# tennisonliu/bayesian-neural-network

Measured on AMD Instinct MI355X. Metric: MC-forward-samples/sec + KL-elements/sec, 784-1200-1200-10 BNN, higher is better.
Workload: dtype bf16

## Files before the change

bayesian-neural-network_amd/bnn_hip/_lib.py:

```python
from __future__ import annotations

import ctypes as C
import os

_HERE = os.path.dirname(os.path.abspath(__file__))
LIB_PATH = os.environ.get("BNN_HIP_LIB") or os.path.join(_HERE, "libbnn_hip.so")
ABI_VERSION = 9

F32, BF16 = 0, 1
MATH_F32, MATH_BF16, MATH_BF16X3 = 0, 1, 2
EPS_PHILOX, EPS_MEMORY, EPS_ZERO = 0, 1, 2
PRIOR_GAUSS, PRIOR_MIXTURE = 0, 1
NLL_REGRESSION, NLL_CLASSIFICATION = 0, 1
FORM_AUTO, FORM_TILE, FORM_GEMM, FORM_GEMM_KSLICE, FORM_BLOCK256 = 0, 1, 2, 3, 4

EXPORTS = (
    "bnn_version", "bnn_philox_rounds", "bnn_status_string",
    "bnn_bbb_linear_fwd_workspace_bytes", "bnn_bbb_split_scratch_bytes", "bnn_bbb_split_scratch_zero_bytes", "bnn_bbb_linear_fwd",
    "bnn_bbb_linear_bwd_workspace_bytes",
    "bnn_bbb_linear_bwd", "bnn_lr_linear_bwd_workspace_bytes", "bnn_lr_linear_bwd", "bnn_adam_step", "bnn_nll_bwd", "bnn_mc_softmax_mean", "bnn_elbo_loss",
    "bnn_elbo_loss_nll_bwd", "bnn_stage_inputs", "bnn_stage_inputs_cast", "bnn_bbb_sample_weights", "bnn_bbb_sample_workspace_bytes",
    "bnn_lr_linear_fwd_workspace_bytes", "bnn_lr_split_scratch_bytes", "bnn_lr_split_scratch_zero_bytes", "bnn_lr_linear_fwd", "bnn_lr_final_fwd", "bnn_lr_plan", "bnn_bbb_plan", "bnn_lr_prepare_bytes", "bnn_lr_prepare", "bnn_lr_prepare_x3_bytes", "bnn_lr_prepare_x3", "bnn_lr_prepare_many",
    "bnn_gauss_kl_workspace_bytes", "bnn_gauss_kl",
    "bnn_elbo_finalize", "bnn_bbb_final_fwd", "bnn_bbb_final_scratch_bytes", "bnn_philox_normal", "bnn_cast_bf16", "bnn_softplus", "bnn_eval_prepare",
    "bnn_ece_workspace_bytes", "bnn_ece", "bnn_snr_db", "bnn_snr_prune", "bnn_mc_predictive",
    "bnn_bandit_rows", "bnn_bandit_act", "bnn_bandit_replay",
    "bnn_bandit_rows_group", "bnn_bandit_act_group", "bnn_bandit_replay_group", "bnn_mlp_group_fwd", "bnn_mlp_group_train",
    "bnn_bbb_group_workspace_bytes", "bnn_bbb_group_fwd", "bnn_bbb_group_train",
    "bnn_dense_fwd", "bnn_dense_plan", "bnn_dropout_mask",
    "bnn_dense_loss", "bnn_dense_bwd", "bnn_sgd_step",
    "bnn_epoch_permutation", "bnn_epoch_stage",
    "bnn_snr_select_workspace_bytes", "bnn_snr_select", "bnn_prune_codes", "bnn_pruned_fwd", "bnn_prune_sweep_tail",
    "bnn_acquire_topk_workspace_bytes", "bnn_acquire_topk", "bnn_acquire_compose", "bnn_acquire_random",
    "bnn_param_hist_workspace_bytes", "bnn_param_hist",
    "bnn_mc_score_workspace_bytes", "bnn_mc_score",
    "bnn_sparse_count", "bnn_sparse_fill", "bnn_sparse_fwd",
)


class Prior(C.Structure):
    _fields_ = [("kind", C.c_int32), ("sigma_p", C.c_float), ("pi", C.c_float),
                ("sigma1", C.c_float), ("sigma2", C.c_float)]


class BbbFwdArgs(C.Structure):
    _fields_ = [
        ("struct_bytes", C.c_uint32),
        ("n_samples", C.c_int32), ("batch", C.c_int32), ("in_features", C.c_int32), ("out_features", C.c_int32),
        ("x", C.c_void_p), ("x_dtype", C.c_int32), ("x_per_sample", C.c_int32),
        ("w_mu", C.c_void_p), ("w_rho", C.c_void_p), ("b_mu", C.c_void_p), ("b_rho", C.c_void_p),
        ("eps_mode", C.c_int32), ("math", C.c_int32),
        ("eps_w", C.c_void_p), ("eps_b", C.c_void_p),
        ("seed", C.c_uint64), ("layer_id", C.c_uint32), ("sample_offset", C.c_uint32),
        ("sample_counter", C.c_void_p), ("sample_group", C.c_uint32), ("sample_group_stride", C.c_uint32),
        ("eps_w_dump", C.c_void_p), ("eps_b_dump", C.c_void_p),
        ("prior", Prior),
        ("want_stats", C.c_int32), ("relu", C.c_int32),
        ("workspace", C.c_void_p), ("workspace_bytes", C.c_size_t),
        ("log_prior", C.c_void_p), ("log_q", C.c_void_p),
        ("y", C.c_void_p), ("y_dtype", C.c_int32), ("form", C.c_int32),
        ("split_scratch", C.c_void_p), ("split_scratch_bytes", C.c_size_t), ("w_sigma", C.c_void_p),
        ("w_sampled", C.c_void_p), ("b_sampled", C.c_void_p), ("rider", C.c_void_p), ("y_bf16_copy", C.c_void_p),
        ("w_sampled_t_out", C.c_void_p), ("x_lo", C.c_void_p), ("y_lo", C.c_void_p),
    ]


SAMPLE_MAX_LAYERS = 8


class SampleLayer(C.Structure):
    _fields_ = [
        ("in_features", C.c_int32), ("out_features", C.c_int32), ("layer_id", C.c_uint32), ("reserved", C.c_int32),
        ("w_mu", C.c_void_p), ("w_rho", C.c_void_p), ("b_mu", C.c_void_p), ("b_rho", C.c_void_p),
        ("w_out", C.c_void_p), ("b_out", C.c_void_p), ("workspace", C.c_void_p), ("workspace_bytes", C.c_size_t),
        ("prior", Prior), ("reserved2", C.c_int32),
    ]


class SampleArgs(C.Structure):
    _fields_ = [
        ("struct_bytes", C.c_uint32), ("n_layers", C.c_int32), ("n_samples", C.c_int32), ("sample_offset", C.c_uint32),
        ("seed", C.c_uint64), ("sample_counter", C.c_void_p), ("sample_group", C.c_uint32), ("sample_group_stride", C.c_uint32),
        ("layer", SampleLayer * SAMPLE_MAX_LAYERS),
        ("cast_src", C.c_void_p), ("cast_dst", C.c_void_p), ("cast_n", C.c_int64),
    ]


class LrRider(C.Structure):
    _fields_ = [
        ("struct_bytes", C.c_uint32), ("in_features", C.c_int32), ("out_features", C.c_int32),
        ("w_mu", C.c_void_p), ("w_rho", C.c_void_p), ("b_mu", C.c_void_p), ("b_rho", C.c_void_p),
        ("w_frag", C.c_void_p), ("w_frag_bytes", C.c_size_t), ("kl_workspace", C.c_void_p), ("kl_workspace_bytes", C.c_size_t),
    ]


class LrFwdArgs(C.Structure):
    _fields_ = [
        ("struct_bytes", C.c_uint32),
        ("n_samples", C.c_int32), ("batch", C.c_int32), ("in_features", C.c_int32), ("out_features", C.c_int32),
        ("x", C.c_void_p), ("x_dtype", C.c_int32), ("x_per_sample", C.c_int32),
        ("w_mu", C.c_void_p), ("w_rho", C.c_void_p), ("b_mu", C.c_void_p), ("b_rho", C.c_void_p),
        ("eps_mode", C.c_int32), ("math", C.c_int32),
        ("eps_act", C.c_void_p), ("eps_b", C.c_void_p),
        ("seed", C.c_uint64), ("layer_id", C.c_uint32), ("sample_offset", C.c_uint32),
        ("sample_counter", C.c_void_p), ("sample_group", C.c_uint32), ("sample_group_stride", C.c_uint32),
        ("eps_act_dump", C.c_void_p), ("eps_b_dump", C.c_void_p),
        ("sigma_p", C.c_float), ("want_kl", C.c_int32), ("relu", C.c_int32), ("form", C.c_int32),
        ("workspace", C.c_void_p), ("workspace_bytes", C.c_size_t),
        ("kl_out", C.c_void_p),
        ("y", C.c_void_p), ("y_dtype", C.c_int32), ("reserved2", C.c_int32),
        ("x_sq", C.c_void_p), ("y_sq", C.c_void_p), ("w_frag", C.c_void_p), ("v_out", C.c_void_p),
        ("hfac_out", C.c_void_p), ("y_bf16_copy", C.c_void_p),
        ("rider", C.POINTER(LrRider)), ("split_scratch", C.c_void_p), ("split_scratch_bytes", C.c_size_t),
        ("x_lo", C.c_void_p), ("y_lo", C.c_void_p),
    ]


class BbbBwdArgs(C.Structure):
    _fields_ = [
        ("struct_bytes", C.c_uint32),
        ("n_samples", C.c_int32), ("batch", C.c_int32), ("in_features", C.c_int32), ("out_features", C.c_int32),
        ("x", C.c_void_p), ("x_per_sample", C.c_int32), ("relu", C.c_int32),
        ("gy", C.c_void_p), ("y", C.c_void_p),
        ("w_mu", C.c_void_p), ("w_rho", C.c_void_p), ("b_mu", C.c_void_p), ("b_rho", C.c_void_p),
        ("eps_mode", C.c_int32), ("math", C.c_int32),
        ("eps_w", C.c_void_p), ("eps_b", C.c_void_p),
        ("seed", C.c_uint64), ("layer_id", C.c_uint32), ("sample_offset", C.c_uint32),
        ("prior", Prior), ("gx_relu_mask", C.c_int32),
        ("g_log_prior", C.c_void_p), ("g_log_q", C.c_void_p),
        ("g_w_mu", C.c_void_p), ("g_w_rho", C.c_void_p), ("g_b_mu", C.c_void_p), ("g_b_rho", C.c_void_p),
        ("g_x", C.c_void_p),
        ("workspace", C.c_void_p), ("workspace_bytes", C.c_size_t),
        ("sample_counter", C.c_void_p), ("w_sampled", C.c_void_p),
        ("w_sampled_t", C.c_void_p), ("gy_bf16", C.c_void_p), ("g_x_bf16", C.c_void_p),
    ]


class LrBwdArgs(C.Structure):
    _fields_ = [
        ("struct_bytes", C.c_uint32),
        ("n_samples", C.c_int32), ("batch", C.c_int32), ("in_features", C.c_int32), ("out_features", C.c_int32),
        ("x", C.c_void_p), ("x_per_sample", C.c_int32), ("relu", C.c_int32),
        ("gy", C.c_void_p), ("y", C.c_void_p), ("v", C.c_void_p),
        ("w_mu", C.c_void_p), ("w_rho", C.c_void_p), ("b_mu", C.c_void_p), ("b_rho", C.c_void_p),
        ("eps_mode", C.c_int32), ("math", C.c_int32),
        ("eps_act", C.c_void_p), ("eps_b", C.c_void_p),
        ("seed", C.c_uint64), ("layer_id", C.c_uint32), ("sample_offset", C.c_uint32),
        ("sigma_p", C.c_float), ("gx_relu_mask", C.c_int32),
        ("g_kl", C.c_void_p),
        ("g_w_mu", C.c_void_p), ("g_w_rho", C.c_void_p), ("g_b_mu", C.c_void_p), ("g_b_rho", C.c_void_p),
        ("g_x", C.c_void_p), ("workspace", C.c_void_p), ("workspace_bytes", C.c_size_t),
        ("sample_counter", C.c_void_p), ("hfac", C.c_void_p),
    ]


ADAM_MAX_TENSORS = 16


class AdamArgs(C.Structure):
    _fields_ = [
        ("struct_bytes", C.c_uint32), ("n_tensors", C.c_int32),
        ("param", C.c_void_p * ADAM_MAX_TENSORS), ("grad", C.c_void_p * ADAM_MAX_TENSORS),
        ("exp_avg", C.c_void_p * ADAM_MAX_TENSORS), ("exp_avg_sq", C.c_void_p * ADAM_MAX_TENSORS),
        ("numel", C.c_int64 * ADAM_MAX_TENSORS),
        ("lr", C.c_double), ("beta1", C.c_double), ("beta2", C.c_double), ("eps", C.c_double), ("weight_decay", C.c_double),
        ("step", C.c_uint32), ("bump_by", C.c_uint32),
        ("lr_device", C.c_void_p), ("step_device", C.c_void_p), ("step_advance", C.c_int32), ("grad_dtype", C.c_int32),
        ("ticket", C.c_void_p), ("bump_counter", C.c_void_p),
    ]


class LossArgs(C.Structure):
    _fields_ = [("beta", C.c_void_p), ("total_samples", C.c_float), ("grad_scale", C.c_float), ("out4", C.c_void_p),
                ("g_a", C.c_void_p), ("g_b", C.c_void_p), ("g_kl3", C.c_void_p), ("g_logits", C.c_void_p)]


class FinalizeArgs(C.Structure):
    _fields_ = [
        ("struct_bytes", C.c_uint32),
        ("n_layers", C.c_int32), ("local_reparam", C.c_int32),
        ("n_samples", C.c_int32), ("batch", C.c_int32), ("classes", C.c_int32),
        ("layer_workspace", C.c_void_p * 8), ("layer_in", C.c_int32 * 8), ("layer_out", C.c_int32 * 8),
        ("prior", Prior),
        ("logits", C.c_void_p), ("target", C.c_void_p),
        ("nll_mode", C.c_int32), ("nll_sigma", C.c_float),
        ("log_prior", C.c_void_p), ("log_q", C.c_void_p), ("kl", C.c_void_p), ("nll", C.c_void_p),
        ("sample_counter", C.c_void_p), ("sample_counter_inc", C.c_uint32), ("reserved", C.c_uint32),
        ("sums", C.c_void_p), ("ticket", C.c_void_p), ("scratch", C.c_void_p), ("scratch_bytes", C.c_size_t),
        ("group_samples", C.c_int32), ("target_per_group", C.c_int32),
        ("loss", C.POINTER(LossArgs)),
    ]


class Plan(C.Structure):
    _fields_ = [("form", C.c_int32), ("k_classes", C.c_int32), ("waves", C.c_int32), ("batch_rows", C.c_int32),
                ("k_slices", C.c_int32), ("blocks", C.c_int32), ("lds_bytes", C.c_int32), ("features_per_block", C.c_int32)]


PREPARE_MAX = 8
PREPARE_MANY_MAX = 8


class PrepareArgs(C.Structure):
    _fields_ = [("struct_bytes", C.c_uint32), ("n_softplus", C.c_int32),
                ("rho", C.c_void_p * PREPARE_MAX), ("sigma", C.c_void_p * PREPARE_MAX), ("n", C.c_int64 * PREPARE_MAX),
                ("cast_src", C.c_void_p), ("cast_dst", C.c_void_p), ("cast_dst_sq", C.c_void_p), ("cast_n", C.c_int64),
                ("cast_dst_lo", C.c_void_p)]


PREDICTIVE_MAX_QUANTILES = 8
PREDICTIVE_MAX_QUANTILE_SAMPLES = 1024


class McPredictiveArgs(C.Structure):
    _fields_ = [("struct_bytes", C.c_uint32), ("mode", C.c_int32),
                ("groups", C.c_int32), ("n_samples", C.c_int32), ("batch", C.c_int32), ("classes", C.c_int32),
                ("logits", C.c_void_p), ("scale", C.c_float), ("sigma", C.c_float),
                ("probs", C.c_void_p), ("preds", C.c_void_p), ("predictive_entropy", C.c_void_p),
                ("expected_entropy", C.c_void_p), ("mutual_information", C.c_void_p),
                ("mean", C.c_void_p), ("variance", C.c_void_p), ("predictive_variance", C.c_void_p),
                ("n_quantiles", C.c_int32), ("reserved", C.c_int32),
                ("quantile", C.c_double * PREDICTIVE_MAX_QUANTILES), ("quantiles", C.c_void_p)]


BANDIT_MAX_ACTIONS = 64
BANDIT_MAX_BUFFER = 8192


class BanditActArgs(C.Structure):
    _fields_ = [("struct_bytes", C.c_uint32), ("n_actions", C.c_int32), ("n_labels", C.c_int32), ("n_samples", C.c_int32),
                ("output_sample_stride", C.c_int32), ("context_dim", C.c_int32), ("n_contexts", C.c_int64),
                ("buffer_size", C.c_int32), ("sample_counter_inc", C.c_uint32), ("max_steps", C.c_int64),
                ("n_indices", C.c_int64), ("epsilon", C.c_float), ("reserved", C.c_uint32), ("seed", C.c_uint64),
                ("x", C.c_void_p), ("labels", C.c_void_p), ("rewards", C.c_void_p), ("oracle", C.c_void_p),
                ("indices", C.c_void_p), ("outputs", C.c_void_p), ("step", C.c_void_p), ("cur_index", C.c_void_p),
                ("rows", C.c_void_p), ("actions", C.c_void_p), ("reward_out", C.c_void_p), ("regrets", C.c_void_p),
                ("counts", C.c_void_p), ("ring_index", C.c_void_p), ("ring_action", C.c_void_p), ("ring_reward", C.c_void_p),
                ("sample_counter", C.c_void_p)]


class BanditReplayArgs(C.Structure):
    _fields_ = [("struct_bytes", C.c_uint32), ("batch_size", C.c_int32), ("num_batches", C.c_int32), ("buffer_size", C.c_int32),
                ("context_dim", C.c_int32), ("n_actions", C.c_int32), ("n_contexts", C.c_int64), ("seed", C.c_uint64),
                ("step", C.c_void_p), ("x", C.c_void_p), ("ring_index", C.c_void_p), ("ring_action", C.c_void_p),
                ("ring_reward", C.c_void_p), ("workspace", C.c_void_p), ("slab", C.c_void_p), ("targets", C.c_void_p),
                ("n_batches", C.c_void_p)]


MLP_GROUP_MAX_IN = 128
MLP_GROUP_MAX_HIDDEN = 128
MLP_GROUP_MAX_OUT = 1
MLP_GROUP_MAX_BATCH = 64
MLP_GROUP_MAX_BATCHES = 128
MLP_GROUP_MAX_AGENTS = 4096


class BanditGroupArgs(C.Structure):
    _fields_ = [("struct_bytes", C.c_uint32), ("n_agents", C.c_int32), ("blocks_host", C.c_void_p), ("blocks", C.c_void_p),
                ("blocks_bytes", C.c_int64)]


class MlpGroupAgent(C.Structure):
    _fields_ = [("param", C.c_void_p * 6), ("exp_avg", C.c_void_p * 6), ("exp_avg_sq", C.c_void_p * 6), ("step", C.c_void_p),
                ("lr", C.c_void_p), ("slab", C.c_void_p), ("targets", C.c_void_p), ("n_batches", C.c_void_p), ("loss", C.c_void_p),
                ("rows", C.c_void_p), ("outputs", C.c_void_p)]


class MlpGroupArgs(C.Structure):
    _fields_ = [("struct_bytes", C.c_uint32), ("n_agents", C.c_int32), ("in_features", C.c_int32), ("hidden", C.c_int32),
                ("out_features", C.c_int32), ("batch", C.c_int32), ("max_batches", C.c_int32), ("n_rows", C.c_int32),
                ("beta1", C.c_double), ("beta2", C.c_double), ("eps", C.c_double), ("weight_decay", C.c_double),
                ("agents_host", C.c_void_p), ("agents", C.c_void_p), ("agents_bytes", C.c_int64)]


BBB_GROUP_MAX_SAMPLES = 8


class BbbGroupAgent(C.Structure):
    _fields_ = [("param", C.c_void_p * 12), ("exp_avg", C.c_void_p * 12), ("exp_avg_sq", C.c_void_p * 12), ("step", C.c_void_p),
                ("lr", C.c_void_p), ("slab", C.c_void_p), ("targets", C.c_void_p), ("n_batches", C.c_void_p),
                ("loss_info", C.c_void_p), ("rows", C.c_void_p), ("outputs", C.c_void_p), ("sample_counter", C.c_void_p),
                ("workspace", C.c_void_p), ("eps_seed", C.c_uint64), ("eps_mode", C.c_int32), ("reserved", C.c_int32)]


class BbbGroupArgs(C.Structure):
    _fields_ = [("struct_bytes", C.c_uint32), ("n_agents", C.c_int32), ("in_features", C.c_int32), ("hidden", C.c_int32),
                ("out_features", C.c_int32), ("batch", C.c_int32), ("max_batches", C.c_int32), ("n_rows", C.c_int32),
                ("n_samples", C.c_int32), ("prior", Prior),
                ("beta1", C.c_double), ("beta2", C.c_double), ("eps", C.c_double), ("weight_decay", C.c_double),
                ("beta", C.c_float * MLP_GROUP_MAX_BATCHES), ("workspace_bytes", C.c_int64),
# ... 396 lines not shown
```

bayesian-neural-network_amd/bnn_hip/engine.py:

```python
from __future__ import annotations

import os
from typing import List, Optional, Sequence, Tuple

import torch

from . import _lib as L
from . import ops
from .functional import AllReduceSumFn, BBBLinearFn, ElboFn, LayerCall, LRLinearFn, NetCall, NLLFn
from .ops import Predictive
from .runtime import state, take_samples


CAST_INPUT_MIN_SAMPLES = 4
CAST_INPUT_MIN_SAMPLES_LR = 1
LR_SQUARES_MIN_SAMPLES = 7
SPLIT_MIN_SAMPLES = 4
SPLIT_MIN_WEIGHTS = 250_000
SPLIT_MAX_UNITS = 1024

FUSED_ELBO_NODE = True


FINAL_ROWS_MAX_SAMPLES = 16
# ... 433 lines not shown
        self.counter = torch.tensor([first], dtype=torch.int32, device=dev)
        S = self.n_local
        B = self.x.shape[-2]
        self.lr_x3 = (self.lr and state.math == L.MATH_BF16X3 and self.G > 1 and len(self.specs) >= 2 and S >= LR_SQUARES_MIN_SAMPLES and
                      self.x.dtype == torch.float32 and
                      all(sp.in_out[0] % 8 == 0 and lr_use_prepare(sp.in_out[1], S, B) for sp in self.specs[:-1]))
        math_mode = self.math = L.MATH_BF16X3 if self.lr_x3 else effective_math(self.lr)
        self.x3 = math_mode == L.MATH_BF16X3
        hid = torch.float32 if math_mode == L.MATH_F32 else torch.bfloat16
        self.bufs, self.ws, self.bufs_lo = [], [], []
        nl_ = len(self.specs)
        for i, sp in enumerate(self.specs):
            fin, fout = sp.in_out
            last = i == nl_ - 1
            f32_out = last or (self.lr_x3 and i == nl_ - 2)
            self.bufs.append(torch.empty((S, B, fout), dtype=torch.float32 if f32_out else hid, device=dev))
            self.bufs_lo.append(torch.empty((S, B, fout), dtype=torch.bfloat16, device=dev) if (self.x3 and not f32_out) else None)
            self.ws.append(ops.lr_workspace(fout, dev) if self.lr else ops.bbb_workspace(S, fout, dev))
        keys = ("kl",) if self.lr else ("log_prior", "log_q")
        self.out = {k: torch.zeros(S, dtype=torch.float32, device=dev) for k in keys + ("nll",)}
        self._sums = torch.zeros((self.G, 4), dtype=torch.float32, device=dev)
        self.sums = self._sums if self.G > 1 else self._sums.view(4)
        self.ticket = torch.zeros(1, dtype=torch.int32, device=dev)
        self.scratch = ops.final_scratch(S, dev) if (not self.lr or wide_nll(self.specs, B) or self.specs[-1].in_out[1] <= 16) else None
        self.lib = [use_block_gemm(sp, B, hid) for sp in self.specs]
        self.lib_w = [torch.empty((S, sp.in_out[1], sp.in_out[0]), dtype=torch.bfloat16, device=dev) if lb else None
                      for sp, lb in zip(self.specs, self.lib)]
        self.lib_b = [torch.empty((S, sp.in_out[1]), dtype=torch.float32, device=dev) if lb else None
                      for sp, lb in zip(self.specs, self.lib)]
        for i, (sp, lb) in enumerate(zip(self.specs, self.lib)):
            if lb:
                self.ws[i] = ops.sample_workspace(S, sp.in_out[0], sp.in_out[1], dev)
        shared0 = self.lr and not self.G > 1 and lr_unit_samples(S, True) == 1
        k3s_first = (self.lr and hid == torch.bfloat16 and len(self.specs) > 1 and self.specs[0].in_out[0] % 8 == 0 and
                     lr_use_split(self.specs[0].in_out[1], S, B, shared0) and not self.G > 1)
        shared0 = shared0 and k3s_first
        self.x16 = (torch.empty(self.x.shape, dtype=torch.bfloat16, device=dev)
                    if (hid == torch.bfloat16 and self.x.dtype == torch.float32 and
                        (self.lib[0] or S >= (CAST_INPUT_MIN_SAMPLES_LR if self.lr else CAST_INPUT_MIN_SAMPLES)) and
                        not k3s_first) else None)
        self.x16_lo = torch.empty(self.x.shape, dtype=torch.bfloat16, device=dev) if (self.x3 and self.x16 is not None) else None
        self.lr_sq = self.lr and (self.x16 is not None or (k3s_first and hid == torch.bfloat16)) and S >= LR_SQUARES_MIN_SAMPLES
        self.x16_sq = torch.empty(self.x.shape, dtype=torch.bfloat16, device=dev) if (self.lr_sq and self.x16 is not None) else None
        self.bufs_sq = [torch.empty(b.shape, dtype=torch.bfloat16, device=dev)
                        if (self.lr_sq and i < len(self.bufs) - 1 and b.dtype == torch.bfloat16) else None for i, b in enumerate(self.bufs)]
        self.split = [ops.split_scratch(S, B, sp.in_out[1], dev)
                      if (not self.lr and hid == torch.bfloat16 and not self.lib[i] and
                          use_split(sp.in_out[0], sp.in_out[1], S, B)) else None
                      for i, sp in enumerate(self.specs)]
        self.lr_split = [ops.lr_split_scratch(lr_unit_samples(S, shared0 and i == 0), B, sp.in_out[1], dev)
                         if (self.lr and hid == torch.bfloat16 and i < len(self.specs) - 1 and
                             lr_use_split(sp.in_out[1], S, B, shared0 and i == 0)) else None
                         for i, sp in enumerate(self.specs)]
        self.wsigma = [torch.empty_like(sp.m.weight_rho.detach())
                      if (not self.lr and hid == torch.bfloat16 and not lb and hoist_sigma(*sp.in_out, S, B)) else None
                      for sp, lb in zip(self.specs, self.lib)]
        self.wfrag = [None] * len(self.specs)
        if self.lr_sq:
            frag_bytes = L.load().bnn_lr_prepare_x3_bytes if self.lr_x3 else L.load().bnn_lr_prepare_bytes
            self.wfrag = [torch.empty(frag_bytes(*sp.in_out) // 4, dtype=torch.float32, device=dev)
                          if (lr_use_prepare(sp.in_out[1], S, B) and not (shared0 and i == 0) and not (self.lr_x3 and i == nl_ - 1)) else None
                          for i, sp in enumerate(self.specs)]
        nl = len(self.specs)
        self.lr_rider = None
        if (self.lr_sq and not self.lr_x3 and self.wfrag[nl - 1] is None and any(w is not None for w in self.wfrag) and
                self.scratch is not None and not wide_nll(self.specs, B) and self.specs[-1].in_out[1] <= 16 and S <= LR_FINAL_ROWS_MAX_SAMPLES):
            self.wfrag[nl - 1] = torch.empty(L.load().bnn_lr_prepare_bytes(*self.specs[-1].in_out) // 4, dtype=torch.float32, device=dev)
        if (self.lr and hid == torch.bfloat16 and nl > 1 and self.wfrag[nl - 1] is None and self.scratch is not None and
                not wide_nll(self.specs, B) and self.specs[-1].in_out[1] <= 16 and S <= 16 and self.lr_split[nl - 2] is not None and
                lr_kslice_expected(*self.specs[-2].in_out, S, B)):
            sp = self.specs[-1]
            self.lr_rider = dict(w_mu=sp.m.weight_mu.detach(), w_rho=sp.m.weight_rho.detach(), b_mu=sp.m.bias_mu.detach(),
                                 b_rho=sp.m.bias_rho.detach(), workspace=self.ws[nl - 1],
                                 w_frag=torch.empty(L.load().bnn_lr_prepare_bytes(*sp.in_out) // 4, dtype=torch.float32, device=dev))
        self.pre_from = presample_from(self.specs, S, B, hid)
        self.rows = self.pre_from >= 0
        self.w_pre, self.b_pre = [None] * len(self.specs), [None] * len(self.specs)
        if self.rows:
            for i in range(self.pre_from + 1, len(self.specs)):
                k_i, n_i = self.specs[i].in_out
                self.w_pre[i] = torch.empty((S, n_i, k_i), dtype=torch.bfloat16, device=dev)
                self.b_pre[i] = torch.empty((S, n_i), dtype=torch.float32, device=dev)
                self.ws[i] = ops.sample_workspace(S, k_i, n_i, dev)
        self.graph = None
        self.calls = None
        if capture == "calls":
            rec_stream = self.stream if self.stream is not None else torch.cuda.current_stream()
            with torch.cuda.stream(rec_stream):
                self._enqueue()
            take_samples(self.total_samples)
            torch.cuda.synchronize()
            before = torch.cuda.memory_stats(dev).get("allocation.all.allocated", 0)
            with L.recording() as calls, torch.cuda.stream(rec_stream):
                self._eager()
            take_samples(self.total_samples * self.per_replay)
            torch.cuda.synchronize()
            if torch.cuda.memory_stats(dev).get("allocation.all.allocated", 0) != before:
                raise ops.BnnHipError("GraphedElbo(capture='calls'): the evaluation allocated device memory while it was recorded -- "
                                      "a replay would launch on freed buffers; use capture=True (hipGraph) for this configuration")
            self.calls = list(calls)
        elif capture:
            self._enqueue()
            take_samples(self.total_samples)
            torch.cuda.synchronize()
            side = self.stream if self.stream is not None else torch.cuda.Stream()
            side.wait_stream(torch.cuda.current_stream())
            with torch.cuda.stream(side):
                g = torch.cuda.CUDAGraph()
                with torch.cuda.graph(g, stream=side):
                    self._eager()
            torch.cuda.current_stream().wait_stream(side)
            self.graph = g

    def _enqueue(self):
        math_mode = self.math
        h_sq, h_lo = None, None
        hoist = [i for i, w in enumerate(self.wsigma) if w is not None]
        h = self.x
        if self.x16 is not None or hoist:
            ops.eval_prepare([self.specs[i].m.weight_rho.detach() for i in hoist], [self.wsigma[i] for i in hoist],
                             cast=self.x if self.x16 is not None else None, cast_out=self.x16,
                             cast_out_sq=self.x16_sq, cast_out_lo=self.x16_lo)
            if self.x16 is not None:
                h, h_sq, h_lo = self.x16, self.x16_sq, self.x16_lo
        last = len(self.specs) - 1
        if self.lr and any(w is not None for w in self.wfrag):
            jobs = [dict(w_mu=sp.m.weight_mu.detach(), w_rho=sp.m.weight_rho.detach(), b_mu=sp.m.bias_mu.detach(),
                         b_rho=sp.m.bias_rho.detach(), workspace=self.ws[i], out=self.wfrag[i])
                    for i, sp in enumerate(self.specs) if self.wfrag[i] is not None]
            ops.lr_prepare_many(jobs, x3=self.lr_x3)
        grp = dict(sample_group=self.group, sample_group_stride=self.samples) if self.G > 1 else {}
        fin_kw = dict(layer_in=[sp.in_out[0] for sp in self.specs], layer_out=[sp.in_out[1] for sp in self.specs],
                      local_reparam=self.lr, prior=self.specs[0].m._prior_spec, n_samples=self.n_local,
                      target=self.target, mode=self.net.mode, nll_sigma=self.sigma, sample_counter=self.counter,
                      sample_counter_inc=self.total_samples, out=self.out, sums=self._sums,
                      ticket=self.ticket, scratch=self.scratch, group_samples=self.group)
        for i, sp in enumerate(self.specs):
            p = tuple(t.detach() for t in (sp.m.weight_mu, sp.m.weight_rho, sp.m.bias_mu, sp.m.bias_rho))
            common = dict(n_samples=self.n_local, math_mode=math_mode, relu=sp.relu, y_dtype=self.bufs[i].dtype,
                          eps_mode=L.EPS_PHILOX, seed=state.seed, layer_id=sp.layer_id, sample_offset=self.lo,
                          sample_counter=self.counter, workspace=self.ws[i], out=self.bufs[i], form=state.form, **grp)
            if self.lr:
                if self.lr_x3 and i == last:
                    common["math_mode"] = L.MATH_F32
                if i == last and self.scratch is not None and not wide_nll(self.specs, self.x.shape[-2]):
                    ops.lr_final_fwd((h,) + p, dict(sigma_p=sp.m._prior_spec.sigma_p, want_kl=True, x_sq=h_sq,
                                                    w_frag=self.lr_rider["w_frag"] if self.lr_rider is not None else self.wfrag[i],
                                                    **common), dict(workspaces=self.ws, **fin_kw))
                    return
                ops.lr_linear_fwd(h, *p, sigma_p=sp.m._prior_spec.sigma_p, want_kl=True, x_sq=h_sq,
                                  out_sq=self.bufs_sq[i], w_frag=self.wfrag[i], split_scratch=self.lr_split[i],
                                  rider=self.lr_rider if i == last - 1 else None,
                                  x_lo=h_lo if self.lr_x3 else None, out_lo=self.bufs_lo[i] if self.lr_x3 else None, **common)
                h_sq = self.bufs_sq[i]
            elif self.lib[i]:
                self._sample_layer(i, grp)
                ops.bbb_sampled_matmul(h, self.lib_w[i], self.lib_b[i], n_samples=self.n_local, relu=sp.relu,
                                       y_dtype=self.bufs[i].dtype, out=self.bufs[i])
                if i == last:
                    ops.elbo_finalize(workspaces=self.ws, logits=self.bufs[i], **fin_kw)
            else:
                kw = dict(prior=sp.m._prior_spec, want_stats=True, split_scratch=self.split[i], w_sigma=self.wsigma[i], **common)
                if self.x3:
                    kw.update(x_lo=h_lo if h.dtype == torch.bfloat16 else None, out_lo=self.bufs_lo[i])
                if i == last and self.rows:
                    ops.bbb_final_fwd((h, None, None, None, None),
                                      dict(n_samples=self.n_local, prior=sp.m._prior_spec, math_mode=math_mode, relu=sp.relu,
                                           y_dtype=self.bufs[i].dtype, eps_mode=L.EPS_ZERO, want_stats=False, out=self.bufs[i],
                                           w_sampled=self.w_pre[i], b_sampled=self.b_pre[i]),
                                      dict(workspaces=self.ws, **fin_kw))
                elif i == last:
                    ops.bbb_final_fwd((h,) + p, kw, dict(workspaces=self.ws[:last], **fin_kw))
                else:
                    if i == self.pre_from:
                        kw["rider"] = ops.build_sample_job(
                            [dict(w_mu=q.m.weight_mu.detach(), w_rho=q.m.weight_rho.detach(), b_mu=q.m.bias_mu.detach(),
                                  b_rho=q.m.bias_rho.detach(), prior=q.m._prior_spec, layer_id=q.layer_id,
                                  workspace=self.ws[j], w_out=self.w_pre[j], b_out=self.b_pre[j])
                             for j, q in enumerate(self.specs) if j > i],
                            n_samples=self.n_local, seed=state.seed, sample_offset=self.lo, sample_counter=self.counter, **grp)
                    ops.bbb_linear_fwd(h, *p, **kw)
            h, h_lo = self.bufs[i], self.bufs_lo[i]
        if self.lr:
            ops.elbo_finalize(workspaces=self.ws, logits=h, **fin_kw)

    def _sample_layer(self, i, grp):
        sp = self.specs[i]
        p = tuple(t.detach() for t in (sp.m.weight_mu, sp.m.weight_rho, sp.m.bias_mu, sp.m.bias_rho))
        ops.bbb_sample_weights([dict(w_mu=p[0], w_rho=p[1], b_mu=p[2], b_rho=p[3], prior=sp.m._prior_spec, layer_id=sp.layer_id,
                                     workspace=self.ws[i], w_out=self.lib_w[i], b_out=self.lib_b[i])],
                               n_samples=self.n_local, seed=state.seed, sample_offset=self.lo, sample_counter=self.counter, **grp)

    def _eager(self):
        for _ in range(self.per_replay):
            self._enqueue()

    def replay(self) -> torch.Tensor:
        if self.calls is not None:
            for fn, args, name in self.calls:
                rc = fn(*args)
                if rc:
                    L.check(rc, name)
            take_samples(self.total_samples * self.per_replay)
            return self.sums
        if self.stream is not None:
            with torch.cuda.stream(self.stream):
                self.graph.replay() if self.graph is not None else self._eager()
        elif self.graph is not None:
            self.graph.replay()
        else:
            self._eager()
        take_samples(self.total_samples * self.per_replay)
        return self.sums

    @property
    def logits(self) -> torch.Tensor:
        return self.bufs[-1]


class GraphedPredict(GraphedElbo):

    def __init__(self, net, x: torch.Tensor, samples: int, capture: bool = True, stream: Optional[torch.cuda.Stream] = None):
        if net.mode != "classification":
            raise ops.BnnHipError("GraphedPredict: the MC-averaged class prediction exists for classification networks")
        xf = net._flat(x)
        self.probs = torch.empty((xf.shape[0], net._specs()[-1].in_out[1]), dtype=torch.float32, device=x.device)
        self.preds = torch.empty(xf.shape[0], dtype=torch.int64, device=x.device)
        super().__init__(net, x, torch.zeros(xf.shape[0], dtype=torch.int64, device=x.device), samples, capture=capture, stream=stream)

    def _enqueue(self):
        super()._enqueue()
        ops.mc_softmax_mean(self.logits, 1.0 / self.samples, out_probs=self.probs, out_preds=self.preds if self.world == 1 else None,
                            want_preds=self.world == 1)

    def replay(self):
        super().replay()
        if self.world > 1:
            import torch.distributed as dist
            dist.all_reduce(self.probs, op=dist.ReduceOp.SUM)
            self.preds.copy_(torch.argmax(self.probs, dim=1))
        return self.preds, self.probs


class GraphedPredictive(GraphedElbo):

    def __init__(self, net, x: torch.Tensor, samples: int, quantiles=None, sigma: float = 1.0, capture=True,
                 stream: Optional[torch.cuda.Stream] = None, stacked: bool = False):
        mode = net.mode
        if mode not in ("classification", "regression"):
            raise Exception("Training mode must be either 'regression' or 'classification'")
        if mode == "classification" and quantiles:
            raise ops.BnnHipError("GraphedPredictive: quantiles are a regression summary")
        self.mode, self.quantile_levels, self.pred_sigma = mode, ops.quantile_levels(quantiles), float(sigma)
        if self.quantile_levels and dist_info()[1] > 1:
            raise ops.BnnHipError("GraphedPredictive: quantiles need every MC sample on one rank (sample sharding is on)")
        G = int(x.shape[0]) if stacked else 1
        B = net._flat(x[0] if stacked else x).shape[0]
        Cc = net._specs()[-1].in_out[1]
        lead = (G, B) if stacked else (B,)
        target = (torch.zeros(lead, dtype=torch.int64, device=x.device) if mode == "classification"
                  else torch.zeros(lead + (Cc,), dtype=torch.float32, device=x.device))
        self._pred = ops.predictive_buffers(mode, G, B, Cc, x.device, self.quantile_levels)
        self.result = self._pred if stacked else _first_minibatch(self._pred)
        super().__init__(net, x, target, samples, sigma=sigma, capture=capture, stream=stream, stacked=stacked)

    def _enqueue(self):
        super()._enqueue()
# ... 63 lines not shown
```

bayesian-neural-network_amd/bnn_hip/ops.py:

```python
from __future__ import annotations

import ctypes as C
import math
from dataclasses import dataclass
from typing import NamedTuple, Optional, Sequence

import torch

from . import _lib as L
from ._lib import BnnHipError


@dataclass(frozen=True)
class PriorSpec:
    mixture: bool = False
    sigma_p: float = 1.0
    pi: float = 0.5
    sigma1: float = 1.0
    sigma2: float = 1.0

    @staticmethod
    def from_init(prior_init: Sequence[float], mixture: bool) -> "PriorSpec":
        if mixture:
            assert len(prior_init) == 3, "Scale Mixture Prior requires three values in prior initialisation"
            return PriorSpec(True, 1.0, float(prior_init[0]), math.exp(prior_init[1]), math.exp(prior_init[2]))
        assert len(prior_init) == 1, "Gaussian Prior requires one value in prior initialisation"
        return PriorSpec(False, float(prior_init[0]))

    def c(self) -> L.Prior:
        return L.Prior(L.PRIOR_MIXTURE if self.mixture else L.PRIOR_GAUSS, self.sigma_p, self.pi,
                       self.sigma1, self.sigma2)


def _stream() -> int:
    return torch._C._cuda_getCurrentRawStream(torch._C._cuda_getDevice())


def require_device(*tensors: torch.Tensor):
    for t in tensors:
        if t is not None and not t.is_cuda:
            raise BnnHipError(
                "bnn_hip: the Bayes-by-backprop hot path runs on a ROCm device only (tensor is on "
                f"{t.device}); there is no CPU fallback.  Move the module and its inputs to DEVICE.")


def _f32c(t: torch.Tensor, name: str) -> torch.Tensor:
    if t.dtype != torch.float32:
        raise BnnHipError(f"{name} must be float32, got {t.dtype}")
    return t if t.is_contiguous() else t.contiguous()


def _ptr(t: Optional[torch.Tensor]) -> Optional[int]:
    return None if t is None else t.data_ptr()


def _dt(t: torch.Tensor) -> int:
    if t.dtype == torch.float32:
        return L.F32
    if t.dtype == torch.bfloat16:
        return L.BF16
    raise BnnHipError(f"activations must be float32 or bfloat16, got {t.dtype}")


def _exact_unless_bf16(math_mode: int) -> int:
    return L.MATH_F32 if math_mode == L.MATH_BF16X3 else math_mode


def _x3(x: torch.Tensor, n_samples: int):
    if x.dim() == 2:
        xs = x if x.is_contiguous() else x.contiguous()
        return xs, x.shape[0], x.shape[1], 0
    if x.dim() == 3:
        if x.shape[0] < 1 or n_samples % x.shape[0]:
            raise BnnHipError(f"x has {x.shape[0]} row blocks, which does not divide {n_samples} samples")
        xs = x if x.is_contiguous() else x.contiguous()
        return xs, x.shape[1], x.shape[2], n_samples // x.shape[0]
    raise BnnHipError(f"x must be [batch,in] or [rows,batch,in], got {tuple(x.shape)}")


def bbb_workspace(n_samples: int, out_features: int, device) -> torch.Tensor:
    nbytes = L.load().bnn_bbb_linear_fwd_workspace_bytes(n_samples, out_features)
    return torch.empty(nbytes // 4, dtype=torch.float32, device=device)


def split_scratch(n_samples: int, batch: int, out_features: int, device) -> torch.Tensor:
    lib = L.load()
    nbytes = lib.bnn_bbb_split_scratch_bytes(n_samples, batch, out_features)
    t = torch.empty((nbytes + 3) // 4, dtype=torch.int32, device=device)
    t[:lib.bnn_bbb_split_scratch_zero_bytes(n_samples, batch, out_features) // 4].zero_()
    return t


_split_cache = {}


def split_scratch_cached(n_samples: int, batch: int, out_features: int, device) -> torch.Tensor:
    if torch.cuda.is_current_stream_capturing():
        return split_scratch(n_samples, batch, out_features, device)
    key = (str(device), torch.cuda.current_stream(device).cuda_stream, n_samples, batch, out_features)
    t = _split_cache.get(key)
    if t is None:
        if len(_split_cache) >= 16:
            _split_cache.clear()
        t = _split_cache[key] = split_scratch(n_samples, batch, out_features, device)
    return t


def final_scratch(n_samples: int, device) -> torch.Tensor:
    nbytes = L.load().bnn_bbb_final_scratch_bytes(n_samples)
    return torch.zeros((nbytes + 3) // 4, dtype=torch.int32, device=device)


def lr_split_scratch(n_samples: int, batch: int, out_features: int, device) -> torch.Tensor:
    lib = L.load()
    nbytes = lib.bnn_lr_split_scratch_bytes(n_samples, batch, out_features)
    t = torch.empty((nbytes + 3) // 4, dtype=torch.int32, device=device)
    t[:lib.bnn_lr_split_scratch_zero_bytes(n_samples, batch, out_features) // 4].zero_()
    return t


_lr_split_cache = {}


def lr_split_scratch_cached(n_samples: int, batch: int, out_features: int, device) -> torch.Tensor:
    if torch.cuda.is_current_stream_capturing():
        return lr_split_scratch(n_samples, batch, out_features, device)
    key = (str(device), torch.cuda.current_stream(device).cuda_stream, n_samples, batch, out_features)
    t = _lr_split_cache.get(key)
    if t is None:
        if len(_lr_split_cache) >= 16:
            _lr_split_cache.clear()
        t = _lr_split_cache[key] = lr_split_scratch(n_samples, batch, out_features, device)
    return t


def lr_workspace(out_features: int, device) -> torch.Tensor:
    nbytes = L.load().bnn_lr_linear_fwd_workspace_bytes(out_features)
    return torch.empty(nbytes // 4, dtype=torch.float32, device=device)


def _y16(a, y: torch.Tensor) -> torch.Tensor:
    if y.dtype != torch.float32:
        raise BnnHipError("want_y16 goes with fp32 y")
    y16 = torch.empty(tuple(y.shape), dtype=torch.bfloat16, device=y.device)
    a.y_bf16_copy = y16.data_ptr()
    return y16


def _bbb_build(x, w_mu, w_rho, b_mu, b_rho, *, n_samples: int, prior: PriorSpec, math_mode: int,
               relu: bool, y_dtype: torch.dtype, eps_mode: int, eps_w=None, eps_b=None, seed: int = 0,
               layer_id: int = 0, sample_offset: int = 0, want_stats: bool = True,
               want_scalars: bool = False, dump_eps: bool = False, workspace=None, sample_counter=None,
               out=None, split_scratch=None, w_sigma=None, form: int = 0, sample_group: int = 0,
               sample_group_stride: int = 0, w_sampled=None, b_sampled=None, rider=None, want_y16: bool = False, wt_out=None,
               x_lo=None, out_lo=None):
    require_device(x, w_mu, w_rho, b_mu, b_rho, eps_w, eps_b, w_sampled, b_sampled)
    if w_sampled is not None:
        if w_sampled.dtype != torch.bfloat16 or b_sampled is None or b_sampled.dtype != torch.float32 or \
                not w_sampled.is_contiguous() or not b_sampled.is_contiguous() or w_sampled.dim() != 3:
            raise BnnHipError("w_sampled must be contiguous bf16 [S,out,in], b_sampled contiguous fp32 [S,out]")
        if w_sampled.shape[0] != n_samples or b_sampled.numel() != n_samples * w_sampled.shape[1]:
            raise BnnHipError("w_sampled / b_sampled do not match n_samples")
        N, K = w_sampled.shape[1], w_sampled.shape[2]
        xs, B, Kx, per_sample = _x3(x, n_samples)
        if Kx != K:
            raise BnnHipError(f"shape mismatch: x[...,{Kx}] sampled weight {tuple(w_sampled.shape)}")
        y = out if out is not None else torch.empty((n_samples, B, N), dtype=y_dtype, device=xs.device)
        a = L.BbbFwdArgs()
        a.struct_bytes = C.sizeof(L.BbbFwdArgs)
        a.n_samples, a.batch, a.in_features, a.out_features = n_samples, B, K, N
        a.x, a.x_dtype, a.x_per_sample = xs.data_ptr(), _dt(xs), per_sample
        a.eps_mode, a.math = L.EPS_ZERO, L.MATH_BF16
        a.want_stats, a.relu = 0, int(relu)
        a.y, a.y_dtype = y.data_ptr(), _dt(y)
        a.w_sampled, a.b_sampled = w_sampled.data_ptr(), b_sampled.data_ptr()
        if wt_out is not None:
            require_device(wt_out)
            if wt_out.dtype != torch.bfloat16 or not wt_out.is_contiguous() or tuple(wt_out.shape) != (n_samples, K, N):
                raise BnnHipError("wt_out must be a contiguous bf16 [samples,in,out] tensor")
            a.w_sampled_t_out = wt_out.data_ptr()
        a.form = int(form)
        y16 = _y16(a, y) if want_y16 else None
        return a, dict(y=y, y16=y16, workspace=None, log_prior=None, log_q=None, eps_w=None, eps_b=None), (xs, w_sampled, b_sampled, y)
    w_mu, w_rho = _f32c(w_mu, "weight_mu"), _f32c(w_rho, "weight_rho")
    b_mu, b_rho = _f32c(b_mu, "bias_mu"), _f32c(b_rho, "bias_rho")
    N, K = w_mu.shape
    xs, B, Kx, per_sample = _x3(x, n_samples)
    if Kx != K or tuple(w_rho.shape) != (N, K) or tuple(b_mu.shape) != (N,) or tuple(b_rho.shape) != (N,):
        raise BnnHipError(f"shape mismatch: x[...,{Kx}] weight {tuple(w_mu.shape)} bias {tuple(b_mu.shape)}")
    dev = xs.device
    y = out if out is not None else torch.empty((n_samples, B, N), dtype=y_dtype, device=dev)
    if want_stats and workspace is None:
        workspace = bbb_workspace(n_samples, N, dev)
    lp = torch.empty(n_samples, dtype=torch.float32, device=dev) if want_scalars else None
    lq = torch.empty(n_samples, dtype=torch.float32, device=dev) if want_scalars else None
    if eps_mode == L.EPS_MEMORY:
        eps_w, eps_b = _f32c(eps_w, "eps_w"), _f32c(eps_b, "eps_b")
        if eps_w.numel() != n_samples * N * K or eps_b.numel() != n_samples * N:
            raise BnnHipError("eps_w/eps_b must be [samples,out,in] / [samples,out]")
    dw = torch.empty((n_samples, N, K), dtype=torch.float32, device=dev) if dump_eps else None
    db = torch.empty((n_samples, N), dtype=torch.float32, device=dev) if dump_eps else None
    a = L.BbbFwdArgs()
    a.struct_bytes = C.sizeof(L.BbbFwdArgs)
    a.n_samples, a.batch, a.in_features, a.out_features = n_samples, B, K, N
    a.x, a.x_dtype, a.x_per_sample = xs.data_ptr(), _dt(xs), per_sample
    a.w_mu, a.w_rho, a.b_mu, a.b_rho = w_mu.data_ptr(), w_rho.data_ptr(), b_mu.data_ptr(), b_rho.data_ptr()
    a.eps_mode, a.math = eps_mode, math_mode
    a.eps_w, a.eps_b = _ptr(eps_w) if eps_mode == L.EPS_MEMORY else None, _ptr(eps_b) if eps_mode == L.EPS_MEMORY else None
    a.seed, a.layer_id, a.sample_offset = seed & 0xFFFFFFFFFFFFFFFF, layer_id, sample_offset & 0xFFFFFFFF
    a.sample_counter = _ptr(sample_counter)
    a.sample_group, a.sample_group_stride = int(sample_group), int(sample_group_stride)
    a.form = int(form)
    a.eps_w_dump, a.eps_b_dump = _ptr(dw), _ptr(db)
    a.prior = prior.c()
    a.want_stats, a.relu = int(want_stats), int(relu)
    a.workspace = _ptr(workspace) if want_stats else None
    a.workspace_bytes = workspace.numel() * 4 if (want_stats and workspace is not None) else 0
    a.log_prior, a.log_q = _ptr(lp), _ptr(lq)
    a.y, a.y_dtype = y.data_ptr(), _dt(y)
    y_lo = None
    if math_mode == L.MATH_BF16X3:
        if xs.dtype == torch.bfloat16:
            if x_lo is None or x_lo.dtype != torch.bfloat16 or tuple(x_lo.shape) != tuple(x.shape) or not x_lo.is_contiguous():
                raise BnnHipError("bf16x3 math on bf16 x needs x_lo: the contiguous bf16 low plane, shaped like x")
            require_device(x_lo)
            a.x_lo = x_lo.data_ptr()
        if y.dtype == torch.bfloat16:
            y_lo = out_lo if out_lo is not None else torch.empty(tuple(y.shape), dtype=torch.bfloat16, device=dev)
            if y_lo.dtype != torch.bfloat16 or y_lo.numel() != y.numel() or not y_lo.is_contiguous():
                raise BnnHipError("out_lo must be a contiguous bf16 tensor shaped like y")
            a.y_lo = y_lo.data_ptr()
    if w_sigma is not None:
        a.w_sigma = w_sigma.data_ptr()
    if split_scratch is not None:
        a.split_scratch = split_scratch.data_ptr()
        a.split_scratch_bytes = split_scratch.numel() * split_scratch.element_size()
    if rider is not None:
        a.rider = C.addressof(rider[0])
    res = dict(y=y, y16=_y16(a, y) if want_y16 else None, workspace=workspace, log_prior=lp, log_q=lq, eps_w=dw, eps_b=db, y_lo=y_lo)
    keep = (xs, w_mu, w_rho, b_mu, b_rho, eps_w, eps_b, sample_counter, split_scratch, w_sigma, rider, x_lo, y_lo)
    a._keep = keep
    return a, res, keep


def bbb_linear_fwd(x, w_mu, w_rho, b_mu, b_rho, **kw):
    lib = L.load()
    a, res, keep = _bbb_build(x, w_mu, w_rho, b_mu, b_rho, **kw)
    L.check(lib.bnn_bbb_linear_fwd(C.byref(a), _stream()), "bnn_bbb_linear_fwd")
    return res


def _plan_dict(pl: L.Plan) -> dict:
    return {k: getattr(pl, k) for k, _ in L.Plan._fields_}


def bbb_plan(x, w_mu, w_rho, b_mu, b_rho, **kw) -> dict:
    a, res, keep = _bbb_build(x, w_mu, w_rho, b_mu, b_rho, **kw)
    pl = L.Plan()
    L.check(L.load().bnn_bbb_plan(C.byref(a), C.byref(pl)), "bnn_bbb_plan")
    return _plan_dict(pl)


def sample_workspace(n_samples: int, fin: int, fout: int, device) -> torch.Tensor:
    nbytes = L.load().bnn_bbb_sample_workspace_bytes(n_samples, fin, fout) or \
        L.load().bnn_bbb_linear_fwd_workspace_bytes(n_samples, fout)
    return torch.empty(nbytes // 4, dtype=torch.float32, device=device)


def build_sample_job(layers, *, n_samples: int, seed: int = 0, sample_offset: int = 0, sample_counter=None, cast=None,
                     sample_group: int = 0, sample_group_stride: int = 0):
    if not 1 <= len(layers) <= L.SAMPLE_MAX_LAYERS:
        raise BnnHipError(f"bbb_sample_weights: 1..{L.SAMPLE_MAX_LAYERS} layers per launch")
    a = L.SampleArgs()
    a.struct_bytes = C.sizeof(L.SampleArgs)
    a.n_layers, a.n_samples = len(layers), int(n_samples)
    a.seed, a.sample_offset = seed & 0xFFFFFFFFFFFFFFFF, sample_offset & 0xFFFFFFFF
    a.sample_counter = _ptr(sample_counter)
    a.sample_group, a.sample_group_stride = int(sample_group), int(sample_group_stride)
    res, keep = [], [sample_counter]
    for i, ly in enumerate(layers):
        w_mu, w_rho = _f32c(ly["w_mu"], "weight_mu"), _f32c(ly["w_rho"], "weight_rho")
        b_mu, b_rho = _f32c(ly["b_mu"], "bias_mu"), _f32c(ly["b_rho"], "bias_rho")
        require_device(w_mu, w_rho, b_mu, b_rho)
        N, K = w_mu.shape
        if K % 8:
            raise BnnHipError("bbb_sample_weights: in_features must be a multiple of 8")
        if tuple(w_rho.shape) != (N, K) or tuple(b_mu.shape) != (N,) or tuple(b_rho.shape) != (N,):
            raise BnnHipError("bbb_sample_weights: parameter shapes disagree")
        dev = w_mu.device
        ws = ly.get("workspace")
        if ws is None:
            ws = sample_workspace(n_samples, K, N, dev)
        w = ly.get("w_out")
        if w is None:
            w = torch.empty((n_samples, N, K), dtype=torch.bfloat16, device=dev)
        b = ly.get("b_out")
        if b is None:
            b = torch.empty((n_samples, N), dtype=torch.float32, device=dev)
        if w.dtype != torch.bfloat16 or w.numel() != n_samples * N * K or b.dtype != torch.float32 or b.numel() != n_samples * N:
            raise BnnHipError("bbb_sample_weights: w_out must be bf16 [S,out,in], b_out fp32 [S,out]")
        e = a.layer[i]
        e.in_features, e.out_features, e.layer_id = K, N, int(ly.get("layer_id", i))
        e.w_mu, e.w_rho, e.b_mu, e.b_rho = w_mu.data_ptr(), w_rho.data_ptr(), b_mu.data_ptr(), b_rho.data_ptr()
        e.w_out, e.b_out = w.data_ptr(), b.data_ptr()
        e.workspace, e.workspace_bytes = ws.data_ptr(), ws.numel() * 4
        e.prior = ly["prior"].c()
        res.append(dict(w=w, b=b, workspace=ws))
        keep.append((w_mu, w_rho, b_mu, b_rho, w, b, ws))
    if cast is not None:
        src, dst = cast
        require_device(src, dst)
        if src.dtype != torch.float32 or dst.dtype != torch.bfloat16 or src.numel() != dst.numel() or \
                not src.is_contiguous() or not dst.is_contiguous():
            raise BnnHipError("bbb_sample_weights: cast = (contiguous fp32 source, contiguous bf16 destination) of one size")
        a.cast_src, a.cast_dst, a.cast_n = src.data_ptr(), dst.data_ptr(), src.numel()
        keep.append((src, dst))
    a._keep = keep
    return a, res, keep


def bbb_sample_weights(layers, **kw):
    a, res, keep = build_sample_job(layers, **kw)
    L.check(L.load().bnn_bbb_sample_weights(C.byref(a), _stream()), "bnn_bbb_sample_weights")
# ... 598 lines not shown
    require_device(src0, dst0, src1, dst1, word)
    for s_, d_ in ((src0, dst0), (src1, dst1)):
        if s_ is None:
            continue
        if s_.dtype != d_.dtype or s_.numel() != d_.numel() or not s_.is_contiguous() or not d_.is_contiguous():
            raise BnnHipError("stage_inputs: source and destination must be contiguous, same dtype and size")
    nb = lambda t: 0 if t is None else t.numel() * t.element_size()
    if cast0 is not None:
        require_device(cast0)
        if src0.dtype != torch.float32 or cast0.dtype != torch.bfloat16 or cast0.numel() != src0.numel() or not cast0.is_contiguous():
            raise BnnHipError("stage_inputs: cast0 must be a contiguous bf16 tensor of the fp32 src0's size")
        L.check(lib.bnn_stage_inputs_cast(_ptr(src0), _ptr(dst0), nb(src0), _ptr(src1), _ptr(dst1), nb(src1), _ptr(word),
                                          float(value), cast0.data_ptr(), _stream()), "bnn_stage_inputs_cast")
        return
    L.check(lib.bnn_stage_inputs(_ptr(src0), _ptr(dst0), nb(src0), _ptr(src1), _ptr(dst1), nb(src1), _ptr(word), float(value),
                                 _stream()), "bnn_stage_inputs")


def nll_bwd(logits, target, g_nll, mode: str, sigma: float = 1.0):
    lib = L.load()
    require_device(logits, target, g_nll)
    lg = _f32c(logits, "logits")
    S, B, Cc = lg.shape
    gn = _f32c(g_nll.reshape(-1), "g_nll")
    if gn.numel() != S:
        raise BnnHipError("g_nll must have one element per MC sample")
    tg, m = _nll_target(target, mode, B, Cc)
    out = torch.empty_like(lg)
    L.check(lib.bnn_nll_bwd(lg.data_ptr(), tg.data_ptr(), gn.data_ptr(), out.data_ptr(), S, B, Cc, m, float(sigma), _stream()),
            "bnn_nll_bwd")
    return out


def adam_step(params, grads, exp_avgs, exp_avg_sqs, *, lr: float, betas, eps: float, weight_decay: float, step: int = 0,
              lr_device=None, step_device=None, ticket=None, bump_counter=None, bump_by: int = 0):
    lib = L.load()
    n = len(params)
    for lo in range(0, n, L.ADAM_MAX_TENSORS):
        hi = min(n, lo + L.ADAM_MAX_TENSORS)
        a = L.AdamArgs()
        a.struct_bytes = C.sizeof(L.AdamArgs)
        a.n_tensors = hi - lo
        for j in range(lo, hi):
            p, g, m, v = params[j], grads[j], exp_avgs[j], exp_avg_sqs[j]
            require_device(p, g, m, v)
            for t_ in (p, m, v):
                if t_.dtype != torch.float32 or not t_.is_contiguous() or t_.numel() != p.numel():
                    raise BnnHipError("adam_step: tensors must be contiguous float32 of the parameter's size")
            if g.dtype not in (torch.float32, torch.bfloat16) or g.dtype != grads[lo].dtype or not g.is_contiguous() or \
                    g.numel() != p.numel():
                raise BnnHipError("adam_step: gradients must be contiguous float32 or bfloat16 (one dtype per launch) of the "
                                  "parameter's size")
            a.param[j - lo], a.grad[j - lo] = p.data_ptr(), g.data_ptr()
            a.exp_avg[j - lo], a.exp_avg_sq[j - lo] = m.data_ptr(), v.data_ptr()
            a.numel[j - lo] = p.numel()
        a.lr, a.beta1, a.beta2, a.eps, a.weight_decay = float(lr), float(betas[0]), float(betas[1]), float(eps), float(weight_decay)
        a.step = int(step)
        a.grad_dtype = _dt(grads[lo])
        a.lr_device = _ptr(lr_device)
        a.step_device = _ptr(step_device)
        a.step_advance = int(lo == 0)
        if lo == 0 and ticket is not None and step_device is not None:
            if ticket.numel() < 16 or ticket.element_size() != 4:
                raise BnnHipError("adam_step: ticket must be a zeroed array of 16 32-bit words")
            a.ticket = ticket.data_ptr()
            if bump_counter is not None:
                a.bump_counter, a.bump_by = bump_counter.data_ptr(), int(bump_by)
        elif bump_counter is not None and lo == 0:
            raise BnnHipError("adam_step: bump_counter needs a device step and a ticket word")
        L.check(lib.bnn_adam_step(C.byref(a), _stream()), "bnn_adam_step")


def softplus(rho: torch.Tensor, out: Optional[torch.Tensor] = None) -> torch.Tensor:
    lib = L.load()
    require_device(rho)
    rho = _f32c(rho, "rho")
    if out is None:
        out = torch.empty_like(rho)
    L.check(lib.bnn_softplus(rho.data_ptr(), out.data_ptr(), rho.numel(), _stream()), "bnn_softplus")
    return out


def eval_prepare(rhos=(), sigmas=None, cast: Optional[torch.Tensor] = None, cast_out: Optional[torch.Tensor] = None,
                 cast_out_sq: Optional[torch.Tensor] = None, want_sq: bool = False, cast_out_lo: Optional[torch.Tensor] = None):
    lib = L.load()
    rhos = [_f32c(r, "rho") for r in rhos]
    require_device(*rhos, cast)
    if len(rhos) > L.PREPARE_MAX:
        raise BnnHipError(f"eval_prepare: at most {L.PREPARE_MAX} tensors per launch")
    if sigmas is None:
        sigmas = [torch.empty_like(r) for r in rhos]
    a = L.PrepareArgs()
    a.struct_bytes = C.sizeof(L.PrepareArgs)
    a.n_softplus = len(rhos)
    for i, (r, sg) in enumerate(zip(rhos, sigmas)):
        if sg.shape != r.shape or sg.dtype != torch.float32 or not sg.is_contiguous():
            raise BnnHipError("eval_prepare: sigma must be a contiguous fp32 tensor of rho's shape")
        a.rho[i], a.sigma[i], a.n[i] = r.data_ptr(), sg.data_ptr(), r.numel()
    if cast is not None:
        cast = _f32c(cast, "x")
        if cast_out is None:
            cast_out = torch.empty(cast.shape, dtype=torch.bfloat16, device=cast.device)
        if want_sq and cast_out_sq is None:
            cast_out_sq = torch.empty(cast.shape, dtype=torch.bfloat16, device=cast.device)
        a.cast_src, a.cast_dst, a.cast_dst_sq, a.cast_n = cast.data_ptr(), cast_out.data_ptr(), _ptr(cast_out_sq), cast.numel()
        if cast_out_lo is not None:
            if cast_out_lo.dtype != torch.bfloat16 or cast_out_lo.numel() != cast.numel() or not cast_out_lo.is_contiguous():
                raise BnnHipError("eval_prepare: cast_out_lo must be a contiguous bf16 tensor of the input's size")
            require_device(cast_out_lo)
            a.cast_dst_lo = cast_out_lo.data_ptr()
    if not rhos and cast is None:
        return [], None, None
    L.check(lib.bnn_eval_prepare(C.byref(a), _stream()), "bnn_eval_prepare")
    return list(sigmas), cast_out, cast_out_sq


def ece_bins(probs: torch.Tensor, labels: torch.Tensor, bin_edges) -> torch.Tensor:
    lib = L.load()
    require_device(probs, labels)
    pr = _f32c(probs, "probs")
    if pr.dim() != 2 or labels.numel() != pr.shape[0]:
        raise BnnHipError("ece: probs must be [n, classes] and labels [n]")
    lb = labels.to(torch.int64).contiguous()
    edges = (C.c_double * len(bin_edges))(*[float(e) for e in bin_edges])
    ws = torch.empty(lib.bnn_ece_workspace_bytes() // 8, dtype=torch.float64, device=pr.device)
    out = torch.empty(1 + 3 * (len(bin_edges) - 1), dtype=torch.float32, device=pr.device)
    L.check(lib.bnn_ece(pr.data_ptr(), lb.data_ptr(), pr.shape[0], pr.shape[1], edges, len(bin_edges), ws.data_ptr(),
                        ws.numel() * 8, out.data_ptr(), _stream()), "bnn_ece")
    return out


def snr_db(mu: torch.Tensor, rho: torch.Tensor, out: Optional[torch.Tensor] = None) -> torch.Tensor:
    lib = L.load()
    require_device(mu, rho)
    mu, rho = _f32c(mu, "mu"), _f32c(rho, "rho")
    if mu.numel() != rho.numel():
        raise BnnHipError("snr_db: mu and rho must have the same number of elements")
    if out is None:
        out = torch.empty_like(mu)
    L.check(lib.bnn_snr_db(mu.data_ptr(), rho.data_ptr(), mu.numel(), out.data_ptr(), _stream()), "bnn_snr_db")
    return out


def snr_prune_(mu: torch.Tensor, rho: torch.Tensor, threshold: float, kept: Optional[torch.Tensor] = None):
    lib = L.load()
    require_device(mu, rho)
    if mu.dtype != torch.float32 or rho.dtype != torch.float32 or not mu.is_contiguous() or not rho.is_contiguous() or \
            mu.numel() != rho.numel():
        raise BnnHipError("snr_prune_: contiguous float32 mu and rho of one size")
    L.check(lib.bnn_snr_prune(mu.data_ptr(), rho.data_ptr(), mu.numel(), float(threshold), _ptr(kept), _stream()),
            "bnn_snr_prune")


def _typed(t: torch.Tensor, dtype: torch.dtype, name: str, numel: Optional[int] = None) -> torch.Tensor:
    require_device(t)
    if t.dtype != dtype or not t.is_contiguous():
        raise BnnHipError(f"{name} must be a contiguous {dtype} tensor")
    if numel is not None and t.numel() != numel:
        raise BnnHipError(f"{name} must have {numel} elements, got {t.numel()}")
    return t


def bandit_act_args(*, x, labels, rewards, oracle, outputs, n_samples: int, output_sample_stride: int, step, cur_index, rows,
                    actions, reward_out, regrets, counts, ring_index, ring_action, ring_reward, epsilon: float, seed: int,
                    indices=None, sample_counter=None, sample_counter_inc: int = 0) -> L.BanditActArgs:
    N, d = x.shape
    K, A = rewards.shape[0], rewards.shape[1]
    T = actions.numel()
    a = L.BanditActArgs()
    a.struct_bytes = C.sizeof(L.BanditActArgs)
    a.n_actions, a.n_labels, a.n_samples, a.output_sample_stride = A, K, int(n_samples), int(output_sample_stride)
    a.context_dim, a.n_contexts, a.buffer_size = d, N, ring_index.numel()
    a.max_steps, a.epsilon, a.seed = T, float(epsilon), int(seed) & 0xFFFFFFFFFFFFFFFF
    keep = [_typed(x, torch.float32, "x"), _typed(labels, torch.int64, "labels", N), _typed(rewards, torch.float32, "rewards", K * A * 3),
            _typed(oracle, torch.float32, "oracle", K), _typed(outputs, torch.float32, "outputs"),
            _typed(step, torch.int32, "step", 1), _typed(cur_index, torch.int32, "cur_index", 1),
            _typed(rows, torch.float32, "rows", A * (d + A)), _typed(actions, torch.int64, "actions"),
            _typed(reward_out, torch.float32, "reward_out", T), _typed(regrets, torch.float64, "regrets", T + 1),
            _typed(counts, torch.int64, "counts", K * A), _typed(ring_index, torch.int32, "ring_index"),
            _typed(ring_action, torch.int32, "ring_action", ring_index.numel()),
            _typed(ring_reward, torch.float32, "ring_reward", ring_index.numel())]
    (a.x, a.labels, a.rewards, a.oracle, a.outputs, a.step, a.cur_index, a.rows, a.actions, a.reward_out, a.regrets, a.counts,
     a.ring_index, a.ring_action, a.ring_reward) = (t.data_ptr() for t in keep)
    if outputs.numel() < (n_samples - 1) * output_sample_stride + A:
        raise BnnHipError("outputs is smaller than its samples and stride say")
    if indices is not None:
        keep.append(_typed(indices, torch.int64, "indices"))
        a.indices, a.n_indices = indices.data_ptr(), indices.numel()
# ... 860 lines not shown
```

bayesian-neural-network_amd/bnn_hip/runtime.py:

```python
from __future__ import annotations

import os
import threading

from . import _lib as L

_lock = threading.Lock()


class _State:
    def __init__(self):
        m = os.environ.get("BNN_HIP_MATH", "bf16").lower()
        self.math = L.MATH_F32 if m in ("f32", "fp32", "float32") else L.MATH_BF16X3 if m in ("bf16x3", "x3") else L.MATH_BF16
        self.seed = int(os.environ.get("BNN_HIP_SEED", "2026"))
        self.host_eps = os.environ.get("BNN_HIP_EPS", "device").lower() == "host"
        self.counter = 0
        self.shard_samples = False
        self.form = L.FORM_AUTO
        self.device_counter = None


state = _State()


def set_math(mode: str):
    m = mode.lower()
    if m in ("bf16", "bfloat16"):
        state.math = L.MATH_BF16
    elif m in ("f32", "fp32", "float32"):
        state.math = L.MATH_F32
    elif m in ("bf16x3", "x3"):
        state.math = L.MATH_BF16X3
    else:
        raise ValueError(f"unknown math mode {mode!r}")


def get_math() -> str:
    return {L.MATH_BF16: "bf16", L.MATH_F32: "f32", L.MATH_BF16X3: "bf16x3"}[state.math]


def manual_seed(seed: int, counter: int = 0):
    with _lock:
        state.seed = int(seed) & 0xFFFFFFFFFFFFFFFF
        state.counter = int(counter)


def take_samples(n: int) -> int:
    with _lock:
        first = state.counter
        state.counter = (state.counter + int(n)) & 0xFFFFFFFF
        return first


def set_host_eps(flag: bool):
    state.host_eps = bool(flag)


def shard_samples(flag: bool = True):
    state.shard_samples = bool(flag)
```

bayesian-neural-network_amd/csrc/bbb_linear.hip:

```cpp
#include "bnn_device.h"
#include "bnn_fin.h"
#include "bbb_sample_body.h"
#include "bbb_block_gemm.h"
#include "../../include/bnn_hip.h"
#include <string.h>

namespace bnn {

struct BbbK {
  const void* x;
  long x_sstride;
  const float* w_mu;
  const float* w_rho;
  const float* w_sigma;
  const float* b_mu;
  const float* b_rho;
  const float* eps_w;
  const float* eps_b;
  float* eps_w_dump;
  float* eps_b_dump;
  void* y;
  float4* ws;
  int S, B, K, N;
  __bf16* y16;
  int eps_mode, prior_kind, want_stats, relu, y_bf16, spb;
  int ksl;
  float4* ks_part;
  uint32_t* ks_ticket;
#ifdef BNN_TUNE
  int tune;
#endif
  Xcd2D xc;
  int ldw;
  const __bf16* w_pre;
  const float* b_pre;
  __bf16* wt_out;
  const float* mask;
  long mask_sstride;
  uint32_t k0, k1, layer_id, sample_offset;
  const uint32_t* sample_counter;
  int xg;
  uint32_t sgrp, sgrp_stride;
  float inv2var1, c1, inv2var2, c2, pi;
  const void* x_lo;
  void* y_lo;
#ifdef BNN_STAMPS
  unsigned long long* dbg;
#endif
};

#ifdef BNN_STAMPS
#define BNN_STAMP(i)                                                                              \
  do {                                                                                            \
    if (p.dbg && threadIdx.x == 0)                                                                \
      p.dbg[((size_t)blockIdx.x) * 16 + (i)] = __builtin_amdgcn_s_memtime(); \
  } while (0)
#define BNN_STAMP_RT(i)                                                                           \
  do {                                                                                            \
    if (p.dbg && threadIdx.x == 0)                                                                \
      p.dbg[((size_t)blockIdx.x) * 16 + (i)] = __builtin_amdgcn_s_memrealtime(); \
  } while (0)
#else
#define BNN_STAMP(i)
#define BNN_STAMP_RT(i)
#endif

template <bool ALIGNED>
__device__ __forceinline__ void load8(const float* __restrict__ p, int valid, float v[8]) {
  if (ALIGNED) {
    if (valid > 0) {
      const float4 a = *reinterpret_cast<const float4*>(p);
      const float4 b = *reinterpret_cast<const float4*>(p + 4);
      v[0] = a.x; v[1] = a.y; v[2] = a.z; v[3] = a.w;
      v[4] = b.x; v[5] = b.y; v[6] = b.z; v[7] = b.w;
    } else {
#pragma unroll
      for (int j = 0; j < 8; ++j) v[j] = 0.0f;
    }
  } else {
#pragma unroll
    for (int j = 0; j < 8; ++j) v[j] = (j < valid) ? p[j] : 0.0f;
  }
}

template <bool ALIGNED>
__device__ __forceinline__ void store8(float* __restrict__ p, int valid, const float v[8]) {
  if (ALIGNED) {
    if (valid > 0) {
      *reinterpret_cast<float4*>(p) = make_float4(v[0], v[1], v[2], v[3]);
      *reinterpret_cast<float4*>(p + 4) = make_float4(v[4], v[5], v[6], v[7]);
    }
  } else {
#pragma unroll
    for (int j = 0; j < 8; ++j)
      if (j < valid) p[j] = v[j];
  }
}

template <int MATH, int XDT, bool ALIGNED>
__device__ __forceinline__ void load_xfrag(const char* __restrict__ xs, long off, int valid, float xv[8], bf16x8& xb) {
  if (XDT == BNN_F32) {
    load8<ALIGNED>(reinterpret_cast<const float*>(xs) + off, valid, xv);
    if (MATH == BNN_MATH_BF16) {
#pragma unroll
      for (int j = 0; j < 8; ++j) xb[j] = (__bf16)xv[j];
    }
  } else {
    const __bf16* p = reinterpret_cast<const __bf16*>(xs) + off;
    if (ALIGNED) {
      if (valid > 0) {
        xb = *reinterpret_cast<const bf16x8*>(p);
      } else {
#pragma unroll
        for (int j = 0; j < 8; ++j) xb[j] = (__bf16)0.0f;
      }
    } else {
#pragma unroll
      for (int j = 0; j < 8; ++j) xb[j] = (j < valid) ? p[j] : (__bf16)0.0f;
    }
    if (MATH == BNN_MATH_F32) {
#pragma unroll
      for (int j = 0; j < 8; ++j) xv[j] = (float)xb[j];
    }
  }
}

__device__ __forceinline__ uint32_t global_sample(const BbbK& p, int s) {
  const uint32_t base = p.sample_offset + (p.sample_counter ? *p.sample_counter : 0u);
// ... 973 lines not shown
      acc[m] = v;
      asm volatile("global_store_dwordx4 %0, %1, off sc1" ::"v"(mine + m * 64), "v"(v) : "memory");
    }
    asm volatile("s_waitcnt vmcnt(0)" ::: "memory");
    __syncthreads();
    if (threadIdx.x == 0) {
      const uint32_t tk = __hip_atomic_fetch_add(p.ks_ticket + item, 1u, __ATOMIC_RELAXED, __HIP_MEMORY_SCOPE_AGENT);
      last_s = (tk == (uint32_t)KS - 1u) ? 1u : 0u;
    }
    __syncthreads();
    if (last_s == 0u) return;
    if (threadIdx.x == 0) __hip_atomic_store(p.ks_ticket + item, 0u, __ATOMIC_RELAXED, __HIP_MEMORY_SCOPE_AGENT);
    f32x4 sum[8];
#pragma unroll
    for (int m = 0; m < 8; ++m) sum[m] = f32x4{0.f, 0.f, 0.f, 0.f};
#pragma nounroll
    for (int j = 0; j < KS; ++j) {
      f32x4 part[8];
      if (j != ks) {
        const float4* src = unit_part + ((size_t)j * NW + wave) * (8 * 64) + lane;
#pragma unroll
        for (int m = 0; m < 8; ++m)
          asm volatile("global_load_dwordx4 %0, %1, off sc1" : "=v"(part[m]) : "v"(src + m * 64) : "memory");
        asm volatile("s_waitcnt vmcnt(0)" ::: "memory");
      } else {
#pragma unroll
        for (int m = 0; m < 8; ++m) part[m] = acc[m];
      }
#pragma unroll
      for (int m = 0; m < 8; ++m) sum[m] += part[m];
    }
#pragma unroll
    for (int m = 0; m < 8; ++m) acc[m] = sum[m];
#pragma unroll
    for (int i = 0; i < 4; ++i) bq[i] = 0.f;
  }
  if (nb < N) {
#pragma unroll
    for (int m = 0; m < 8; ++m) {
      const int brow = m0 + m * 16 + r;
      if (brow < B) {
        f32x4 v = acc[m];
#pragma unroll
        for (int i = 0; i < 4; ++i) {
          float o = v[i] + bq[i];
          if (p.relu) o = fmaxf(o, 0.f);
          v[i] = o;
        }
        const size_t yoff = ((size_t)s * B + brow) * N + nb;
        if (p.y_bf16) {
          __bf16* yp = reinterpret_cast<__bf16*>(p.y) + yoff;
          if (vec_ok) {
            bf16x4 o;
#pragma unroll
            for (int i = 0; i < 4; ++i) o[i] = (__bf16)v[i];
            *reinterpret_cast<bf16x4*>(yp) = o;
          } else {
#pragma unroll
            for (int i = 0; i < 4; ++i)
              if (nb + i < N) yp[i] = (__bf16)v[i];
          }
        } else {
          float* yp = reinterpret_cast<float*>(p.y) + yoff;
          if (vec_ok) {
            *reinterpret_cast<float4*>(yp) = make_float4(v[0], v[1], v[2], v[3]);
          } else {
#pragma unroll
            for (int i = 0; i < 4; ++i)
              if (nb + i < N) yp[i] = v[i];
          }
        }
      }
    }
  }
}

template <int NW, bool SIG, int EPS>
__global__ __launch_bounds__(NW * 64, 4) void bbb_fwd_gemm_kernel(const BbbK p) {
  __shared__ __attribute__((aligned(16))) float4 xt[2][8 * 64];
  __shared__ float bias_s[NW][16];
  bbb_gemm_body<NW, SIG, EPS>(p, xt, bias_s);
}

template <int NF, int SB, int EPS, int NB = 2, bool X3 = false>
__global__ __launch_bounds__(NF * SB * 64, 4) void bbb_fwd_gemm2_kernel(const BbbK p) {
  constexpr int NW = NF * SB;
  static_assert(NB == 2, "two staging buffers");
  constexpr int WPW = 4 / SB;
  constexpr int XPW = 8 / NF;
  constexpr int XT = X3 ? 1024 : 512;
  static_assert(SB == 1 || SB == 2 || SB == 4, "pairs per block");
  static_assert(NF == 2 || NF == 4 || NF == 8, "feature waves per block");
  constexpr int BUF = NF * 256 + SB * XT;
  auto p_idx = [](int buf) { return X3 ? 0 : buf * BUF; };
  auto x_idx = [](int buf) { return X3 ? NF * 256 + buf * (SB * XT) : buf * BUF + NF * 256; };
  __shared__ __attribute__((aligned(16))) float4 sm_all[X3 ? NF * 256 + 2 * SB * XT : NB * BUF + NW * 4];
  float (*bias_s)[16] = reinterpret_cast<float (*)[16]>(sm_all + (X3 ? 0 : NB * BUF));
  const int lane = threadIdx.x & 63, wave = __builtin_amdgcn_readfirstlane(threadIdx.x >> 6);
  const int fw = wave % NF, sb = wave / NF;
  const int r = lane & 15, q = lane >> 4;
  const int K = p.K, N = p.N, B = p.B;
  const int mbs = (B + 127) >> 7;
  const int U = p.S * mbs;
  int tb, ub, in_;
  if (!xcd2d_work_item(p.xc, tb, ub, in_)) return;
  const int unit_raw = ub * SB + sb;
  const bool active = unit_raw < U;
  const int unit = active ? unit_raw : U - 1;
  const int s = unit / mbs, mb = unit - s * mbs;
  const int tile = tb * NF + fw;
  const int n = tile * 16 + r;
  const bool n_ok = n < N;
  const int nc = min(n, N - 1);
  const int m0 = mb * 128;
  const int ksteps = (K + 31) >> 5;
  const uint32_t gs = global_sample(p, s);
  const bool do_stats = p.want_stats && mb == 0 && active;
  const bool do_ls = do_stats && s == 0;
  const bool do_dump = mb == 0 && active;
  const int gpr = (K + 3) >> 2;
  const uint32_t wid = p.layer_id * 4u;
  const __bf16* xs = reinterpret_cast<const __bf16*>(p.x) + (size_t)(s / p.xg) * (size_t)p.x_sstride;
  const __bf16* xs_lo = X3 ? reinterpret_cast<const __bf16*>(p.x_lo) + (size_t)(s / p.xg) * (size_t)p.x_sstride : nullptr;
  const int T = (N + 15) >> 4;

  if (do_stats && tb == 0 && unit == 0 && fw == 0 && lane == 0) p.ws[0] = make_float4(__int_as_float(T), 0.f, 0.f, 0.f);

  const size_t wrow = (size_t)nc * K;
  size_t xrow[XPW];
#pragma unroll
  for (int i = 0; i < XPW; ++i) xrow[i] = (size_t)min(m0 + (fw + i * NF) * 16 + r, B - 1) * K;
  const uint32_t voff_w = ((uint32_t)nc * (uint32_t)K + (uint32_t)(q * 8)) * 4u;
  uint32_t voff_x[XPW];
#pragma unroll
  for (int i = 0; i < XPW; ++i) voff_x[i] = ((uint32_t)xrow[i] + (uint32_t)(q * 8)) * 2u;
  const uint32_t lds0 = (uint32_t)(size_t)(__attribute__((address_space(3))) void*)&sm_all[0];
  auto x_slot = [&](int slot) { return x_idx(slot) + sb * XT; };
  auto stage_fast = [&](int t, int pbuf, int xbuf, auto wp_, auto wx_) __attribute__((always_inline)) {
    if (decltype(wp_)::value) {
#pragma unroll
      for (int i = 0; i < WPW; ++i) {
        const int j = sb * WPW + i;
        const char* base = reinterpret_cast<const char*>((j & 2) ? p.w_sigma : p.w_mu) + (size_t)t * 128 + (j & 1) * 16;
        const uint32_t m0v = lds0 + (uint32_t)((p_idx(pbuf) + (fw * 4 + j) * 64) * 16);
        asm volatile("s_mov_b32 m0, %2\n\ts_nop 0\n\tglobal_load_lds_dwordx4 %0, %1" ::"v"(voff_w), "s"(base), "s"(m0v) : "memory", "m0");
      }
    }
    if (decltype(wx_)::value) {
#pragma unroll
      for (int i = 0; i < XPW; ++i) {
        const char* base = reinterpret_cast<const char*>(xs) + (size_t)t * 64;
        const uint32_t m0v = lds0 + (uint32_t)((x_slot(xbuf) + (fw + i * NF) * 64) * 16);
        asm volatile("s_mov_b32 m0, %2\n\ts_nop 0\n\tglobal_load_lds_dwordx4 %0, %1" ::"v"(voff_x[i]), "s"(base), "s"(m0v) : "memory", "m0");
      }
      if (X3) {
#pragma unroll
        for (int i = 0; i < XPW; ++i) {
          const char* base = reinterpret_cast<const char*>(xs_lo) + (size_t)t * 64;
          const uint32_t m0v = lds0 + (uint32_t)((x_idx(xbuf) + sb * XT + 512 + (fw + i * NF) * 64) * 16);
          asm volatile("s_mov_b32 m0, %2\n\ts_nop 0\n\tglobal_load_lds_dwordx4 %0, %1" ::"v"(voff_x[i]), "s"(base), "s"(m0v) : "memory", "m0");
        }
      }
    }
  };
  auto stage_slow = [&](int t, int pbuf, int xbuf, auto wp_, auto wx_) __attribute__((always_inline)) {
    const int kk = min(t * 32 + q * 8, K - 8);
    if (decltype(wp_)::value) {
#pragma unroll
      for (int i = 0; i < WPW; ++i) {
#ifdef BNN_TUNE
        const int j = ((p.tune & 64) ? (SB - 1 - sb) : sb) * WPW + i;
#else
        const int j = sb * WPW + i;
#endif
        const float* src = ((j & 2) ? p.w_sigma : p.w_mu) + wrow + kk + (j & 1) * 4;
        __builtin_amdgcn_global_load_lds((const __attribute__((address_space(1))) void*)src,
                                         (__attribute__((address_space(3))) void*)&sm_all[p_idx(pbuf) + (fw * 4 + j) * 64], 16, 0, 0);
      }
    }
    if (decltype(wx_)::value) {
#pragma unroll
      for (int i = 0; i < XPW; ++i) {
        __builtin_amdgcn_global_load_lds((const __attribute__((address_space(1))) void*)(xs + xrow[i] + kk),
                                         (__attribute__((address_space(3))) void*)&sm_all[x_slot(xbuf) + (fw + i * NF) * 64], 16, 0, 0);
      }
      if (X3) {
#pragma unroll
        for (int i = 0; i < XPW; ++i) {
          __builtin_amdgcn_global_load_lds((const __attribute__((address_space(1))) void*)(xs_lo + xrow[i] + kk),
                                           (__attribute__((address_space(3))) void*)&sm_all[x_idx(xbuf) + sb * XT + 512 + (fw + i * NF) * 64], 16, 0, 0);
        }
      }
    }
  };
  auto stage_sel = [&](int t, int pbuf, int xbuf, auto wp_, auto wx_) __attribute__((always_inline)) {
    if ((t + 1) * 32 <= K) stage_fast(t, pbuf, xbuf, wp_, wx_);
    else stage_slow(t, pbuf, xbuf, wp_, wx_);
  };
  auto stage = [&](int t, int buf) __attribute__((always_inline)) { stage_sel(t, buf, buf, std::true_type{}, std::true_type{}); };
  const bool phantom = tile >= T;

  if (phantom) stage_sel(0, 0, 0, std::false_type{}, std::true_type{});
  else stage(0, 0);
  float bmu_pre = 0.f, brho_pre = 0.f, beps_pre = 0.f;
  if (q == 0 && n_ok) {
    bmu_pre = p.b_mu[n];
    brho_pre = p.b_rho[n];
    beps_pre = bias_eps(p, n, s, gs, do_dump);
  }
  asm volatile("s_waitcnt vmcnt(0)" ::: "memory");
  __syncthreads();

  f32x4 acc[8];
#pragma unroll
  for (int m = 0; m < 8; ++m) acc[m] = f32x4{0.f, 0.f, 0.f, 0.f};
  float s_e2 = 0.f, s_a = 0.f, s_ls = 0.f;

  typedef __attribute__((ext_vector_type(2))) float f32x2;
#ifdef BNN_STAMPS
  unsigned long long ph[5] = {0, 0, 0, 0, 0};
#define K2_T(v) const unsigned long long v = __builtin_amdgcn_s_memtime()
#else
#define K2_T(v)
#endif
  auto mfma_phase = [&](const bf16x8& wa, const bf16x8& wl, int xi, const f32x4& m_lo) __attribute__((always_inline)) {
    const uint32_t xa = lds0 + (uint32_t)((xi + q * 16 + r) * 16);
#ifdef BNN_TUNE
    const bool tune_nolds = (p.tune & 16) != 0, tune_nomfma = (p.tune & 32) != 0;
#else
    constexpr bool tune_nolds = false, tune_nomfma = false;
#endif
#pragma unroll
    for (int h = 0; h < 2; ++h) {
      f32x4 x0, x1, x2, x3;
      if (tune_nolds) {
        x0 = x1 = x2 = x3 = m_lo;
      } else if (h == 0)
        asm volatile("ds_read_b128 %0, %4\n\tds_read_b128 %1, %4 offset:1024\n\tds_read_b128 %2, %4 offset:2048\n\tds_read_b128 %3, %4 offset:3072"
                     : "=&v"(x0), "=&v"(x1), "=&v"(x2), "=&v"(x3) : "v"(xa));
      else
        asm volatile("ds_read_b128 %0, %4 offset:4096\n\tds_read_b128 %1, %4 offset:5120\n\tds_read_b128 %2, %4 offset:6144\n\tds_read_b128 %3, %4 offset:7168"
                     : "=&v"(x0), "=&v"(x1), "=&v"(x2), "=&v"(x3) : "v"(xa));
      if (X3) {
        f32x4 l0, l1, l2, l3;
        if (h == 0)
          asm volatile("ds_read_b128 %0, %4 offset:8192\n\tds_read_b128 %1, %4 offset:9216\n\tds_read_b128 %2, %4 offset:10240\n\tds_read_b128 %3, %4 offset:11264"
                       : "=&v"(l0), "=&v"(l1), "=&v"(l2), "=&v"(l3) : "v"(xa));
        else
          asm volatile("ds_read_b128 %0, %4 offset:12288\n\tds_read_b128 %1, %4 offset:13312\n\tds_read_b128 %2, %4 offset:14336\n\tds_read_b128 %3, %4 offset:15360"
                       : "=&v"(l0), "=&v"(l1), "=&v"(l2), "=&v"(l3) : "v"(xa));
        asm volatile("s_waitcnt lgkmcnt(4)" : "+v"(x0), "+v"(x1), "+v"(x2), "+v"(x3));
        acc[h * 4 + 0] = __builtin_amdgcn_mfma_f32_16x16x32_bf16(wa, __builtin_bit_cast(bf16x8, x0), acc[h * 4 + 0], 0, 0, 0);
        acc[h * 4 + 1] = __builtin_amdgcn_mfma_f32_16x16x32_bf16(wa, __builtin_bit_cast(bf16x8, x1), acc[h * 4 + 1], 0, 0, 0);
        acc[h * 4 + 2] = __builtin_amdgcn_mfma_f32_16x16x32_bf16(wa, __builtin_bit_cast(bf16x8, x2), acc[h * 4 + 2], 0, 0, 0);
        acc[h * 4 + 3] = __builtin_amdgcn_mfma_f32_16x16x32_bf16(wa, __builtin_bit_cast(bf16x8, x3), acc[h * 4 + 3], 0, 0, 0);
        acc[h * 4 + 0] = __builtin_amdgcn_mfma_f32_16x16x32_bf16(wl, __builtin_bit_cast(bf16x8, x0), acc[h * 4 + 0], 0, 0, 0);
        acc[h * 4 + 1] = __builtin_amdgcn_mfma_f32_16x16x32_bf16(wl, __builtin_bit_cast(bf16x8, x1), acc[h * 4 + 1], 0, 0, 0);
        acc[h * 4 + 2] = __builtin_amdgcn_mfma_f32_16x16x32_bf16(wl, __builtin_bit_cast(bf16x8, x2), acc[h * 4 + 2], 0, 0, 0);
        acc[h * 4 + 3] = __builtin_amdgcn_mfma_f32_16x16x32_bf16(wl, __builtin_bit_cast(bf16x8, x3), acc[h * 4 + 3], 0, 0, 0);
        asm volatile("s_waitcnt lgkmcnt(0)" : "+v"(l0), "+v"(l1), "+v"(l2), "+v"(l3));
        acc[h * 4 + 0] = __builtin_amdgcn_mfma_f32_16x16x32_bf16(wa, __builtin_bit_cast(bf16x8, l0), acc[h * 4 + 0], 0, 0, 0);
        acc[h * 4 + 1] = __builtin_amdgcn_mfma_f32_16x16x32_bf16(wa, __builtin_bit_cast(bf16x8, l1), acc[h * 4 + 1], 0, 0, 0);
        acc[h * 4 + 2] = __builtin_amdgcn_mfma_f32_16x16x32_bf16(wa, __builtin_bit_cast(bf16x8, l2), acc[h * 4 + 2], 0, 0, 0);
// ... 108 lines not shown
          lw[j] = __builtin_bit_cast(uint32_t, __builtin_convertvector(wv - hf, bf16x2));
        }
        wa = __builtin_bit_cast(bf16x8, make_uint4(hw[0], hw[1], hw[2], hw[3]));
        wl = __builtin_bit_cast(bf16x8, make_uint4(lw[0], lw[1], lw[2], lw[3]));
      } else {
#pragma unroll
        for (int j = 0; j < 4; ++j) {
          wa[2 * j] = lane_ok ? (__bf16)w2[j][0] : (__bf16)0.f;
          wa[2 * j + 1] = lane_ok ? (__bf16)w2[j][1] : (__bf16)0.f;
        }
      }
#ifdef BNN_STAMPS
      asm volatile("" :: "v"(wa));
#endif
      K2_T(st2);
      mfma_phase(wa, wl, x_idx(cur) + sb * XT, m_lo);
#ifdef BNN_STAMPS
      asm volatile("" :: "v"(acc[0]), "v"(acc[7]));
      K2_T(st3);
      ph[0] += st1 - st0; ph[1] += st2 - st1; ph[2] += st3 - st2;
#endif
    }
#ifdef BNN_TUNE
    if (!(p.tune & 2)) asm volatile("s_waitcnt vmcnt(0) lgkmcnt(0)" ::: "memory");
    if (!(p.tune & 1)) __builtin_amdgcn_s_barrier();
#else
    K2_T(st3w);
    asm volatile("s_waitcnt vmcnt(0) lgkmcnt(0)" ::: "memory");
    K2_T(st4);
    __builtin_amdgcn_s_barrier();
#endif
    asm volatile("" ::: "memory");
#ifdef BNN_STAMPS
    K2_T(st5);
    ph[3] += st4 - st3w; ph[4] += st5 - st4;
#endif
  };
  {
    const bool tile_full = (tile + 1) * 16 <= N;
    const int full_steps = tile_full ? (K >> 5) : 0;
    int t = 0, cur = 0;
#pragma nounroll
    for (; t < full_steps; ++t, cur = (cur + 1 == NB ? 0 : cur + 1)) step(t, cur, std::true_type{});
#pragma nounroll
    for (; t < ksteps; ++t, cur = (cur + 1 == NB ? 0 : cur + 1)) step(t, cur, std::false_type{});
  }

#ifdef BNN_STAMPS
  if (p.dbg && lane == 0 && blockIdx.x < 1024) {
    unsigned long long* d = p.dbg + ((size_t)blockIdx.x * NW + wave) * 8;
    d[0] = ph[0]; d[1] = ph[1]; d[2] = ph[2]; d[3] = ph[3]; d[4] = ph[4]; d[5] = (unsigned long long)ksteps;
  }
#endif
#undef K2_T
  float b_own = 0.f;
  if (q == 0) {
    if (n_ok) b_own = sample_bias(p, bmu_pre, brho_pre, beps_pre, do_stats, do_ls, s_e2, s_a, s_ls);
    if (!X3) bias_s[wave][r] = b_own;
  }
  if (do_stats) {
    const float a = wave_sum(s_e2), b = wave_sum(s_a), cc = wave_sum(s_ls);
    if (lane == 0 && tile < T) p.ws[1 + (size_t)s * T + tile] = make_float4(a, b, cc, 0.f);
  }
  float bq[4];
  if (X3) {
#pragma unroll
    for (int i = 0; i < 4; ++i) bq[i] = __shfl(b_own, q * 4 + i, 64);
  } else {
    __syncthreads();
  }
  if (!active) return;
  const int nb = tile * 16 + q * 4;
  const bool vec_ok = (N & 3) == 0;
  if (!X3) {
#pragma unroll
    for (int i = 0; i < 4; ++i) bq[i] = bias_s[wave][q * 4 + i];
  }
  if (nb >= N) return;
  auto store_tiles = [&](auto fast_, auto ybf_, auto relu_) __attribute__((always_inline)) {
    constexpr bool FAST = decltype(fast_)::value;
    const bool ybf = FAST ? decltype(ybf_)::value : p.y_bf16 != 0;
    const bool relu = FAST ? decltype(relu_)::value : p.relu != 0;
    const size_t esz = ybf ? 2 : 4;
    const size_t y0 = (((size_t)s * B + m0 + r) * N + nb) * esz, ystep = (size_t)16 * N * esz;
    char* yrow = reinterpret_cast<char*>(p.y) + y0;
    char* lrow = X3 ? reinterpret_cast<char*>(p.y_lo) + y0 : nullptr;
#pragma unroll
    for (int m = 0; m < 8; ++m, yrow += ystep, lrow += X3 ? ystep : 0) {
      if (!FAST && m0 + m * 16 + r >= B) continue;
      f32x4 v = acc[m];
#pragma unroll
      for (int i = 0; i < 4; ++i) {
        float o = v[i] + bq[i];
        if (relu) o = fmaxf(o, 0.f);
        v[i] = o;
      }
      if (ybf) {
        __bf16* yp = reinterpret_cast<__bf16*>(yrow);
        bf16x4 o;
#pragma unroll
        for (int i = 0; i < 4; ++i) o[i] = (__bf16)v[i];
        if (FAST || vec_ok) {
          *reinterpret_cast<bf16x4*>(yp) = o;
        } else {
#pragma unroll
          for (int i = 0; i < 4; ++i)
            if (nb + i < N) yp[i] = o[i];
        }
        if (X3) {
          __bf16* lp = reinterpret_cast<__bf16*>(lrow);
          bf16x4 l;
#pragma unroll
          for (int i = 0; i < 4; ++i) l[i] = (__bf16)(v[i] - (float)o[i]);
          if (FAST || vec_ok) {
            *reinterpret_cast<bf16x4*>(lp) = l;
          } else {
#pragma unroll
            for (int i = 0; i < 4; ++i)
              if (nb + i < N) lp[i] = l[i];
          }
        }
      } else {
        float* yp = reinterpret_cast<float*>(yrow);
        if (FAST || vec_ok) {
          *reinterpret_cast<float4*>(yp) = make_float4(v[0], v[1], v[2], v[3]);
        } else {
#pragma unroll
          for (int i = 0; i < 4; ++i)
            if (nb + i < N) yp[i] = v[i];
        }
      }
    }
  };
  constexpr std::true_type yes{};
  constexpr std::false_type no{};
  if (vec_ok && m0 + 128 <= B) {
    if (p.y_bf16) {
      if (p.relu) store_tiles(yes, yes, yes);
      else store_tiles(yes, yes, no);
    } else {
      if (p.relu) store_tiles(yes, no, yes);
      else store_tiles(yes, no, no);
    }
  } else {
    store_tiles(no, no, no);
  }
}

template <bool SIG, int EPS>
__global__ __launch_bounds__(256, 4) void bbb_fwd_gemm_rider_kernel(const BbbK p, const SampleK sk, int n_main) {
  __shared__ __attribute__((aligned(16))) float4 xt[2][8 * 64];
  __shared__ float bias_s[4][16];
  if ((int)blockIdx.x >= n_main) {
    sample_block(sk, (int)blockIdx.x - n_main, &bias_s[0][0]);
    return;
  }
  bbb_gemm_body<4, SIG, EPS>(p, xt, bias_s);
}

__global__ void bbb_layer_scalars_kernel(const float4* __restrict__ ws, int K, int N, bnn_prior prior,
                                         float* __restrict__ log_prior, float* __restrict__ log_q) {
  __shared__ double scratch[16];
  const int s = blockIdx.x;
  const int T = __float_as_int(ws[0].x);
  double e2 = 0, a = 0, ls = 0;
  for (int t = threadIdx.x; t < T; t += blockDim.x) {
    const float4 v = ws[1 + (size_t)s * T + t];
// ... 136 lines not shown
    pl.lds = kBgLds;
    return BNN_OK;
  }
  if (a->w_sampled) {
    tile_plan(S, B, K, N, true, 8, pl);
    pl.R = 1;
    pl.mt = 2;
    pl.tiles = (N + 15) / 16;
    pl.blocks = (long)pl.tiles * S * ((B + 31) / 32);
    pl.lds = ((size_t)pl.nw * 2 * 64 * 4 + 16 + 3 * pl.nw) * sizeof(float);
    return BNN_OK;
  }
  const long gemm_blocks = (long)((N + 63) / 64) * S * mbs;
  const bool x3 = a->math == BNN_MATH_BF16X3;
  const bool gemm_ok = al && (a->math == BNN_MATH_BF16 || x3) && a->x_dtype == BNN_BF16 && K >= 8 &&
                       (double)N * K * 4.0 < 4294967295.0 && (double)B * K * 2.0 < 4294967295.0 &&
                       (!x3 || (a->w_sigma && !a->rider && (long)S * mbs >= 2 * kGemmPairsX3 && !(reinterpret_cast<uintptr_t>(a->x_lo) & 15) &&
                                (a->y_dtype != BNN_BF16 || !(reinterpret_cast<uintptr_t>(a->y_lo) & 7))));
  const bool slice_ok = gemm_ok && !x3 && a->split_scratch && !(reinterpret_cast<uintptr_t>(a->split_scratch) & 15) &&
                        a->split_scratch_bytes >= bnn_bbb_split_scratch_bytes(S, B, N);
  int forced = 0;
#ifdef BNN_TUNE
  if (const char* v = getenv("BNN_TUNE_KSL")) forced = atoi(v);
#endif
  const int ksl = slice_ok ? kslices(gemm_blocks, K, a->form == BNN_FORM_GEMM_KSLICE ? 2 : 1, forced) : 1;
  int form = a->form;
  if ((form == BNN_FORM_GEMM && !gemm_ok) || (form == BNN_FORM_GEMM_KSLICE && ksl <= 1)) form = BNN_FORM_AUTO;
  if (a->y_bf16_copy) form = BNN_FORM_TILE;
  if (form == BNN_FORM_AUTO) {
    if (ksl > 1 && (long)K * N >= kSliceMinWeights && S >= kSliceMinSamples) form = BNN_FORM_GEMM_KSLICE;
    else if (gemm_ok && gemm_blocks >= kGemmMinBlocks) form = BNN_FORM_GEMM;
    else form = BNN_FORM_TILE;
  }
  if (form == BNN_FORM_TILE) {
    tile_plan(S, B, K, N, al, 8, pl);
    return BNN_OK;
  }
  pl.form = form;
  pl.R = 1; pl.nw = 4; pl.mt = 8; pl.tiles = (N + 15) / 16;
  pl.ksl = form == BNN_FORM_GEMM_KSLICE ? ksl : 1;
  pl.blocks = gemm_blocks * pl.ksl;
  pl.lds = 2 * 8 * 64 * 16 + 4 * 16 * sizeof(float);
  pl.pairs = 1;
  bool pairs_on = true;
#ifdef BNN_TUNE
  if (const char* v = getenv("BNN_TUNE_PAIRS")) pairs_on = atoi(v) != 0;
#endif
  const int pairs = x3 ? kGemmPairsX3 : kGemmPairs;
  if (pairs_on && form == BNN_FORM_GEMM && a->w_sigma && !a->rider && (long)S * mbs >= 2 * pairs) {
    pl.pairs = pairs;
    pl.nw = 4 * pairs;
    pl.blocks = (long)((N + 63) / 64) * (((long)S * mbs + pairs - 1) / pairs);
    pl.lds = x3 ? (4 * 256 + 2 * pairs * 1024) * 16 : kGemmRing * (4 * 256 + pairs * 512) * 16 + pl.nw * 16 * sizeof(float);
  }
  if (x3 && pl.pairs == 1) {
    tile_plan(S, B, K, N, al, 8, pl);
    return BNN_OK;
  }
  return BNN_OK;
}

static int prepare(const bnn_bbb_fwd_args* a, BbbK& k, bool& al) {
  k.mask = nullptr; k.mask_sstride = 0;
  k.w_pre = nullptr; k.b_pre = nullptr; k.wt_out = nullptr;
  if (a && a->w_sampled_t_out && !a->w_sampled) return BNN_ERR_NULL;
  if (!a) return BNN_ERR_NULL;
  if (a->struct_bytes != sizeof(bnn_bbb_fwd_args)) return BNN_ERR_ABI;
  if (a->n_samples <= 0 || a->batch <= 0 || a->in_features <= 0 || a->out_features <= 0) return BNN_ERR_SHAPE;
  if ((double)a->n_samples * ((a->batch + 127) / 128) * ((a->out_features + 3) / 4) > 2.0e9) return BNN_ERR_SHAPE;
  if (a->x_per_sample < 0) return BNN_ERR_SHAPE;
  const bool pre = a->w_sampled != nullptr;
  if (!a->x || !a->y) return BNN_ERR_NULL;
  if (!pre && (!a->w_mu || !a->w_rho || !a->b_mu || !a->b_rho)) return BNN_ERR_NULL;
  if (pre) {
    if (!a->b_sampled) return BNN_ERR_NULL;
    if (a->math != BNN_MATH_BF16 || a->want_stats || a->log_prior || a->log_q || a->eps_w_dump || a->eps_b_dump ||
        (a->in_features & 7))
      return BNN_ERR_SHAPE;
    if (!aligned16(a->x) || !aligned16(a->w_sampled)) return BNN_ERR_ALIGN;
  }
  if ((unsigned)a->x_dtype > 1u || (unsigned)a->y_dtype > 1u || (unsigned)a->math > 2u || (unsigned)a->eps_mode > 2u ||
      (unsigned)a->prior.kind > 1u || (unsigned)a->form > 4u)
    return BNN_ERR_ENUM;
  if (!pre && a->eps_mode == BNN_EPS_MEMORY && (!a->eps_w || !a->eps_b)) return BNN_ERR_NULL;
  if (a->want_stats) {
    if (!a->workspace || a->workspace_bytes < bnn_bbb_linear_fwd_workspace_bytes(a->n_samples, a->out_features))
      return BNN_ERR_WORKSPACE;
    if (!aligned16(a->workspace)) return BNN_ERR_ALIGN;
  }
  if ((a->log_prior || a->log_q) && !a->want_stats) return BNN_ERR_WORKSPACE;
  k.x_lo = nullptr; k.y_lo = nullptr;
  if (a->math == BNN_MATH_BF16X3) {
    if (pre || a->y_bf16_copy || a->rider) return BNN_ERR_ENUM;
    if (a->x_dtype == BNN_BF16) {
      if (!a->x_lo) return BNN_ERR_NULL;
      if (reinterpret_cast<uintptr_t>(a->x_lo) & 1) return BNN_ERR_ALIGN;
      k.x_lo = a->x_lo;
    }
    if (a->y_dtype == BNN_BF16) {
      if (!a->y_lo) return BNN_ERR_NULL;
      if ((a->out_features % 4 == 0) && (reinterpret_cast<uintptr_t>(a->y_lo) & 7)) return BNN_ERR_ALIGN;
      k.y_lo = a->y_lo;
    }
  }
  k.x = a->x;
  k.x_sstride = a->x_per_sample ? (long)a->batch * a->in_features : 0;
  k.xg = a->x_per_sample > 0 ? a->x_per_sample : 1;
  k.sgrp = a->sample_group; k.sgrp_stride = a->sample_group_stride;
  k.w_mu = a->w_mu; k.w_rho = a->w_rho; k.b_mu = a->b_mu; k.b_rho = a->b_rho;
  k.w_sigma = a->w_sigma;
  if (a->w_sigma && (reinterpret_cast<uintptr_t>(a->w_sigma) & 15)) return BNN_ERR_ALIGN;
  k.eps_w = a->eps_w; k.eps_b = a->eps_b; k.eps_w_dump = a->eps_w_dump; k.eps_b_dump = a->eps_b_dump;
  k.y = a->y;
  k.ws = a->want_stats ? reinterpret_cast<float4*>(a->workspace) : nullptr;
  k.S = a->n_samples; k.B = a->batch; k.K = a->in_features; k.N = a->out_features;
  k.eps_mode = a->eps_mode; k.prior_kind = a->prior.kind; k.want_stats = a->want_stats ? 1 : 0;
  k.y16 = reinterpret_cast<__bf16*>(a->y_bf16_copy);
  if (a->y_bf16_copy && a->y_dtype != BNN_F32) return BNN_ERR_ENUM;
  k.relu = a->relu ? 1 : 0; k.y_bf16 = a->y_dtype == BNN_BF16; k.spb = 1; k.ksl = 1; k.ks_part = nullptr; k.ks_ticket = nullptr; k.ldw = 0;
  k.k0 = (uint32_t)a->seed; k.k1 = (uint32_t)(a->seed >> 32);
  k.layer_id = a->layer_id; k.sample_offset = a->sample_offset; k.sample_counter = a->sample_counter;
#ifdef BNN_STAMPS
  {
    const char* v = getenv("BNN_HIP_DBG_PTR");
    k.dbg = v ? reinterpret_cast<unsigned long long*>(strtoull(v, nullptr, 0)) : nullptr;
  }
#endif
  const double c0 = -0.91893853320467274178;
  k.pi = a->prior.pi;
  if (a->prior.kind == BNN_PRIOR_MIXTURE) {
    if (!(a->prior.sigma1 > 0.f) || !(a->prior.sigma2 > 0.f)) return BNN_ERR_SHAPE;
    k.inv2var1 = (float)(1.0 / (2.0 * (double)a->prior.sigma1 * a->prior.sigma1));
    k.inv2var2 = (float)(1.0 / (2.0 * (double)a->prior.sigma2 * a->prior.sigma2));
    k.c1 = (float)(c0 - log((double)a->prior.sigma1));
    k.c2 = (float)(c0 - log((double)a->prior.sigma2));
  } else {
    if (a->want_stats && !(a->prior.sigma_p > 0.f)) return BNN_ERR_SHAPE;
    k.inv2var1 = k.inv2var2 = k.c1 = k.c2 = 0.f;
  }
  const int K = a->in_features;
  al = (K % 8 == 0) && aligned16(a->x) && aligned16(a->w_mu) && aligned16(a->w_rho) && (!k.x_lo || aligned16(k.x_lo));
  if (pre) {
    k.w_pre = reinterpret_cast<const __bf16*>(a->w_sampled);
    k.b_pre = a->b_sampled;
    k.wt_out = reinterpret_cast<__bf16*>(a->w_sampled_t_out);
    k.eps_mode = BNN_EPS_ZERO;
    al = true;
  } else if (a->eps_mode == BNN_EPS_MEMORY) al = al && aligned16(a->eps_w);
  if (a->eps_w_dump) al = al && aligned16(a->eps_w_dump);
  const bool ybf = a->y_dtype == BNN_BF16;
  if ((a->out_features % 4 == 0) && (reinterpret_cast<uintptr_t>(a->y) & (ybf ? 7 : 15))) return BNN_ERR_ALIGN;
  return BNN_OK;
}

extern "C" int bnn_bbb_plan(const bnn_bbb_fwd_args* a, bnn_plan* out) {
  if (!out) return BNN_ERR_NULL;
  BbbK k;
  bool al = false;
  int rc = prepare(a, k, al);
  if (rc != BNN_OK) return rc;
  BbbPlan pl{};
  rc = bbb_plan(a, al, pl);
  if (rc != BNN_OK) return rc;
  out->form = pl.form;
  out->k_classes = pl.R;
  out->waves = pl.nw;
  out->batch_rows = 16 * pl.mt;
  out->k_slices = pl.ksl;
  out->blocks = (int32_t)pl.blocks;
  out->lds_bytes = (int32_t)pl.lds;
  out->features_per_block = pl.form == BNN_FORM_TILE ? 16 / pl.R : pl.form == BNN_FORM_BLOCK256 ? 256 : 64;
  return BNN_OK;
}

static int bbb_linear_fwd_impl(const bnn_bbb_fwd_args* a, void* stream_, bool no_bias, const float* grad_mask, long mask_sstride) {
  BbbK k;
  bool al = false;
  int rc = prepare(a, k, al);
  if (rc != BNN_OK) return rc;
  if (no_bias) k.b_pre = nullptr;
  if (grad_mask) {
    k.mask = grad_mask;
    k.mask_sstride = mask_sstride;
  }
  BbbPlan pl{};
  rc = bbb_plan(a, al, pl, grad_mask == nullptr);
  if (rc != BNN_OK) return rc;
  hipStream_t stream = reinterpret_cast<hipStream_t>(stream_);
  const int K = a->in_features;
  const int xdt = a->x_dtype, math = a->math;
  hipError_t err = hipSuccess;
  const dim3 grid((unsigned)(((pl.blocks + 7) / 8) * 8)), block(pl.nw * 64);
  SampleK sk;
  long rider_blocks = 0;
  bool ride = false;
  if (a->rider) {
    rc = fill_sample(a->rider, sk, rider_blocks);
    if (rc != BNN_OK) return rc;
    ride = !a->w_sampled && al && math == BNN_MATH_BF16 && pl.nw * 64 >= kSampleThreads;
    if (!ride) {
      rc = bnn_bbb_sample_weights(a->rider, stream_);
      if (rc != BNN_OK) return rc;
    }
  }
  if (pl.form == BNN_FORM_BLOCK256) {
    if (a->rider && ride) return BNN_ERR_SHAPE;
    BlockGemmK g{};
    g.x = reinterpret_cast<const __bf16*>(a->x);
    g.x_sstride = k.x_sstride; g.xg = k.xg;
    g.w = k.w_pre; g.bias = k.b_pre; g.y = a->y;
    g.y_bf16 = k.y_bf16; g.relu = k.relu;
    g.S = a->n_samples; g.M = a->batch; g.N = a->out_features; g.K = K;
    err = launch_block_gemm(g, stream);
    return err == hipSuccess ? BNN_OK : (int)err;
  }
  if (a->w_sampled) {
#define BNN_PRE(XDT)                                                                              \
  do {                                                                                            \
    err = allow_big_lds(bbb_fwd_pre_kernel<XDT, 1, 2>, pl.lds);                                   \
    if (err == hipSuccess)                                                                        \
      hipLaunchKernelGGL((bbb_fwd_pre_kernel<XDT, 1, 2>), grid, block, pl.lds, stream, k);        \
  } while (0)
    if (k.wt_out) {
      err = allow_big_lds(bbb_fwd_pre_kernel<BNN_BF16, 1, 2, true>, pl.lds);
      if (xdt != BNN_BF16) return BNN_ERR_ENUM;
      if (err == hipSuccess) hipLaunchKernelGGL((bbb_fwd_pre_kernel<BNN_BF16, 1, 2, true>), grid, block, pl.lds, stream, k);
    } else if (xdt == BNN_F32) BNN_PRE(BNN_F32); else BNN_PRE(BNN_BF16);
#undef BNN_PRE
    if (err != hipSuccess) return (int)err;
    err = hipGetLastError();
    return err == hipSuccess ? BNN_OK : (int)err;
  }
  if (pl.form != BNN_FORM_TILE) {
    k.ksl = pl.ksl;
#ifdef BNN_TUNE
    k.tune = getenv("BNN_TUNE_K1B") ? atoi(getenv("BNN_TUNE_K1B")) : 0;
#endif
    {
      size_t l2_budget = kL2WeightBudget;
#ifdef BNN_TUNE
      if (const char* v = getenv("BNN_TUNE_L2KB")) l2_budget = (size_t)atol(v) * 1024;
#endif
      const int mbs_ = (a->batch + 127) / 128;
      k.xc = xcd2d_make((a->out_features + 63) / 64, a->n_samples * mbs_, pl.ksl, (size_t)64 * K * 8, l2_budget);
    }
    if (pl.ksl > 1) {
      char* base = reinterpret_cast<char*>(a->split_scratch);
      k.ks_ticket = reinterpret_cast<uint32_t*>(base);
      k.ks_part = reinterpret_cast<float4*>(base + split_ticket_bytes(pl.blocks / pl.ksl));
    }
    if (pl.pairs > 1) {
      const int ub = (int)(((long)a->n_samples * ((a->batch + 127) / 128) + pl.pairs - 1) / pl.pairs);
      k.xc = xcd2d_make((a->out_features + 63) / 64, ub, 1, (size_t)64 * K * 8, kL2WeightBudget);
      const dim3 grid2((unsigned)(((pl.blocks + 7) / 8) * 8)), block2(pl.nw * 64);
      if (math == BNN_MATH_BF16X3) {
        if (k.eps_mode == BNN_EPS_PHILOX) hipLaunchKernelGGL((bbb_fwd_gemm2_kernel<4, kGemmPairsX3, BNN_EPS_PHILOX, 2, true>), grid2, block2, 0, stream, k);
        else if (k.eps_mode == BNN_EPS_MEMORY) hipLaunchKernelGGL((bbb_fwd_gemm2_kernel<4, kGemmPairsX3, BNN_EPS_MEMORY, 2, true>), grid2, block2, 0, stream, k);
        else hipLaunchKernelGGL((bbb_fwd_gemm2_kernel<4, kGemmPairsX3, BNN_EPS_ZERO, 2, true>), grid2, block2, 0, stream, k);
      } else if (k.eps_mode == BNN_EPS_PHILOX) hipLaunchKernelGGL((bbb_fwd_gemm2_kernel<4, kGemmPairs, BNN_EPS_PHILOX, kGemmRing>), grid2, block2, 0, stream, k);
      else if (k.eps_mode == BNN_EPS_MEMORY) hipLaunchKernelGGL((bbb_fwd_gemm2_kernel<4, kGemmPairs, BNN_EPS_MEMORY, kGemmRing>), grid2, block2, 0, stream, k);
      else hipLaunchKernelGGL((bbb_fwd_gemm2_kernel<4, kGemmPairs, BNN_EPS_ZERO, kGemmRing>), grid2, block2, 0, stream, k);
    } else if (ride) {
      const unsigned n_main = grid.x;
      const dim3 grid_r(n_main + (unsigned)rider_blocks);
#define BNN_GEMM_EPS(KERNEL, SIGV, ...)                                                                        \
  do {                                                                                                         \
    if (k.eps_mode == BNN_EPS_PHILOX) hipLaunchKernelGGL((KERNEL<SIGV, BNN_EPS_PHILOX>), __VA_ARGS__);          \
    else if (k.eps_mode == BNN_EPS_MEMORY) hipLaunchKernelGGL((KERNEL<SIGV, BNN_EPS_MEMORY>), __VA_ARGS__);     \
    else hipLaunchKernelGGL((KERNEL<SIGV, BNN_EPS_ZERO>), __VA_ARGS__);                                         \
  } while (0)
      if (a->w_sigma) BNN_GEMM_EPS(bbb_fwd_gemm_rider_kernel, true, grid_r, block, 0, stream, k, sk, (int)n_main);
      else BNN_GEMM_EPS(bbb_fwd_gemm_rider_kernel, false, grid_r, block, 0, stream, k, sk, (int)n_main);
    } else if (a->w_sigma) {
      if (k.eps_mode == BNN_EPS_PHILOX) hipLaunchKernelGGL((bbb_fwd_gemm_kernel<4, true, BNN_EPS_PHILOX>), grid, block, 0, stream, k);
      else if (k.eps_mode == BNN_EPS_MEMORY) hipLaunchKernelGGL((bbb_fwd_gemm_kernel<4, true, BNN_EPS_MEMORY>), grid, block, 0, stream, k);
      else hipLaunchKernelGGL((bbb_fwd_gemm_kernel<4, true, BNN_EPS_ZERO>), grid, block, 0, stream, k);
    } else {
      if (k.eps_mode == BNN_EPS_PHILOX) hipLaunchKernelGGL((bbb_fwd_gemm_kernel<4, false, BNN_EPS_PHILOX>), grid, block, 0, stream, k);
      else if (k.eps_mode == BNN_EPS_MEMORY) hipLaunchKernelGGL((bbb_fwd_gemm_kernel<4, false, BNN_EPS_MEMORY>), grid, block, 0, stream, k);
      else hipLaunchKernelGGL((bbb_fwd_gemm_kernel<4, false, BNN_EPS_ZERO>), grid, block, 0, stream, k);
    }
#undef BNN_GEMM_EPS
  } else if (ride) {
    const unsigned n_main = (unsigned)(((pl.blocks + 7) / 8) * 8);
    const dim3 grid_r(n_main + (unsigned)rider_blocks);
    const size_t lds_r = pl.lds > kSampleRedFloats * sizeof(float) ? pl.lds : kSampleRedFloats * sizeof(float);
#define BNN_RIDE(XDT, RR)                                                                                    \
  do {                                                                                                       \
    err = allow_big_lds(bbb_fwd_rider_kernel<XDT, RR>, lds_r);                                               \
    if (err == hipSuccess)                                                                                   \
      hipLaunchKernelGGL((bbb_fwd_rider_kernel<XDT, RR>), grid_r, block, lds_r, stream, k, sk, (int)n_main); \
  } while (0)
#define BNN_RIDE_R(XDT)                          \
  do {                                           \
    if (pl.R == 1) BNN_RIDE(XDT, 1);             \
    else if (pl.R == 2) BNN_RIDE(XDT, 2);        \
    else BNN_RIDE(XDT, 4);                       \
  } while (0)
    if (xdt == BNN_F32) BNN_RIDE_R(BNN_F32); else BNN_RIDE_R(BNN_BF16);
#undef BNN_RIDE
#undef BNN_RIDE_R
    if (err != hipSuccess) return (int)err;
  } else {
#define BNN_GO(MATH, XDT, RR, AL)                                                              \
  do {                                                                                         \
    err = allow_big_lds(bbb_fwd_kernel<MATH, XDT, RR, AL>, pl.lds);                            \
    if (err == hipSuccess)                                                                     \
      hipLaunchKernelGGL((bbb_fwd_kernel<MATH, XDT, RR, AL>), grid, block, pl.lds, stream, k); \
  } while (0)
#define BNN_GO_R(MATH, XDT)                                   \
  do {                                                        \
    if (!al) BNN_GO(MATH, XDT, 1, false);                     \
    else if (pl.R == 1) BNN_GO(MATH, XDT, 1, true);           \
    else if (pl.R == 2) BNN_GO(MATH, XDT, 2, true);           \
    else BNN_GO(MATH, XDT, 4, true);                          \
  } while (0)
    if (math == BNN_MATH_BF16) {
      if (xdt == BNN_F32) BNN_GO_R(BNN_MATH_BF16, BNN_F32); else BNN_GO_R(BNN_MATH_BF16, BNN_BF16);
    } else if (math == BNN_MATH_BF16X3) {
      if (xdt == BNN_F32) BNN_GO_R(BNN_MATH_BF16X3, BNN_F32); else BNN_GO_R(BNN_MATH_BF16X3, BNN_BF16);
    } else {
      if (xdt == BNN_F32) BNN_GO_R(BNN_MATH_F32, BNN_F32); else BNN_GO_R(BNN_MATH_F32, BNN_BF16);
    }
#undef BNN_GO
#undef BNN_GO_R
    if (err != hipSuccess) return (int)err;
  }
  err = hipGetLastError();
  if (err != hipSuccess) return (int)err;
  if (a->log_prior || a->log_q) {
    hipLaunchKernelGGL(bbb_layer_scalars_kernel, dim3(a->n_samples), dim3(256), 0, stream, k.ws, K, a->out_features,
                       a->prior, a->log_prior, a->log_q);
    err = hipGetLastError();
    if (err != hipSuccess) return (int)err;
  }
  return BNN_OK;
}

extern "C" int bnn_bbb_linear_fwd(const bnn_bbb_fwd_args* a, void* stream_) {
  return bbb_linear_fwd_impl(a, stream_, false, nullptr, 0);
}

static constexpr int kFinalMaxSlices = 8;
static constexpr int kFinalTicketMaxSamples = 16;
static constexpr int kRowsTicketMaxSamples = 64;

extern "C" int bnn_elbo_sums_(const bnn_finalize_args* f, void* stream);

extern "C" size_t bnn_bbb_final_scratch_bytes(int32_t n_samples) {
  if (n_samples <= 0) return 0;
  const size_t S = (size_t)n_samples;
  return ((S * 4 + 255) / 256) * 256 + S * kFinalMaxSlices * 16 + S * kFinalMaxSlices * (128 * 16 * 4);
}

extern "C" int bnn_loss_tail_(const bnn_finalize_args* f, void* stream_);
static int loss_tail(const bnn_finalize_args* f, void* stream_) { return bnn_loss_tail_(f, stream_); }

extern "C" int bnn_bbb_final_fwd(const bnn_bbb_fwd_args* a, const bnn_finalize_args* f, void* stream_) {
  BbbK k;
  bool al = false;
  int rc = prepare(a, k, al);
  if (rc != BNN_OK) return rc;
  FinPack fp;
  rc = make_fin(f, fp.k, fp.c);
  if (rc != BNN_OK) return rc;
  const int nl = f->n_layers;
  rc = check_fin_loss(f);
  if (rc != BNN_OK) return rc;
  if (a->w_sampled) {
    const int S = a->n_samples, B = a->batch, N = a->out_features, K = a->in_features;
    const bool rows = a->y_dtype == BNN_F32 && N <= 16 && B <= 128 && S <= 4096 && !f->local_reparam &&
                      nl >= 1 && f->n_samples == S && f->classes == N && f->batch == B && f->logits == a->y && f->nll &&
                      f->scratch && f->scratch_bytes >= bnn_bbb_final_scratch_bytes(S) &&
                      !(reinterpret_cast<uintptr_t>(f->scratch) & 15) &&
                      (S == 1 || f->ticket || (S > kRowsTicketMaxSamples && !f->loss)) && !a->rider &&
                      (N % 4 != 0 || !(reinterpret_cast<uintptr_t>(a->y) & 15));
    if (!rows) {
      rc = bnn_bbb_linear_fwd(a, stream_);
      if (rc == BNN_OK) rc = bnn_elbo_finalize(f, stream_);
      return rc != BNN_OK ? rc : loss_tail(f, stream_);
    }
    const FinLoss tr = make_fin_loss(f);
    FinRows fr;
    fr.x = a->x;
    fr.x_sstride = k.x_sstride; fr.xg = k.xg;
    fr.w = k.w_pre; fr.b = k.b_pre;
    fr.y = reinterpret_cast<float*>(a->y);
    fr.S = S; fr.B = B; fr.K = K; fr.N = N; fr.relu = a->relu ? 1 : 0;
    char* base = reinterpret_cast<char*>(f->scratch);
    fr.tickets = reinterpret_cast<uint32_t*>(base);
    fr.parts = reinterpret_cast<float*>(base + (((size_t)S * 4 + 255) / 256) * 256);
    const bool rows_tail = S > kRowsTicketMaxSamples && !tr.out4;
    fp.sums = f->sums;
    fp.ticket = rows_tail ? nullptr : f->ticket;
    fp.ks = 1; fp.ks_ticket = nullptr; fp.ks_stats = nullptr; fp.ks_tiles = nullptr;
    const int RB = (B + 15) / 16;
    if (a->x_dtype == BNN_BF16)
      hipLaunchKernelGGL(bbb_final_rows_kernel<false>, dim3((unsigned)(S * (RB + 1))), dim3(256), 0, reinterpret_cast<hipStream_t>(stream_),
                         fr, fp, tr);
    else
      hipLaunchKernelGGL(bbb_final_rows_kernel<true>, dim3((unsigned)(S * (RB + 1))), dim3(256), 0, reinterpret_cast<hipStream_t>(stream_),
                         fr, fp, tr);
    const hipError_t e2 = hipGetLastError();
    if (e2 != hipSuccess) return (int)e2;
    return rows_tail ? bnn_elbo_sums_(f, stream_) : (int)BNN_OK;
  }
  const bool fuse = al && a->out_features <= 16 && a->batch <= 128 && a->want_stats && !f->local_reparam && nl >= 1 &&
                    f->layer_workspace[nl - 1] == a->workspace && f->n_samples == a->n_samples &&
                    f->classes == a->out_features && f->batch == a->batch && a->y_dtype == BNN_F32 &&
                    (a->n_samples == 1 || a->n_samples > kFinalTicketMaxSamples || f->ticket != nullptr) && !(a->log_prior || a->log_q) &&
                    a->form == BNN_FORM_AUTO;
  if (!fuse) {
    rc = bnn_bbb_linear_fwd(a, stream_);
    if (rc != BNN_OK) return rc;
    rc = bnn_elbo_finalize(f, stream_);
    return rc != BNN_OK ? rc : loss_tail(f, stream_);
  }
  hipStream_t stream = reinterpret_cast<hipStream_t>(stream_);
  fp.sums = f->sums;
  const bool tail_kernel = a->n_samples > kFinalTicketMaxSamples;
  fp.ticket = tail_kernel ? nullptr : f->ticket;
  const int K = a->in_features;
  const int ssteps = (K + 31) / 32;
  int KS = (ssteps + 11) / 12;
  KS = KS > kFinalMaxSlices ? kFinalMaxSlices : KS;
  for (int ks = KS; ks <= kFinalMaxSlices; ++ks) {
    const int per = (ssteps + ks - 1) / ks;
    if (per <= 12 && ((per & 3) == 0 || per < 4)) {
      KS = ks;
      break;
    }
  }
  if ((long)a->n_samples * KS > 128) KS = 1;
  if (KS > 1 && (!f->scratch || f->scratch_bytes < bnn_bbb_final_scratch_bytes(a->n_samples) ||
                 (reinterpret_cast<uintptr_t>(f->scratch) & 15)))
    KS = 1;
  const int spb = (ssteps + KS - 1) / KS;
  int spw = 1;
  while ((spb + spw - 1) / spw > 12) ++spw;
  int nw = (spb + spw - 1) / spw;
  nw = nw < 1 ? 1 : nw;
  fp.ks = KS;
  {
    char* base = reinterpret_cast<char*>(f->scratch);
    const size_t S = (size_t)a->n_samples;
// ... 117 lines not shown
```

bayesian-neural-network_amd/csrc/bnn_device.h:

```cpp
#pragma once
#include <hip/hip_runtime.h>
#include <stdint.h>
#include "../../include/bnn_hip.h"

namespace bnn {

typedef __attribute__((ext_vector_type(4))) float f32x4;
typedef __attribute__((ext_vector_type(8))) __bf16 bf16x8;
typedef __attribute__((ext_vector_type(4))) __bf16 bf16x4;

constexpr int kWave = 64;
constexpr float kC0 = -0.918938533204672742f;
constexpr float kLn2 = 0.693147180559945309f;
constexpr float kLog2e = 1.442695040888963407f;

__device__ __forceinline__ uint32_t xor3(uint32_t a, uint32_t b, uint32_t c) {
#if __has_builtin(__builtin_amdgcn_bitop3_b32)
  return __builtin_amdgcn_bitop3_b32(a, b, c, 0x96);
#else
  return a ^ b ^ c;
#endif
}
template <int ROUNDS = BNN_PHILOX_ROUNDS>
__device__ __forceinline__ uint4 philox4x32(uint4 c, uint32_t k0, uint32_t k1) {
// ... 130 lines not shown
  const int chunk = (total + 7) >> 3;
  item = (b & 7) * chunk + (b >> 3);
  return (b >> 3) < chunk && item < total;
}

struct Xcd2D {
  int G, U, classes, inner;
};
__device__ __forceinline__ bool xcd2d_work_item(const Xcd2D& m, int& g, int& u, int& in) {
  const long total = (long)m.G * m.U * m.inner;
  const long chunk = (total + 7) >> 3;
  const int b = blockIdx.x;
  long f = (long)(b & 7) * chunk + (b >> 3);
  if ((b >> 3) >= chunk || f >= total) return false;
  const int base = m.G / m.classes, extra = m.G % m.classes;
  const long per_group = (long)m.U * m.inner;
  int h = 0, start = 0, size = base + (extra > 0 ? 1 : 0);
#pragma unroll 1
  while (f >= (long)size * per_group) {
    f -= (long)size * per_group;
    start += size;
    ++h;
    size = base + (h < extra ? 1 : 0);
  }
  const int row = size * m.inner;
  u = (int)(f / row);
  const int rem = (int)(f - (long)u * row);
  g = start + rem / m.inner;
  in = rem % m.inner;
  return true;
}
inline Xcd2D xcd2d_make(int G, int U, int inner, size_t group_bytes, size_t l2_budget) {
  Xcd2D m;
  m.G = G; m.U = U; m.inner = inner < 1 ? 1 : inner;
  size_t per = group_bytes ? l2_budget / group_bytes : (size_t)G;
  if (per < 1) per = 1;
  int c = (int)((G + per - 1) / per);
  m.classes = c < 1 ? 1 : (c > G ? G : c);
  return m;
}

__device__ __forceinline__ __bf16 split_lo(float v, __bf16 hi) { return (__bf16)(v - (float)hi); }

__device__ __forceinline__ __bf16 sq_bf16(float v) {
  const float r = (float)(__bf16)v;
  return (__bf16)(r * r);
}

__device__ __forceinline__ void cast_bf16_span(const float* __restrict__ src, __bf16* __restrict__ dst,
                                               __bf16* __restrict__ dsq, long n, int vec_ok, long tid, long nt,
                                               __bf16* __restrict__ dlo = nullptr) {
  if (vec_ok) {
    const long n8 = n >> 3;
    for (long i = tid; i < n8; i += nt) {
      const float4 a = reinterpret_cast<const float4*>(src)[2 * i], b = reinterpret_cast<const float4*>(src)[2 * i + 1];
      const float f[8] = {a.x, a.y, a.z, a.w, b.x, b.y, b.z, b.w};
      bf16x8 v, q, l;
#pragma unroll
      for (int j = 0; j < 8; ++j) {
        v[j] = (__bf16)f[j];
        l[j] = split_lo(f[j], v[j]);
        q[j] = dlo ? (__bf16)(f[j] * f[j]) : sq_bf16(f[j]);
      }
      reinterpret_cast<bf16x8*>(dst)[i] = v;
      if (dsq) reinterpret_cast<bf16x8*>(dsq)[i] = q;
      if (dlo) reinterpret_cast<bf16x8*>(dlo)[i] = l;
    }
    for (long i = (n8 << 3) + tid; i < n; i += nt) {
      const __bf16 h = (__bf16)src[i], l = split_lo(src[i], h);
      dst[i] = h;
      if (dsq) dsq[i] = dlo ? (__bf16)(src[i] * src[i]) : sq_bf16(src[i]);
      if (dlo) dlo[i] = l;
    }
  } else {
    for (long i = tid; i < n; i += nt) {
      const __bf16 h = (__bf16)src[i], l = split_lo(src[i], h);
      dst[i] = h;
      if (dsq) dsq[i] = dlo ? (__bf16)(src[i] * src[i]) : sq_bf16(src[i]);
      if (dlo) dlo[i] = l;
    }
  }
}

}
```

bayesian-neural-network_amd/csrc/reduce.hip:

```cpp
#include "bnn_device.h"
#include "bnn_fin.h"
#include "../../include/bnn_hip.h"

namespace bnn {

constexpr int kKlBlock = 256;
constexpr int kKlMaxBlocks = 2048;

__global__ __launch_bounds__(kKlBlock) void gauss_kl_partial_kernel(const float* __restrict__ mu,
                                                                  const float* __restrict__ rho, long n,
                                                                  int vec_ok, float4* __restrict__ partial) {
  __shared__ float scratch[3 * (kKlBlock / 64)];
  float ls = 0.f, s2 = 0.f, m2 = 0.f;
  const long tid = (long)blockIdx.x * blockDim.x + threadIdx.x;
  const long nthreads = (long)gridDim.x * blockDim.x;
  if (vec_ok) {
    const long n4 = n >> 2;
    const float4* mu4 = reinterpret_cast<const float4*>(mu);
    const float4* rho4 = reinterpret_cast<const float4*>(rho);
    for (long i = tid; i < n4; i += nthreads) {
      const float4 m = mu4[i], r = rho4[i];
      const float a = softplus(r.x), b = softplus(r.y), c = softplus(r.z), d = softplus(r.w);
      ls += (fast_log(a) + fast_log(b)) + (fast_log(c) + fast_log(d));
      s2 += (a * a + b * b) + (c * c + d * d);
// ... 118 lines not shown
    }
  }
}

__global__ __launch_bounds__(256) void nll_rows_kernel(const FinK p, const FinC cst, int rows_per_block, float* __restrict__ partial) {
  __shared__ float red[4];
  const int rb = blockIdx.x, s = blockIdx.y, nrb = gridDim.x;
  const int row0 = rb * rows_per_block, row1 = min(p.B, row0 + rows_per_block);
  const float acc = fin_nll(p, cst, s, p.logits + (size_t)s * p.B * p.C, p.C, row0, row1);
  const float w = wave_sum(acc);
  if ((threadIdx.x & 63) == 0) red[threadIdx.x >> 6] = w;
  __syncthreads();
  if (threadIdx.x == 0) partial[(size_t)s * nrb + rb] = ((red[0] + red[1]) + red[2]) + red[3];
}

__global__ void sample_sums_kernel(const float* __restrict__ a, const float* __restrict__ b,
                                   const float* __restrict__ c, int S, int g, float* sums, uint32_t* counter,
                                   uint32_t counter_inc) {
  __shared__ double scratch[16];
  if (g > 0 && g < S) {
    const int G = S / g;
    for (int m = blockIdx.x * blockDim.x + threadIdx.x; m < G; m += gridDim.x * blockDim.x) {
      double x = 0, y = 0, z = 0;
      for (int i = m * g; i < (m + 1) * g; ++i) {
        if (a) x += a[i];
        if (b) y += b[i];
        if (c) z += c[i];
      }
      if (sums) {
        sums[4 * m + 0] = (float)x;
        sums[4 * m + 1] = (float)y;
        sums[4 * m + 2] = (float)z;
        sums[4 * m + 3] = (float)g;
      }
    }
    if (counter && blockIdx.x == 0 && threadIdx.x == 0) *counter += counter_inc;
    return;
  }
  double x = 0, y = 0, z = 0;
  for (int i = threadIdx.x; i < S; i += blockDim.x) {
    if (a) x += a[i];
    if (b) y += b[i];
    if (c) z += c[i];
  }
  x = block_sum(x, scratch);
  y = block_sum(y, scratch);
  z = block_sum(z, scratch);
  if (threadIdx.x == 0) {
    if (sums) {
      sums[0] = (float)x;
      sums[1] = (float)y;
      sums[2] = (float)z;
      sums[3] = (float)S;
    }
    if (counter) *counter += counter_inc;
  }
}

__global__ void softplus_kernel(const float* __restrict__ rho, float* __restrict__ sigma, long n, int vec_ok) {
  const long tid = (long)blockIdx.x * blockDim.x + threadIdx.x, nt = (long)gridDim.x * blockDim.x;
  if (vec_ok) {
    for (long i = tid; i < (n >> 2); i += nt) {
      const float4 r = reinterpret_cast<const float4*>(rho)[i];
      reinterpret_cast<float4*>(sigma)[i] = make_float4(softplus(r.x), softplus(r.y), softplus(r.z), softplus(r.w));
    }
    for (long i = ((n >> 2) << 2) + tid; i < n; i += nt) sigma[i] = softplus(rho[i]);
  } else {
    for (long i = tid; i < n; i += nt) sigma[i] = softplus(rho[i]);
  }
}

struct PrepK {
  const float* rho[BNN_PREPARE_MAX];
  float* sigma[BNN_PREPARE_MAX];
  long n[BNN_PREPARE_MAX];
  int first_block[BNN_PREPARE_MAX + 1];
  int n_softplus;
  const float* cast_src;
  __bf16* cast_dst;
  __bf16* cast_dsq;
  __bf16* cast_dlo;
  long cast_n;
  int cast_vec;
};
constexpr int kPrepPerBlock = 4096;

__global__ __launch_bounds__(256) void eval_prepare_kernel(const PrepK p) {
  const int b = blockIdx.x;
  if (b >= p.first_block[p.n_softplus]) {
    const long lo = (long)(b - p.first_block[p.n_softplus]) * kPrepPerBlock;
    const long cnt = min((long)kPrepPerBlock, p.cast_n - lo);
    cast_bf16_span(p.cast_src + lo, p.cast_dst + lo, p.cast_dsq ? p.cast_dsq + lo : nullptr, cnt, p.cast_vec, threadIdx.x, 256,
                   p.cast_dlo ? p.cast_dlo + lo : nullptr);
    return;
  }
  int j = 0;
#pragma unroll 1
  while (j + 1 < p.n_softplus && b >= p.first_block[j + 1]) ++j;
  const long lo = (long)(b - p.first_block[j]) * kPrepPerBlock;
  const long cnt = min((long)kPrepPerBlock, p.n[j] - lo);
  const float* rho = p.rho[j] + lo;
  float* sg = p.sigma[j] + lo;
  const bool vec = !((reinterpret_cast<uintptr_t>(rho) | reinterpret_cast<uintptr_t>(sg)) & 15);
  if (vec) {
    for (long i = threadIdx.x; i < (cnt >> 2); i += 256) {
      const float4 r = reinterpret_cast<const float4*>(rho)[i];
      reinterpret_cast<float4*>(sg)[i] = make_float4(softplus(r.x), softplus(r.y), softplus(r.z), softplus(r.w));
    }
    for (long i = ((cnt >> 2) << 2) + threadIdx.x; i < cnt; i += 256) sg[i] = softplus(rho[i]);
  } else {
    for (long i = threadIdx.x; i < cnt; i += 256) sg[i] = softplus(rho[i]);
  }
}


__global__ void philox_normal_kernel(float* __restrict__ eps, uint32_t k0, uint32_t k1, uint32_t tensor_id,
                                     uint32_t sample_offset, int S, int rows, int cols) {
  const int gpr = (cols + 3) >> 2;
  const long groups = (long)rows * gpr;
  const long total = groups * S;
  for (long i = (long)blockIdx.x * blockDim.x + threadIdx.x; i < total; i += (long)gridDim.x * blockDim.x) {
    const int s = (int)(i / groups);
    const long g = i - (long)s * groups;
    const int row = (int)(g / gpr), c0 = (int)(g - (long)row * gpr) * 4;
    float e[4];
    philox_normal4((uint32_t)g, sample_offset + (uint32_t)s, tensor_id, k0, k1, e);
    float* out = eps + ((size_t)s * rows + row) * cols + c0;
#pragma unroll
    for (int j = 0; j < 4; ++j)
      if (c0 + j < cols) out[j] = e[j];
  }
}

__device__ __forceinline__ void elbo_loss_block(const float* __restrict__ a, const float* __restrict__ b,
                                                const float* __restrict__ nll, const float* __restrict__ beta_p, int S,
                                                float total, float grad_scale, int local_reparam, float* __restrict__ out4,
                                                float* __restrict__ g_a, float* __restrict__ g_b, float* __restrict__ g_nll,
                                                float* __restrict__ g_kl3) {
  __shared__ double scratch[16];
  double x = 0, y = 0, z = 0;
  for (int i = threadIdx.x; i < S; i += blockDim.x) {
    x += a[i];
    if (b) y += b[i];
    z += nll[i];
  }
  x = block_sum(x, scratch);
  y = block_sum(y, scratch);
  z = block_sum(z, scratch);
  const float beta = *beta_p;
  const float inv = grad_scale / total;
  for (int i = threadIdx.x; i < S; i += blockDim.x) {
    if (g_a) g_a[i] = local_reparam ? 0.f : -beta * inv;
    if (g_b) g_b[i] = beta * inv;
    if (g_nll) g_nll[i] = inv;
  }
  if (threadIdx.x == 0) {
    const float am = (float)x / total, bm = (float)y / total, nm = (float)z / total;
    out4[0] = local_reparam ? beta * am + nm : beta * bm - beta * am + nm;
    out4[1] = am;
    out4[2] = bm;
    out4[3] = nm;
    if (g_kl3) { g_kl3[0] = beta * grad_scale; g_kl3[1] = 0.f; g_kl3[2] = 0.f; }
  }
}

__global__ void elbo_loss_kernel(const float* __restrict__ a, const float* __restrict__ b, const float* __restrict__ nll,
                                 const float* __restrict__ beta_p, int S, float total, float grad_scale, int local_reparam,
                                 float* __restrict__ out4, float* __restrict__ g_a, float* __restrict__ g_b,
                                 float* __restrict__ g_nll, float* __restrict__ g_kl3) {
  elbo_loss_block(a, b, nll, beta_p, S, total, grad_scale, local_reparam, out4, g_a, g_b, g_nll, g_kl3);
}
// ... 255 lines not shown
    hipLaunchKernelGGL(sample_sums_kernel, dim3(1), dim3(256), 0, stream, first, second, a->nll, a->n_samples,
                       a->group_samples, a->sums, (uint32_t*)nullptr, 0u);
    err = hipGetLastError();
  }
  return err == hipSuccess ? BNN_OK : (int)err;
}

extern "C" int bnn_philox_normal(float* eps, uint64_t seed, uint32_t tensor_id, uint32_t sample_offset,
                                 int32_t n_samples, int32_t rows, int32_t cols, void* stream_) {
  if (!eps) return BNN_ERR_NULL;
  if (n_samples <= 0 || rows <= 0 || cols <= 0) return BNN_ERR_SHAPE;
  const long total = (long)n_samples * rows * ((cols + 3) / 4);
  long nb = (total + 255) / 256;
  if (nb > 4096) nb = 4096;
  hipLaunchKernelGGL(philox_normal_kernel, dim3((unsigned)nb), dim3(256), 0, reinterpret_cast<hipStream_t>(stream_), eps,
                     (uint32_t)seed, (uint32_t)(seed >> 32), tensor_id, sample_offset, n_samples, rows, cols);
  hipError_t err = hipGetLastError();
  return err == hipSuccess ? BNN_OK : (int)err;
}

extern "C" int bnn_elbo_sums_(const bnn_finalize_args* f, void* stream_) {
  const float* first = f->local_reparam ? f->kl : f->log_prior;
  const float* second = f->local_reparam ? nullptr : f->log_q;
  hipLaunchKernelGGL(sample_sums_kernel, dim3(1), dim3(256), 0, reinterpret_cast<hipStream_t>(stream_), first, second,
                     f->nll, f->n_samples, f->group_samples, f->sums, f->sample_counter, f->sample_counter_inc);
  hipError_t err = hipGetLastError();
  return err == hipSuccess ? BNN_OK : (int)err;
}

extern "C" int bnn_softplus(const float* rho, float* sigma, int64_t n, void* stream_) {
  if (!rho || !sigma) return BNN_ERR_NULL;
  if (n <= 0) return BNN_ERR_SHAPE;
  if ((reinterpret_cast<uintptr_t>(rho) | reinterpret_cast<uintptr_t>(sigma)) & 3) return BNN_ERR_ALIGN;
  const int vec_ok = !((reinterpret_cast<uintptr_t>(rho) | reinterpret_cast<uintptr_t>(sigma)) & 15);
  long nb = (n / 4 + 255) / 256;
  nb = nb < 1 ? 1 : (nb > 2048 ? 2048 : nb);
  hipLaunchKernelGGL(softplus_kernel, dim3((unsigned)nb), dim3(256), 0, reinterpret_cast<hipStream_t>(stream_), rho, sigma,
                     (long)n, vec_ok);
  hipError_t err = hipGetLastError();
  return err == hipSuccess ? BNN_OK : (int)err;
}

extern "C" int bnn_cast_bf16(const float* src, void* dst, void* dst_sq, int64_t n, void* stream_) {
  if (!src || !dst) return BNN_ERR_NULL;
  if (n <= 0) return BNN_ERR_SHAPE;
  if ((reinterpret_cast<uintptr_t>(src) & 3) || (reinterpret_cast<uintptr_t>(dst) & 1)) return BNN_ERR_ALIGN;
  const int vec_ok = !((reinterpret_cast<uintptr_t>(src) | reinterpret_cast<uintptr_t>(dst) |
                        reinterpret_cast<uintptr_t>(dst_sq)) & 15);
  long nb = (n / 8 + 255) / 256;
  nb = nb < 1 ? 1 : (nb > 2048 ? 2048 : nb);
  hipLaunchKernelGGL(cast_bf16_kernel, dim3((unsigned)nb), dim3(256), 0, reinterpret_cast<hipStream_t>(stream_), src,
                     reinterpret_cast<__bf16*>(dst), reinterpret_cast<__bf16*>(dst_sq), (long)n, vec_ok);
  hipError_t err = hipGetLastError();
  return err == hipSuccess ? BNN_OK : (int)err;
}

extern "C" int bnn_eval_prepare(const bnn_prepare_args* a, void* stream_) {
  if (!a) return BNN_ERR_NULL;
  if (a->struct_bytes != sizeof(bnn_prepare_args)) return BNN_ERR_ABI;
  if (a->n_softplus < 0 || a->n_softplus > BNN_PREPARE_MAX || a->cast_n < 0) return BNN_ERR_SHAPE;
  PrepK k{};
  long blocks = 0;
  for (int i = 0; i < a->n_softplus; ++i) {
    if (!a->rho[i] || !a->sigma[i]) return BNN_ERR_NULL;
    if (a->n[i] <= 0) return BNN_ERR_SHAPE;
    if ((reinterpret_cast<uintptr_t>(a->rho[i]) | reinterpret_cast<uintptr_t>(a->sigma[i])) & 3) return BNN_ERR_ALIGN;
    k.rho[i] = a->rho[i]; k.sigma[i] = a->sigma[i]; k.n[i] = (long)a->n[i];
    k.first_block[i] = (int)blocks;
    blocks += (a->n[i] + kPrepPerBlock - 1) / kPrepPerBlock;
    if (blocks > 0x3fffffff) return BNN_ERR_SHAPE;
  }
  k.n_softplus = a->n_softplus;
  for (int i = a->n_softplus; i <= BNN_PREPARE_MAX; ++i) k.first_block[i] = (int)blocks;
  if (a->cast_n > 0) {
    if (!a->cast_src || !a->cast_dst) return BNN_ERR_NULL;
    if ((reinterpret_cast<uintptr_t>(a->cast_src) & 3) || (reinterpret_cast<uintptr_t>(a->cast_dst) & 1) ||
        (reinterpret_cast<uintptr_t>(a->cast_dst_sq) & 1) || (reinterpret_cast<uintptr_t>(a->cast_dst_lo) & 1))
      return BNN_ERR_ALIGN;
    k.cast_src = a->cast_src; k.cast_dst = reinterpret_cast<__bf16*>(a->cast_dst);
    k.cast_dsq = reinterpret_cast<__bf16*>(a->cast_dst_sq); k.cast_n = (long)a->cast_n;
    k.cast_dlo = reinterpret_cast<__bf16*>(a->cast_dst_lo);
    k.cast_vec = !((reinterpret_cast<uintptr_t>(a->cast_src) | reinterpret_cast<uintptr_t>(a->cast_dst) |
                    reinterpret_cast<uintptr_t>(a->cast_dst_sq) | reinterpret_cast<uintptr_t>(a->cast_dst_lo)) & 15);
    blocks += (a->cast_n + kPrepPerBlock - 1) / kPrepPerBlock;
    if (blocks > 0x3fffffff) return BNN_ERR_SHAPE;
  }
  if (blocks == 0) return BNN_ERR_SHAPE;
  hipLaunchKernelGGL(eval_prepare_kernel, dim3((unsigned)blocks), dim3(256), 0, reinterpret_cast<hipStream_t>(stream_), k);
  hipError_t err = hipGetLastError();
  return err == hipSuccess ? BNN_OK : (int)err;
}

extern "C" int bnn_version(void) { return BNN_HIP_ABI_VERSION; }
extern "C" int bnn_philox_rounds(void) { return BNN_PHILOX_ROUNDS; }

extern "C" const char* bnn_status_string(int status) {
  switch (status) {
    case BNN_OK: return "ok";
    case BNN_ERR_NULL: return "required pointer is NULL";
    case BNN_ERR_SHAPE: return "non-positive or unsupported dimension";
    case BNN_ERR_ENUM: return "unknown dtype / mode / prior kind";
    case BNN_ERR_WORKSPACE: return "workspace missing or too small";
    case BNN_ERR_ABI: return "struct_bytes mismatch (header/library version skew)";
    case BNN_ERR_ALIGN: return "pointer not aligned";
    default: return status > 0 ? "hip runtime error (status is a hipError_t)" : "unknown status";
  }
}
```

include/bnn_hip.h:

```cpp
#ifndef BNN_HIP_H_
#define BNN_HIP_H_

#include <stddef.h>
#include <stdint.h>

#ifdef __cplusplus
extern "C" {
#endif

#define BNN_HIP_ABI_VERSION 9
#define BNN_EPS_MAP_VERSION 2
#ifndef BNN_PHILOX_ROUNDS
#define BNN_PHILOX_ROUNDS 7
#endif

enum bnn_status {
  BNN_OK = 0,
  BNN_ERR_NULL = -1,
  BNN_ERR_SHAPE = -2,
  BNN_ERR_ENUM = -3,
  BNN_ERR_WORKSPACE = -4,
  BNN_ERR_ABI = -5,
  BNN_ERR_ALIGN = -6
};

enum bnn_dtype { BNN_F32 = 0, BNN_BF16 = 1 };

enum bnn_math { BNN_MATH_F32 = 0, BNN_MATH_BF16 = 1, BNN_MATH_BF16X3 = 2 };

enum bnn_eps_mode {
  BNN_EPS_PHILOX = 0,
  BNN_EPS_MEMORY = 1,
  BNN_EPS_ZERO = 2
};

enum bnn_prior_kind {
  BNN_PRIOR_GAUSS = 0,
  BNN_PRIOR_MIXTURE = 1
};

enum bnn_nll_mode { BNN_NLL_REGRESSION = 0, BNN_NLL_CLASSIFICATION = 1 };

enum bnn_form { BNN_FORM_AUTO = 0, BNN_FORM_TILE = 1, BNN_FORM_GEMM = 2, BNN_FORM_GEMM_KSLICE = 3, BNN_FORM_BLOCK256 = 4 };

typedef struct bnn_prior {
  int32_t kind;
  float sigma_p;
  float pi;
  float sigma1;
  float sigma2;
} bnn_prior;

typedef struct bnn_plan {
  int32_t form;
  int32_t k_classes;
  int32_t waves;
  int32_t batch_rows;
  int32_t k_slices;
  int32_t blocks;
  int32_t lds_bytes;
  int32_t features_per_block;
} bnn_plan;

struct bnn_bbb_sample_args;

typedef struct bnn_bbb_fwd_args {
  uint32_t struct_bytes;
  int32_t n_samples, batch, in_features, out_features;
  const void* x;
  int32_t x_dtype;
  int32_t x_per_sample;
  const float* w_mu;
  const float* w_rho;
  const float* b_mu;
  const float* b_rho;
  int32_t eps_mode;
  int32_t math;
  const float* eps_w;
  const float* eps_b;
  uint64_t seed;
  uint32_t layer_id;
  uint32_t sample_offset;
  const uint32_t* sample_counter;
  uint32_t sample_group;
  uint32_t sample_group_stride;
  float* eps_w_dump;
  float* eps_b_dump;
  bnn_prior prior;
  int32_t want_stats;
  int32_t relu;
  void* workspace;
  size_t workspace_bytes;
  float* log_prior;
  float* log_q;
  void* y;
  int32_t y_dtype;
  int32_t form;
  void* split_scratch;
  size_t split_scratch_bytes;
  const float* w_sigma;
  const void* w_sampled;
  const float* b_sampled;
  const struct bnn_bbb_sample_args* rider;
  void* y_bf16_copy;
  void* w_sampled_t_out;
  const void* x_lo;
  void* y_lo;
} bnn_bbb_fwd_args;

size_t bnn_bbb_linear_fwd_workspace_bytes(int32_t n_samples, int32_t out_features);
size_t bnn_bbb_split_scratch_bytes(int32_t n_samples, int32_t batch, int32_t out_features);
size_t bnn_bbb_split_scratch_zero_bytes(int32_t n_samples, int32_t batch, int32_t out_features);
int bnn_bbb_linear_fwd(const bnn_bbb_fwd_args* args, void* stream);
int bnn_bbb_plan(const bnn_bbb_fwd_args* args, bnn_plan* plan);

#define BNN_SAMPLE_MAX_LAYERS 8
typedef struct bnn_bbb_sample_layer {
  int32_t in_features, out_features;
  uint32_t layer_id;
  int32_t reserved;
  const float* w_mu;
  const float* w_rho;
  const float* b_mu;
  const float* b_rho;
  void* w_out;
  float* b_out;
  void* workspace;
  size_t workspace_bytes;
  bnn_prior prior;
  int32_t reserved2;
} bnn_bbb_sample_layer;

typedef struct bnn_bbb_sample_args {
  uint32_t struct_bytes;
  int32_t n_layers;
  int32_t n_samples;
  uint32_t sample_offset;
  uint64_t seed;
  const uint32_t* sample_counter;
  uint32_t sample_group;
  uint32_t sample_group_stride;
  bnn_bbb_sample_layer layer[BNN_SAMPLE_MAX_LAYERS];
  const float* cast_src;
  void* cast_dst;
  int64_t cast_n;
} bnn_bbb_sample_args;

size_t bnn_bbb_sample_workspace_bytes(int32_t n_samples, int32_t in_features, int32_t out_features);
int bnn_bbb_sample_weights(const bnn_bbb_sample_args* args, void* stream);

typedef struct bnn_lr_rider {
  uint32_t struct_bytes;
  int32_t in_features, out_features;
  const float* w_mu;
  const float* w_rho;
  const float* b_mu;
  const float* b_rho;
  void* w_frag;
  size_t w_frag_bytes;
  void* kl_workspace;
  size_t kl_workspace_bytes;
} bnn_lr_rider;

typedef struct bnn_lr_fwd_args {
  uint32_t struct_bytes;
  int32_t n_samples, batch, in_features, out_features;
  const void* x;
  int32_t x_dtype;
  int32_t x_per_sample;
  const float* w_mu;
  const float* w_rho;
  const float* b_mu;
  const float* b_rho;
  int32_t eps_mode;
  int32_t math;
  const float* eps_act;
  const float* eps_b;
  uint64_t seed;
  uint32_t layer_id;
  uint32_t sample_offset;
  const uint32_t* sample_counter;
  uint32_t sample_group;
  uint32_t sample_group_stride;
  float* eps_act_dump;
  float* eps_b_dump;
  float sigma_p;
  int32_t want_kl;
  int32_t relu;
  int32_t form;
  void* workspace;
// ... 651 lines not shown
} bnn_mc_score_args;
size_t bnn_mc_score_workspace_bytes(int32_t groups, int32_t batch, int32_t classes);
int bnn_mc_score(const bnn_mc_score_args* args, void* stream);

typedef struct bnn_sparse_count_args {
  uint32_t struct_bytes;
  int32_t out_features;
  int32_t in_features;
  int32_t ld;
  int32_t level;
  int32_t reserved;
  const uint8_t* code;
  int32_t* row_ptr;
} bnn_sparse_count_args;
int bnn_sparse_count(const bnn_sparse_count_args* args, void* stream);

typedef struct bnn_sparse_fill_args {
  uint32_t struct_bytes;
  int32_t out_features;
  int32_t in_features;
  int32_t ld;
  int32_t level;
  int32_t transposed;
  const uint8_t* code;
  const int32_t* row_ptr;
  const float* mu;
  const float* rho;
  uint16_t* col;
  float* mu_val;
  float* rho_val;
} bnn_sparse_fill_args;
int bnn_sparse_fill(const bnn_sparse_fill_args* args, void* stream);

typedef struct bnn_sparse_fwd_args {
  uint32_t struct_bytes;
  int32_t n_samples;
  int32_t rows;
  int32_t in_features;
  int32_t out_features;
  int32_t eps_mode;
  int32_t relu;
  int32_t x_per_sample;
  int32_t x_feature_major;
  int32_t y_feature_major;
  uint32_t layer_id;
  uint32_t sample_offset;
  uint64_t seed;
  uint32_t sample_group;
  uint32_t sample_group_stride;
  int32_t reserved0, reserved1;
  const uint32_t* sample_counter;
  const int32_t* row_ptr;
  const uint16_t* col;
  const float* mu_val;
  const float* sigma_val;
  const float* b_mu;
  const float* b_sigma;
  const float* x;
  float* y;
  const float* eps;
  const float* eps_b;
  float* eps_dump;
  float* eps_b_dump;
  float* x_scratch;
} bnn_sparse_fwd_args;
int bnn_sparse_fwd(const bnn_sparse_fwd_args* args, void* stream);

int bnn_softplus(const float* rho, float* sigma, int64_t n, void* stream);

int bnn_cast_bf16(const float* src, void* dst_bf16, void* dst_sq_bf16 , int64_t n, void* stream);

#define BNN_PREPARE_MAX 8
typedef struct bnn_prepare_args {
  uint32_t struct_bytes;
  int32_t n_softplus;
  const float* rho[BNN_PREPARE_MAX];
  float* sigma[BNN_PREPARE_MAX];
  int64_t n[BNN_PREPARE_MAX];
  const float* cast_src;
  void* cast_dst;
  void* cast_dst_sq;
  int64_t cast_n;
  void* cast_dst_lo;
} bnn_prepare_args;
int bnn_eval_prepare(const bnn_prepare_args* args, void* stream);

int bnn_version(void);
int bnn_philox_rounds(void);
const char* bnn_status_string(int status);

#ifdef __cplusplus
}
#endif
#endif
```

Baseline: 428,200.

## Add piece-order activation and parameter layouts for the 8-wave GEMM forward path

Introduces a tiled "pieces" memory layout for bf16 activations and for the interleaved fp32 mu/sigma parameters. The layout matches the fragment order consumed by the 8-wave GEMM BBB forward kernel. eval_prepare gains paths that write the input cast and the softplus(rho)/mu pairs directly in this order, and the engine switches hidden-layer buffers to it when the plan selects that kernel form. The goal is coalesced, fragment-ready loads with no in-kernel reshuffling. In exchange it adds extra layout-specialised kernel instantiations, extra prepare work and buffer-format constraints, such as rejecting the final/LR paths.

```diff
diff --git a/bayesian-neural-network_amd/bnn_hip/_lib.py b/bayesian-neural-network_amd/bnn_hip/_lib.py
--- a/bayesian-neural-network_amd/bnn_hip/_lib.py
+++ b/bayesian-neural-network_amd/bnn_hip/_lib.py
@@ -13,6 +13,7 @@
 PRIOR_GAUSS, PRIOR_MIXTURE = 0, 1
 NLL_REGRESSION, NLL_CLASSIFICATION = 0, 1
 FORM_AUTO, FORM_TILE, FORM_GEMM, FORM_GEMM_KSLICE, FORM_BLOCK256 = 0, 1, 2, 3, 4
+LAYOUT_ROWS, LAYOUT_PIECES = 0, 1
 
 EXPORTS = (
     "bnn_version", "bnn_philox_rounds", "bnn_status_string",
@@ -62,6 +63,7 @@
         ("split_scratch", C.c_void_p), ("split_scratch_bytes", C.c_size_t), ("w_sigma", C.c_void_p),
         ("w_sampled", C.c_void_p), ("b_sampled", C.c_void_p), ("rider", C.c_void_p), ("y_bf16_copy", C.c_void_p),
         ("w_sampled_t_out", C.c_void_p), ("x_lo", C.c_void_p), ("y_lo", C.c_void_p),
+        ("x_layout", C.c_int32), ("y_layout", C.c_int32), ("w_pieces", C.c_void_p),
     ]
 
 
@@ -205,7 +207,9 @@
     _fields_ = [("struct_bytes", C.c_uint32), ("n_softplus", C.c_int32),
                 ("rho", C.c_void_p * PREPARE_MAX), ("sigma", C.c_void_p * PREPARE_MAX), ("n", C.c_int64 * PREPARE_MAX),
                 ("cast_src", C.c_void_p), ("cast_dst", C.c_void_p), ("cast_dst_sq", C.c_void_p), ("cast_n", C.c_int64),
-                ("cast_dst_lo", C.c_void_p)]
+                ("cast_dst_lo", C.c_void_p), ("cast_layout", C.c_int32), ("cast_batch", C.c_int32), ("cast_features", C.c_int32),
+                ("mu", C.c_void_p * PREPARE_MAX), ("pieces", C.c_void_p * PREPARE_MAX),
+                ("rows", C.c_int32 * PREPARE_MAX), ("cols", C.c_int32 * PREPARE_MAX)]
 
 
 PREDICTIVE_MAX_QUANTILES = 8
diff --git a/bayesian-neural-network_amd/bnn_hip/engine.py b/bayesian-neural-network_amd/bnn_hip/engine.py
--- a/bayesian-neural-network_amd/bnn_hip/engine.py
+++ b/bayesian-neural-network_amd/bnn_hip/engine.py
@@ -539,6 +539,17 @@
                 self.w_pre[i] = torch.empty((S, n_i, k_i), dtype=torch.bfloat16, device=dev)
                 self.b_pre[i] = torch.empty((S, n_i), dtype=torch.float32, device=dev)
                 self.ws[i] = ops.sample_workspace(S, k_i, n_i, dev)
+        self.k1b2 = self._k1b2_layers() if state.pieces else [False] * nl
+        for i in range(nl - 1):
+            if self.k1b2[i] and i == 0 and self.x16 is not None:
+                self.x16 = ops.pieces_activation(self.x.shape, dev)
+            elif self.k1b2[i] and i > 0 and self.k1b2[i - 1]:
+                self.bufs[i - 1] = ops.pieces_activation(self.bufs[i - 1].shape, dev)
+        self.wpieces = [ops.param_pieces(sp.in_out[1], sp.in_out[0], dev) if (k and state.param_pieces) else None
+                        for sp, k in zip(self.specs, self.k1b2)]
+        for w, pc in zip(self.wsigma, self.wpieces):
+            if pc is not None:
+                w.bnn_param_pieces = pc
         self.graph = None
         self.calls = None
         if capture == "calls":
@@ -577,7 +588,8 @@
         if self.x16 is not None or hoist:
             ops.eval_prepare([self.specs[i].m.weight_rho.detach() for i in hoist], [self.wsigma[i] for i in hoist],
                              cast=self.x if self.x16 is not None else None, cast_out=self.x16,
-                             cast_out_sq=self.x16_sq, cast_out_lo=self.x16_lo)
+                             cast_out_sq=self.x16_sq, cast_out_lo=self.x16_lo,
+                             mus=[self.specs[i].m.weight_mu.detach() for i in hoist], pieces=[self.wpieces[i] for i in hoist])
             if self.x16 is not None:
                 h, h_sq, h_lo = self.x16, self.x16_sq, self.x16_lo
         last = len(self.specs) - 1
@@ -594,9 +606,7 @@
                       ticket=self.ticket, scratch=self.scratch, group_samples=self.group)
         for i, sp in enumerate(self.specs):
             p = tuple(t.detach() for t in (sp.m.weight_mu, sp.m.weight_rho, sp.m.bias_mu, sp.m.bias_rho))
-            common = dict(n_samples=self.n_local, math_mode=math_mode, relu=sp.relu, y_dtype=self.bufs[i].dtype,
-                          eps_mode=L.EPS_PHILOX, seed=state.seed, layer_id=sp.layer_id, sample_offset=self.lo,
-                          sample_counter=self.counter, workspace=self.ws[i], out=self.bufs[i], form=state.form, **grp)
+            common = self._common_kw(i)
             if self.lr:
                 if self.lr_x3 and i == last:
                     common["math_mode"] = L.MATH_F32
@@ -617,9 +627,7 @@
                 if i == last:
                     ops.elbo_finalize(workspaces=self.ws, logits=self.bufs[i], **fin_kw)
             else:
-                kw = dict(prior=sp.m._prior_spec, want_stats=True, split_scratch=self.split[i], w_sigma=self.wsigma[i], **common)
-                if self.x3:
-                    kw.update(x_lo=h_lo if h.dtype == torch.bfloat16 else None, out_lo=self.bufs_lo[i])
+                kw = self._bbb_kw(i, h, h_lo, common)
                 if i == last and self.rows:
                     ops.bbb_final_fwd((h, None, None, None, None),
                                       dict(n_samples=self.n_local, prior=sp.m._prior_spec, math_mode=math_mode, relu=sp.relu,
@@ -629,17 +637,45 @@
                 elif i == last:
                     ops.bbb_final_fwd((h,) + p, kw, dict(workspaces=self.ws[:last], **fin_kw))
                 else:
-                    if i == self.pre_from:
-                        kw["rider"] = ops.build_sample_job(
-                            [dict(w_mu=q.m.weight_mu.detach(), w_rho=q.m.weight_rho.detach(), b_mu=q.m.bias_mu.detach(),
-                                  b_rho=q.m.bias_rho.detach(), prior=q.m._prior_spec, layer_id=q.layer_id,
-                                  workspace=self.ws[j], w_out=self.w_pre[j], b_out=self.b_pre[j])
-                             for j, q in enumerate(self.specs) if j > i],
-                            n_samples=self.n_local, seed=state.seed, sample_offset=self.lo, sample_counter=self.counter, **grp)
                     ops.bbb_linear_fwd(h, *p, **kw)
             h, h_lo = self.bufs[i], self.bufs_lo[i]
         if self.lr:
             ops.elbo_finalize(workspaces=self.ws, logits=h, **fin_kw)
+
+    def _common_kw(self, i):
+        sp = self.specs[i]
+        grp = dict(sample_group=self.group, sample_group_stride=self.samples) if self.G > 1 else {}
+        return dict(n_samples=self.n_local, math_mode=self.math, relu=sp.relu, y_dtype=self.bufs[i].dtype,
+                    eps_mode=L.EPS_PHILOX, seed=state.seed, layer_id=sp.layer_id, sample_offset=self.lo,
+                    sample_counter=self.counter, workspace=self.ws[i], out=self.bufs[i], form=state.form, **grp)
+
+    def _bbb_kw(self, i, h, h_lo, common):
+        sp = self.specs[i]
+        kw = dict(prior=sp.m._prior_spec, want_stats=True, split_scratch=self.split[i], w_sigma=self.wsigma[i], **common)
+        if self.x3:
+            kw.update(x_lo=h_lo if h.dtype == torch.bfloat16 else None, out_lo=self.bufs_lo[i])
+        if i == self.pre_from and i < len(self.specs) - 1:
+            grp = dict(sample_group=self.group, sample_group_stride=self.samples) if self.G > 1 else {}
+            kw["rider"] = ops.build_sample_job(
+                [dict(w_mu=q.m.weight_mu.detach(), w_rho=q.m.weight_rho.detach(), b_mu=q.m.bias_mu.detach(),
+                      b_rho=q.m.bias_rho.detach(), prior=q.m._prior_spec, layer_id=q.layer_id,
+                      workspace=self.ws[j], w_out=self.w_pre[j], b_out=self.b_pre[j])
+                 for j, q in enumerate(self.specs) if j > i],
+                n_samples=self.n_local, seed=state.seed, sample_offset=self.lo, sample_counter=self.counter, **grp)
+        return kw
+
+    def _k1b2_layers(self):
+        res = [False] * len(self.specs)
+        if self.lr or self.math != L.MATH_BF16:
+            return res
+        h = self.x16 if self.x16 is not None else self.x
+        for i, sp in enumerate(self.specs[:-1]):
+            if not self.lib[i] and self.wsigma[i] is not None and h.dtype == torch.bfloat16:
+                p = tuple(t.detach() for t in (sp.m.weight_mu, sp.m.weight_rho, sp.m.bias_mu, sp.m.bias_rho))
+                plan = ops.bbb_plan(h, *p, **self._bbb_kw(i, h, None, self._common_kw(i)))
+                res[i] = plan["form"] == L.FORM_GEMM and plan["waves"] == 8
+            h = self.bufs[i]
+        return res
 
     def _sample_layer(self, i, grp):
         sp = self.specs[i]
diff --git a/bayesian-neural-network_amd/bnn_hip/ops.py b/bayesian-neural-network_amd/bnn_hip/ops.py
--- a/bayesian-neural-network_amd/bnn_hip/ops.py
+++ b/bayesian-neural-network_amd/bnn_hip/ops.py
@@ -66,7 +66,40 @@
     return L.MATH_F32 if math_mode == L.MATH_BF16X3 else math_mode
 
 
-def _x3(x: torch.Tensor, n_samples: int):
+def pieces_activation(shape, device) -> torch.Tensor:
+    shape = tuple(int(d) for d in shape)
+    if len(shape) not in (2, 3) or min(shape) < 1:
+        raise BnnHipError(f"pieces_activation: shape must be [batch,features] or [rows,batch,features], got {shape}")
+    rows = shape[0] if len(shape) == 3 else 1
+    t = torch.zeros((rows * ((shape[-2] + 127) // 128), (shape[-1] + 31) // 32, 8, 64, 8), dtype=torch.bfloat16, device=device)
+    t.bnn_pieces = shape
+    return t
+
+
+def param_pieces(out_features: int, in_features: int, device) -> torch.Tensor:
+    return torch.zeros(((out_features + 15) // 16, (in_features + 31) // 32, 4, 64, 4), dtype=torch.float32, device=device)
+
+
+def pieces_shape(t: Optional[torch.Tensor]):
+    return getattr(t, "bnn_pieces", None) if t is not None else None
+
+
+def unpiece(t: torch.Tensor) -> torch.Tensor:
+    shape = pieces_shape(t)
+    rows, B, K = (shape if len(shape) == 3 else (1,) + shape)
+    mbs, ks = (B + 127) // 128, (K + 31) // 32
+    v = t.view(rows, mbs, ks, 8, 4, 16, 8).permute(0, 1, 3, 5, 2, 4, 6).reshape(rows, mbs * 128, ks * 32)
+    return v[:, :B, :K].reshape(shape).contiguous()
+
+
+def _x3(x: torch.Tensor, n_samples: int, pieces_ok: bool = False):
+    shape = pieces_shape(x)
+    if shape is not None:
+        if not pieces_ok:
+            raise BnnHipError("a piece-order activation buffer (ops.pieces_activation) is read by bbb_linear_fwd only")
+        if len(shape) == 3 and n_samples % shape[0]:
+            raise BnnHipError(f"x has {shape[0]} row blocks, which does not divide {n_samples} samples")
+        return x, shape[-2], shape[-1], (n_samples // shape[0] if len(shape) == 3 else 0)
     if x.dim() == 2:
         xs = x if x.is_contiguous() else x.contiguous()
         return xs, x.shape[0], x.shape[1], 0
@@ -147,13 +180,21 @@
     return y16
 
 
+def _layouts(x, y, n_samples: int, B: int, N: int):
+    ys = pieces_shape(y)
+    if ys is not None and tuple(ys) != (n_samples, B, N):
+        raise BnnHipError(f"out: a piece-order buffer for {tuple(ys)}, the launch writes {(n_samples, B, N)}")
+    return (L.LAYOUT_PIECES if pieces_shape(x) is not None else L.LAYOUT_ROWS,
+            L.LAYOUT_PIECES if ys is not None else L.LAYOUT_ROWS)
+
+
 def _bbb_build(x, w_mu, w_rho, b_mu, b_rho, *, n_samples: int, prior: PriorSpec, math_mode: int,
                relu: bool, y_dtype: torch.dtype, eps_mode: int, eps_w=None, eps_b=None, seed: int = 0,
                layer_id: int = 0, sample_offset: int = 0, want_stats: bool = True,
                want_scalars: bool = False, dump_eps: bool = False, workspace=None, sample_counter=None,
                out=None, split_scratch=None, w_sigma=None, form: int = 0, sample_group: int = 0,
                sample_group_stride: int = 0, w_sampled=None, b_sampled=None, rider=None, want_y16: bool = False, wt_out=None,
-               x_lo=None, out_lo=None):
+               x_lo=None, out_lo=None, w_pieces=None):
     require_device(x, w_mu, w_rho, b_mu, b_rho, eps_w, eps_b, w_sampled, b_sampled)
     if w_sampled is not None:
         if w_sampled.dtype != torch.bfloat16 or b_sampled is None or b_sampled.dtype != torch.float32 or \
@@ -162,7 +203,7 @@
         if w_sampled.shape[0] != n_samples or b_sampled.numel() != n_samples * w_sampled.shape[1]:
             raise BnnHipError("w_sampled / b_sampled do not match n_samples")
         N, K = w_sampled.shape[1], w_sampled.shape[2]
-        xs, B, Kx, per_sample = _x3(x, n_samples)
+        xs, B, Kx, per_sample = _x3(x, n_samples, pieces_ok=True)
         if Kx != K:
             raise BnnHipError(f"shape mismatch: x[...,{Kx}] sampled weight {tuple(w_sampled.shape)}")
         y = out if out is not None else torch.empty((n_samples, B, N), dtype=y_dtype, device=xs.device)
@@ -170,6 +211,7 @@
         a.struct_bytes = C.sizeof(L.BbbFwdArgs)
         a.n_samples, a.batch, a.in_features, a.out_features = n_samples, B, K, N
         a.x, a.x_dtype, a.x_per_sample = xs.data_ptr(), _dt(xs), per_sample
+        a.x_layout, a.y_layout = _layouts(xs, y, n_samples, B, N)
         a.eps_mode, a.math = L.EPS_ZERO, L.MATH_BF16
         a.want_stats, a.relu = 0, int(relu)
         a.y, a.y_dtype = y.data_ptr(), _dt(y)
@@ -185,7 +227,7 @@
     w_mu, w_rho = _f32c(w_mu, "weight_mu"), _f32c(w_rho, "weight_rho")
     b_mu, b_rho = _f32c(b_mu, "bias_mu"), _f32c(b_rho, "bias_rho")
     N, K = w_mu.shape
-    xs, B, Kx, per_sample = _x3(x, n_samples)
+    xs, B, Kx, per_sample = _x3(x, n_samples, pieces_ok=True)
     if Kx != K or tuple(w_rho.shape) != (N, K) or tuple(b_mu.shape) != (N,) or tuple(b_rho.shape) != (N,):
         raise BnnHipError(f"shape mismatch: x[...,{Kx}] weight {tuple(w_mu.shape)} bias {tuple(b_mu.shape)}")
     dev = xs.device
@@ -218,6 +260,7 @@
     a.workspace_bytes = workspace.numel() * 4 if (want_stats and workspace is not None) else 0
     a.log_prior, a.log_q = _ptr(lp), _ptr(lq)
     a.y, a.y_dtype = y.data_ptr(), _dt(y)
+    a.x_layout, a.y_layout = _layouts(xs, y, n_samples, B, N)
     y_lo = None
     if math_mode == L.MATH_BF16X3:
         if xs.dtype == torch.bfloat16:
@@ -232,13 +275,21 @@
             a.y_lo = y_lo.data_ptr()
     if w_sigma is not None:
         a.w_sigma = w_sigma.data_ptr()
+        if w_pieces is None:
+            w_pieces = getattr(w_sigma, "bnn_param_pieces", None)
+    if w_pieces is not None:
+        require_device(w_pieces)
+        if w_sigma is None or w_pieces.dtype != torch.float32 or not w_pieces.is_contiguous() or \
+                w_pieces.numel() != ((N + 15) // 16) * ((K + 31) // 32) * 1024:
+            raise BnnHipError("w_pieces: ops.param_pieces(out, in) filled by eval_prepare, beside w_sigma")
+        a.w_pieces = w_pieces.data_ptr()
     if split_scratch is not None:
         a.split_scratch = split_scratch.data_ptr()
         a.split_scratch_bytes = split_scratch.numel() * split_scratch.element_size()
     if rider is not None:
         a.rider = C.addressof(rider[0])
     res = dict(y=y, y16=_y16(a, y) if want_y16 else None, workspace=workspace, log_prior=lp, log_q=lq, eps_w=dw, eps_b=db, y_lo=y_lo)
-    keep = (xs, w_mu, w_rho, b_mu, b_rho, eps_w, eps_b, sample_counter, split_scratch, w_sigma, rider, x_lo, y_lo)
+    keep = (xs, w_mu, w_rho, b_mu, b_rho, eps_w, eps_b, sample_counter, split_scratch, w_sigma, rider, x_lo, y_lo, w_pieces)
     a._keep = keep
     return a, res, keep
 
@@ -1003,7 +1054,8 @@
 
 
 def eval_prepare(rhos=(), sigmas=None, cast: Optional[torch.Tensor] = None, cast_out: Optional[torch.Tensor] = None,
-                 cast_out_sq: Optional[torch.Tensor] = None, want_sq: bool = False, cast_out_lo: Optional[torch.Tensor] = None):
+                 cast_out_sq: Optional[torch.Tensor] = None, want_sq: bool = False, cast_out_lo: Optional[torch.Tensor] = None,
+                 mus=None, pieces=None):
     lib = L.load()
     rhos = [_f32c(r, "rho") for r in rhos]
     require_device(*rhos, cast)
@@ -1018,6 +1070,15 @@
         if sg.shape != r.shape or sg.dtype != torch.float32 or not sg.is_contiguous():
             raise BnnHipError("eval_prepare: sigma must be a contiguous fp32 tensor of rho's shape")
         a.rho[i], a.sigma[i], a.n[i] = r.data_ptr(), sg.data_ptr(), r.numel()
+        pc = pieces[i] if pieces is not None else None
+        if pc is not None:
+            mu = _f32c(mus[i], "mu")
+            require_device(mu, pc)
+            if r.dim() != 2 or mu.shape != r.shape or pc.dtype != torch.float32 or not pc.is_contiguous() or \
+                    pc.numel() != ((r.shape[0] + 15) // 16) * ((r.shape[1] + 31) // 32) * 1024:
+                raise BnnHipError("eval_prepare: pieces[i] must be ops.param_pieces(out, in) of the [out, in] tensors mus[i] / rhos[i]")
+            a.mu[i], a.pieces[i], a.rows[i], a.cols[i] = mu.data_ptr(), pc.data_ptr(), r.shape[0], r.shape[1]
+            a._keep_mu = getattr(a, "_keep_mu", ()) + (mu,)
     if cast is not None:
         cast = _f32c(cast, "x")
         if cast_out is None:
@@ -1025,6 +1086,11 @@
         if want_sq and cast_out_sq is None:
             cast_out_sq = torch.empty(cast.shape, dtype=torch.bfloat16, device=cast.device)
         a.cast_src, a.cast_dst, a.cast_dst_sq, a.cast_n = cast.data_ptr(), cast_out.data_ptr(), _ptr(cast_out_sq), cast.numel()
+        ps = pieces_shape(cast_out)
+        if ps is not None:
+            if tuple(ps) != tuple(cast.shape):
+                raise BnnHipError(f"eval_prepare: cast_out is a piece-order buffer for {tuple(ps)}, the input is {tuple(cast.shape)}")
+            a.cast_layout, a.cast_batch, a.cast_features = L.LAYOUT_PIECES, ps[-2], ps[-1]
         if cast_out_lo is not None:
             if cast_out_lo.dtype != torch.bfloat16 or cast_out_lo.numel() != cast.numel() or not cast_out_lo.is_contiguous():
                 raise BnnHipError("eval_prepare: cast_out_lo must be a contiguous bf16 tensor of the input's size")
diff --git a/bayesian-neural-network_amd/bnn_hip/runtime.py b/bayesian-neural-network_amd/bnn_hip/runtime.py
--- a/bayesian-neural-network_amd/bnn_hip/runtime.py
+++ b/bayesian-neural-network_amd/bnn_hip/runtime.py
@@ -17,6 +17,8 @@
         self.counter = 0
         self.shard_samples = False
         self.form = L.FORM_AUTO
+        self.pieces = os.environ.get("BNN_HIP_PIECES", "1") != "0"
+        self.param_pieces = self.pieces and os.environ.get("BNN_HIP_PARAM_PIECES", "1") != "0"
         self.device_counter = None
 
 
diff --git a/bayesian-neural-network_amd/csrc/bbb_linear.hip b/bayesian-neural-network_amd/csrc/bbb_linear.hip
--- a/bayesian-neural-network_amd/csrc/bbb_linear.hip
+++ b/bayesian-neural-network_amd/csrc/bbb_linear.hip
@@ -44,6 +44,7 @@
   float inv2var1, c1, inv2var2, c2, pi;
   const void* x_lo;
   void* y_lo;
+  const char* w_pieces;
 #ifdef BNN_STAMPS
   unsigned long long* dbg;
 #endif
@@ -1183,9 +1184,11 @@
   bbb_gemm_body<NW, SIG, EPS>(p, xt, bias_s);
 }
 
-template <int NF, int SB, int EPS, int NB = 2, bool X3 = false>
+template <int NF, int SB, int EPS, int NB = 2, bool X3 = false, int LAY = 0>
 __global__ __launch_bounds__(NF * SB * 64, 4) void bbb_fwd_gemm2_kernel(const BbbK p) {
   constexpr int NW = NF * SB;
+  constexpr bool XTL = (LAY & 1) != 0, YTL = (LAY & 2) != 0, WTL = (LAY & 4) != 0;
+  static_assert(!X3 || LAY == 0, "piece order: bf16 form only");
   static_assert(NB == 2, "two staging buffers");
   constexpr int WPW = 4 / SB;
   constexpr int XPW = 8 / NF;
@@ -1237,8 +1240,30 @@
   for (int i = 0; i < XPW; ++i) voff_x[i] = ((uint32_t)xrow[i] + (uint32_t)(q * 8)) * 2u;
   const uint32_t lds0 = (uint32_t)(size_t)(__attribute__((address_space(3))) void*)&sm_all[0];
   auto x_slot = [&](int slot) { return x_idx(slot) + sb * XT; };
+  const char* xt_unit = reinterpret_cast<const char*>(xs) + (size_t)mb * (size_t)ksteps * 8192;
+  const uint32_t voff_xt = (uint32_t)lane * 16u;
+  const char* wt_tile = p.w_pieces + (size_t)tile * (size_t)ksteps * 4096;
+  auto stage_w_pieces = [&](int t, int pbuf) __attribute__((always_inline)) {
+#pragma unroll
+    for (int i = 0; i < WPW; ++i) {
+      const int j = sb * WPW + i;
+      const char* base = wt_tile + (size_t)t * 4096 + j * 1024;
+      const uint32_t m0v = lds0 + (uint32_t)((p_idx(pbuf) + (fw * 4 + j) * 64) * 16);
+      asm volatile("s_mov_b32 m0, %2\n\ts_nop 0\n\tglobal_load_lds_dwordx4 %0, %1" ::"v"(voff_xt), "s"(base), "s"(m0v) : "memory", "m0");
+    }
+  };
+  auto stage_x_pieces = [&](int t, int xbuf) __attribute__((always_inline)) {
+#pragma unroll
+    for (int i = 0; i < XPW; ++i) {
+      const char* base = xt_unit + (size_t)t * 8192 + (fw + i * NF) * 1024;
+      const uint32_t m0v = lds0 + (uint32_t)((x_slot(xbuf) + (fw + i * NF) * 64) * 16);
+      asm volatile("s_mov_b32 m0, %2\n\ts_nop 0\n\tglobal_load_lds_dwordx4 %0, %1" ::"v"(voff_xt), "s"(base), "s"(m0v) : "memory", "m0");
+    }
+  };
   auto stage_fast = [&](int t, int pbuf, int xbuf, auto wp_, auto wx_) __attribute__((always_inline)) {
-    if (decltype(wp_)::value) {
+    if (WTL && decltype(wp_)::value) {
+      stage_w_pieces(t, pbuf);
+    } else if (decltype(wp_)::value) {
 #pragma unroll
       for (int i = 0; i < WPW; ++i) {
         const int j = sb * WPW + i;
@@ -1247,7 +1272,9 @@
         asm volatile("s_mov_b32 m0, %2\n\ts_nop 0\n\tglobal_load_lds_dwordx4 %0, %1" ::"v"(voff_w), "s"(base), "s"(m0v) : "memory", "m0");
       }
     }
-    if (decltype(wx_)::value) {
+    if (XTL && decltype(wx_)::value) {
+      stage_x_pieces(t, xbuf);
+    } else if (decltype(wx_)::value) {
 #pragma unroll
       for (int i = 0; i < XPW; ++i) {
         const char* base = reinterpret_cast<const char*>(xs) + (size_t)t * 64;
@@ -1266,7 +1293,9 @@
   };
   auto stage_slow = [&](int t, int pbuf, int xbuf, auto wp_, auto wx_) __attribute__((always_inline)) {
     const int kk = min(t * 32 + q * 8, K - 8);
-    if (decltype(wp_)::value) {
+    if (WTL && decltype(wp_)::value) {
+      stage_w_pieces(t, pbuf);
+    } else if (decltype(wp_)::value) {
 #pragma unroll
       for (int i = 0; i < WPW; ++i) {
 #ifdef BNN_TUNE
@@ -1279,7 +1308,9 @@
                                          (__attribute__((address_space(3))) void*)&sm_all[p_idx(pbuf) + (fw * 4 + j) * 64], 16, 0, 0);
       }
     }
-    if (decltype(wx_)::value) {
+    if (XTL && decltype(wx_)::value) {
+      stage_x_pieces(t, xbuf);
+    } else if (decltype(wx_)::value) {
 #pragma unroll
       for (int i = 0; i < XPW; ++i) {
         __builtin_amdgcn_global_load_lds((const __attribute__((address_space(1))) void*)(xs + xrow[i] + kk),
@@ -1554,7 +1585,9 @@
     const bool ybf = FAST ? decltype(ybf_)::value : p.y_bf16 != 0;
     const bool relu = FAST ? decltype(relu_)::value : p.relu != 0;
     const size_t esz = ybf ? 2 : 4;
-    const size_t y0 = (((size_t)s * B + m0 + r) * N + nb) * esz, ystep = (size_t)16 * N * esz;
+    const size_t y0 = YTL ? (((size_t)unit * ((N + 31) >> 5) + (tile >> 1)) * 8192 + ((2 * (tile & 1) + (q >> 1)) * 16 + r) * 16 + (q & 1) * 8)
+                          : (((size_t)s * B + m0 + r) * N + nb) * esz;
+    const size_t ystep = YTL ? (size_t)1024 : (size_t)16 * N * esz;
     char* yrow = reinterpret_cast<char*>(p.y) + y0;
     char* lrow = X3 ? reinterpret_cast<char*>(p.y_lo) + y0 : nullptr;
 #pragma unroll
@@ -1857,6 +1890,10 @@
   if ((unsigned)a->x_dtype > 1u || (unsigned)a->y_dtype > 1u || (unsigned)a->math > 2u || (unsigned)a->eps_mode > 2u ||
       (unsigned)a->prior.kind > 1u || (unsigned)a->form > 4u)
     return BNN_ERR_ENUM;
+  if ((unsigned)a->x_layout > 1u || (unsigned)a->y_layout > 1u) return BNN_ERR_ENUM;
+  if ((a->x_layout && a->x_dtype != BNN_BF16) || (a->y_layout && a->y_dtype != BNN_BF16)) return BNN_ERR_ENUM;
+  if ((a->x_layout && !aligned16(a->x)) || (a->y_layout && !aligned16(a->y)) || !aligned16(a->w_pieces)) return BNN_ERR_ALIGN;
+  k.w_pieces = reinterpret_cast<const char*>(a->w_pieces);
   if (!pre && a->eps_mode == BNN_EPS_MEMORY && (!a->eps_w || !a->eps_b)) return BNN_ERR_NULL;
   if (a->want_stats) {
     if (!a->workspace || a->workspace_bytes < bnn_bbb_linear_fwd_workspace_bytes(a->n_samples, a->out_features))
@@ -1961,6 +1998,8 @@
   BbbPlan pl{};
   rc = bbb_plan(a, al, pl, grad_mask == nullptr);
   if (rc != BNN_OK) return rc;
+  if ((a->x_layout || a->y_layout || a->w_pieces) && !(pl.form == BNN_FORM_GEMM && pl.pairs > 1 && a->math == BNN_MATH_BF16))
+    return BNN_ERR_ENUM;
   hipStream_t stream = reinterpret_cast<hipStream_t>(stream_);
   const int K = a->in_features;
   const int xdt = a->x_dtype, math = a->math;
@@ -2032,9 +2071,30 @@
         if (k.eps_mode == BNN_EPS_PHILOX) hipLaunchKernelGGL((bbb_fwd_gemm2_kernel<4, kGemmPairsX3, BNN_EPS_PHILOX, 2, true>), grid2, block2, 0, stream, k);
         else if (k.eps_mode == BNN_EPS_MEMORY) hipLaunchKernelGGL((bbb_fwd_gemm2_kernel<4, kGemmPairsX3, BNN_EPS_MEMORY, 2, true>), grid2, block2, 0, stream, k);
         else hipLaunchKernelGGL((bbb_fwd_gemm2_kernel<4, kGemmPairsX3, BNN_EPS_ZERO, 2, true>), grid2, block2, 0, stream, k);
-      } else if (k.eps_mode == BNN_EPS_PHILOX) hipLaunchKernelGGL((bbb_fwd_gemm2_kernel<4, kGemmPairs, BNN_EPS_PHILOX, kGemmRing>), grid2, block2, 0, stream, k);
-      else if (k.eps_mode == BNN_EPS_MEMORY) hipLaunchKernelGGL((bbb_fwd_gemm2_kernel<4, kGemmPairs, BNN_EPS_MEMORY, kGemmRing>), grid2, block2, 0, stream, k);
-      else hipLaunchKernelGGL((bbb_fwd_gemm2_kernel<4, kGemmPairs, BNN_EPS_ZERO, kGemmRing>), grid2, block2, 0, stream, k);
+      } else {
+        const int lay = (a->x_layout == BNN_LAYOUT_PIECES ? 1 : 0) | (a->y_layout == BNN_LAYOUT_PIECES ? 2 : 0) | (a->w_pieces ? 4 : 0);
+        if (lay & 1) k.x_sstride = a->x_per_sample ? (long)((a->batch + 127) / 128) * ((K + 31) / 32) * 4096 : 0;
+#define BNN_GEMM2(LAYV)                                                                                                               \
+  do {                                                                                                                                \
+    if (k.eps_mode == BNN_EPS_PHILOX)                                                                                                 \
+      hipLaunchKernelGGL((bbb_fwd_gemm2_kernel<4, kGemmPairs, BNN_EPS_PHILOX, kGemmRing, false, LAYV>), grid2, block2, 0, stream, k); \
+    else if (k.eps_mode == BNN_EPS_MEMORY)                                                                                            \
+      hipLaunchKernelGGL((bbb_fwd_gemm2_kernel<4, kGemmPairs, BNN_EPS_MEMORY, kGemmRing, false, LAYV>), grid2, block2, 0, stream, k); \
+    else                                                                                                                              \
+      hipLaunchKernelGGL((bbb_fwd_gemm2_kernel<4, kGemmPairs, BNN_EPS_ZERO, kGemmRing, false, LAYV>), grid2, block2, 0, stream, k);   \
+  } while (0)
+        switch (lay) {
+          case 0: BNN_GEMM2(0); break;
+          case 1: BNN_GEMM2(1); break;
+          case 2: BNN_GEMM2(2); break;
+          case 3: BNN_GEMM2(3); break;
+          case 4: BNN_GEMM2(4); break;
+          case 5: BNN_GEMM2(5); break;
+          case 6: BNN_GEMM2(6); break;
+          default: BNN_GEMM2(7); break;
+        }
+#undef BNN_GEMM2
+      }
     } else if (ride) {
       const unsigned n_main = grid.x;
       const dim3 grid_r(n_main + (unsigned)rider_blocks);
@@ -2136,6 +2196,7 @@
   bool al = false;
   int rc = prepare(a, k, al);
   if (rc != BNN_OK) return rc;
+  if (a->x_layout || a->y_layout || a->w_pieces) return BNN_ERR_ENUM;
   FinPack fp;
   rc = make_fin(f, fp.k, fp.c);
   if (rc != BNN_OK) return rc;
diff --git a/bayesian-neural-network_amd/csrc/bnn_device.h b/bayesian-neural-network_amd/csrc/bnn_device.h
--- a/bayesian-neural-network_amd/csrc/bnn_device.h
+++ b/bayesian-neural-network_amd/csrc/bnn_device.h
@@ -236,4 +236,33 @@
   }
 }
 
-}
+__device__ __forceinline__ void cast_bf16_pieces(const float* __restrict__ src, __bf16* __restrict__ dst, int rows, int K, int t0,
+                                                 int vec_ok, int tid) {
+  const int q = tid & 3, r = (tid >> 2) & 15, t = t0 + (tid >> 6);
+  const int col = t * 32 + q * 8;
+  if (col >= K) return;
+  float f[8][8];
+#pragma unroll
+  for (int m = 0; m < 8; ++m) {
+    const int row = m * 16 + r;
+    if (row >= rows) continue;
+    const float* sp = src + (size_t)row * K + col;
+    if (vec_ok) {
+      const float4 a = reinterpret_cast<const float4*>(sp)[0], b = reinterpret_cast<const float4*>(sp)[1];
+      f[m][0] = a.x; f[m][1] = a.y; f[m][2] = a.z; f[m][3] = a.w; f[m][4] = b.x; f[m][5] = b.y; f[m][6] = b.z; f[m][7] = b.w;
+    } else {
+#pragma unroll
+      for (int i = 0; i < 8; ++i) f[m][i] = sp[i];
+    }
+  }
+#pragma unroll
+  for (int m = 0; m < 8; ++m) {
+    if (m * 16 + r >= rows) continue;
+    bf16x8 v;
+#pragma unroll
+    for (int i = 0; i < 8; ++i) v[i] = (__bf16)f[m][i];
+    reinterpret_cast<bf16x8*>(dst)[((size_t)t * 8 + m) * 64 + q * 16 + r] = v;
+  }
+}
+
+}
diff --git a/bayesian-neural-network_amd/csrc/reduce.hip b/bayesian-neural-network_amd/csrc/reduce.hip
--- a/bayesian-neural-network_amd/csrc/reduce.hip
+++ b/bayesian-neural-network_amd/csrc/reduce.hip
@@ -224,11 +224,52 @@
   __bf16* cast_dlo;
   long cast_n;
   int cast_vec;
+  int cast_pieces;
+  int cast_b, cast_k;
+  const float* pp_mu[BNN_PREPARE_MAX];
+  const float* pp_rho[BNN_PREPARE_MAX];
+  float4* pp_dst[BNN_PREPARE_MAX];
+  int pp_n[BNN_PREPARE_MAX], pp_k[BNN_PREPARE_MAX];
+  int pp_first[BNN_PREPARE_MAX + 1];
+  int n_pp;
 };
 constexpr int kPrepPerBlock = 4096;
 
 __global__ __launch_bounds__(256) void eval_prepare_kernel(const PrepK p) {
   const int b = blockIdx.x;
+  if (p.n_pp > 0 && b >= p.pp_first[0]) {
+    int j = 0;
+#pragma unroll 1
+    while (j + 1 < p.n_pp && b >= p.pp_first[j + 1]) ++j;
+    const int N = p.pp_n[j], K = p.pp_k[j], ksteps = (K + 31) >> 5, tq = (ksteps + 3) >> 2;
+    const int blk = b - p.pp_first[j], tile = blk / tq, t0 = (blk - tile * tq) * 4;
+    const int which = threadIdx.x >> 7, c = threadIdx.x & 7, r = (threadIdx.x >> 3) & 15;
+    const int n = tile * 16 + r;
+    if (n >= N) return;
+    const float* src = (which ? p.pp_rho[j] : p.pp_mu[j]) + (size_t)n * K + c * 4;
+    float4 v[4];
+#pragma unroll
+    for (int i = 0; i < 4; ++i)
+      if ((t0 + i) * 32 + c * 4 < K) v[i] = *reinterpret_cast<const float4*>(src + (t0 + i) * 32);
+#pragma unroll
+    for (int i = 0; i < 4; ++i) {
+      if ((t0 + i) * 32 + c * 4 >= K) continue;
+      if (which) v[i] = make_float4(softplus(v[i].x), softplus(v[i].y), softplus(v[i].z), softplus(v[i].w));
+      p.pp_dst[j][(((size_t)tile * ksteps + t0 + i) * 4 + which * 2 + (c & 1)) * 64 + (c >> 1) * 16 + r] = v[i];
+    }
+    return;
+  }
+  if (b >= p.first_block[p.n_softplus] && p.cast_pieces) {
+    const int ksteps = (p.cast_k + 31) >> 5, mbs = (p.cast_b + 127) >> 7, tq = (ksteps + 3) >> 2;
+    const long blk = b - p.first_block[p.n_softplus];
+    const int t0 = (int)(blk % tq) * 4;
+    const long um = blk / tq;
+    const int mb = (int)(um % mbs);
+    const long slot = um / mbs;
+    cast_bf16_pieces(p.cast_src + (slot * p.cast_b + (long)mb * 128) * p.cast_k, p.cast_dst + um * ksteps * 4096, p.cast_b - mb * 128,
+                     p.cast_k, t0, p.cast_vec, threadIdx.x);
+    return;
+  }
   if (b >= p.first_block[p.n_softplus]) {
     const long lo = (long)(b - p.first_block[p.n_softplus]) * kPrepPerBlock;
     const long cnt = min((long)kPrepPerBlock, p.cast_n - lo);
@@ -650,9 +691,34 @@
     k.cast_dlo = reinterpret_cast<__bf16*>(a->cast_dst_lo);
     k.cast_vec = !((reinterpret_cast<uintptr_t>(a->cast_src) | reinterpret_cast<uintptr_t>(a->cast_dst) |
                     reinterpret_cast<uintptr_t>(a->cast_dst_sq) | reinterpret_cast<uintptr_t>(a->cast_dst_lo)) & 15);
-    blocks += (a->cast_n + kPrepPerBlock - 1) / kPrepPerBlock;
+    if ((unsigned)a->cast_layout > 1u) return BNN_ERR_ENUM;
+    if (a->cast_layout == BNN_LAYOUT_PIECES) {
+      if (a->cast_dst_sq || a->cast_dst_lo) return BNN_ERR_ENUM;
+      if (a->cast_batch <= 0 || a->cast_features <= 0 || (a->cast_features & 7) ||
+          a->cast_n % ((int64_t)a->cast_batch * a->cast_features))
+        return BNN_ERR_SHAPE;
+      if (reinterpret_cast<uintptr_t>(a->cast_dst) & 15) return BNN_ERR_ALIGN;
+      k.cast_pieces = 1; k.cast_b = a->cast_batch; k.cast_k = a->cast_features;
+      blocks += a->cast_n / ((int64_t)a->cast_batch * a->cast_features) * ((a->cast_batch + 127) / 128) * ((a->cast_features + 127) / 128);
+    } else {
+      blocks += (a->cast_n + kPrepPerBlock - 1) / kPrepPerBlock;
+    }
     if (blocks > 0x3fffffff) return BNN_ERR_SHAPE;
   }
+  for (int i = 0; i < a->n_softplus; ++i) {
+    if (!a->pieces[i]) continue;
+    if (!a->mu[i]) return BNN_ERR_NULL;
+    if (a->rows[i] <= 0 || a->cols[i] <= 0 || (a->cols[i] & 7) || (int64_t)a->rows[i] * a->cols[i] != a->n[i]) return BNN_ERR_SHAPE;
+    if ((reinterpret_cast<uintptr_t>(a->mu[i]) | reinterpret_cast<uintptr_t>(a->rho[i]) | reinterpret_cast<uintptr_t>(a->pieces[i])) & 15)
+      return BNN_ERR_ALIGN;
+    const int j = k.n_pp++;
+    k.pp_mu[j] = a->mu[i]; k.pp_rho[j] = a->rho[i]; k.pp_dst[j] = reinterpret_cast<float4*>(a->pieces[i]);
+    k.pp_n[j] = a->rows[i]; k.pp_k[j] = a->cols[i];
+    k.pp_first[j] = (int)blocks;
+    blocks += (long)((a->rows[i] + 15) / 16) * ((a->cols[i] + 127) / 128);
+    if (blocks > 0x3fffffff) return BNN_ERR_SHAPE;
+  }
+  for (int j = k.n_pp; j <= BNN_PREPARE_MAX; ++j) k.pp_first[j] = (int)blocks;
   if (blocks == 0) return BNN_ERR_SHAPE;
   hipLaunchKernelGGL(eval_prepare_kernel, dim3((unsigned)blocks), dim3(256), 0, reinterpret_cast<hipStream_t>(stream_), k);
   hipError_t err = hipGetLastError();
diff --git a/include/bnn_hip.h b/include/bnn_hip.h
--- a/include/bnn_hip.h
+++ b/include/bnn_hip.h
@@ -63,6 +63,8 @@
 } bnn_plan;
 
 struct bnn_bbb_sample_args;
+
+typedef enum bnn_layout { BNN_LAYOUT_ROWS = 0, BNN_LAYOUT_PIECES = 1 } bnn_layout;
 
 typedef struct bnn_bbb_fwd_args {
   uint32_t struct_bytes;
@@ -106,6 +108,9 @@
   void* w_sampled_t_out;
   const void* x_lo;
   void* y_lo;
+  int32_t x_layout;
+  int32_t y_layout;
+  const void* w_pieces;
 } bnn_bbb_fwd_args;
 
 size_t bnn_bbb_linear_fwd_workspace_bytes(int32_t n_samples, int32_t out_features);
@@ -923,6 +928,11 @@
   void* cast_dst_sq;
   int64_t cast_n;
   void* cast_dst_lo;
+  int32_t cast_layout;
+  int32_t cast_batch, cast_features;
+  const float* mu[BNN_PREPARE_MAX];
+  void* pieces[BNN_PREPARE_MAX];
+  int32_t rows[BNN_PREPARE_MAX], cols[BNN_PREPARE_MAX];
 } bnn_prepare_args;
 int bnn_eval_prepare(const bnn_prepare_args* args, void* stream);
 
```

Result: faster. 478,000 (median of 6 runs) (+11.6%).
